# urw7rs/diffusion-models-made-easy

Hardware: AMD Instinct MI355X
Metric: denoising steps/sec + training images/sec, DDPM UNet CIFAR10 32×32 @1/2/4/8 GPU (higher is better)
Workload: dtype bf16; 1 GPU; DDPM T=1000 sampling, CIFAR10 32x32, default UNet (32,416,643 params, random init), batch 128 per GPU, t.shape=(1,); global_batch=128, parallelism=dp1 (independent chains per GPU, no data-path collective)

## Files before the change

### diffusion-models-made-easy_amd/_lib.py

```python

from __future__ import annotations

import ctypes as C
import os
import subprocess
import threading

_HERE = os.path.dirname(os.path.abspath(__file__))
LIB_PATH = os.environ.get("DMME_LIB_PATH") or os.path.join(_HERE, "libdmme_hip.so")
CSRC = os.path.join(_HERE, "csrc")

F16R32 = 4
F32, BF16, BF16X3, F16 = 0, 1, 2, 3
CHAIN_DDPM, CHAIN_DDIM, CHAIN_IDDPM, CHAIN_DDPM_GUIDED, CHAIN_DDIM_GUIDED, CHAIN_GDDIM = 0, 1, 2, 3, 4, 5
CHAIN_DDPM_CFG, CHAIN_GDDIM_CFG = 6, 7
CHAIN_DPMPP, CHAIN_DPMPP_CFG = 8, 9
CHAIN_REPAINT = 10
PRED_EPS, PRED_X0, PRED_V = 0, 1, 2
PREDICTIONS = {"eps": PRED_EPS, "x0": PRED_X0, "v": PRED_V}
ARCH_DDPM, ARCH_IDDPM, ARCH_CLASSIFIER, ARCH_DDPM_COND = 0, 1, 2, 3
DTYPES = {"fp32": F32, "float32": F32, "32": F32, "bf16": BF16, "bfloat16": BF16, "16": BF16, "bf16-mixed": BF16, "16-mixed": BF16,
          "bf16x3": BF16X3, "fp16": F16, "float16": F16, "half": F16, "fp16r32": F16R32}

_lock = threading.Lock()
# ... 7 lines not shown
        ("emb_dim", C.c_int),
        ("num_groups", C.c_int),
        ("dropout", C.c_float),
        ("num_depths", C.c_int),
        ("channels_per_depth", C.c_int * 8),
        ("num_blocks", C.c_int),
        ("num_attention_depths", C.c_int),
        ("attention_depths", C.c_int * 8),
        ("arch", C.c_int),
        ("num_heads", C.c_int),
        ("num_classes", C.c_int),
    ]


class ConvDesc(C.Structure):
    _fields_ = [(n, C.c_int) for n in (
        "dtype", "N", "Hin", "Win", "C1", "C2", "upsample", "stride", "taps", "Cout", "pro_silu", "out_silu",
        "nt", "tproj_ld", "in_nchw", "out_nchw", "force_generic")]


BUCKET_FN = C.CFUNCTYPE(None, C.c_void_p, C.c_int, C.c_int64, C.c_int64)


class DmmeError(RuntimeError):
    pass


def build(verbose: bool = False) -> str:
    cmd = ["make", "-C", CSRC, "-j", str(min(8, os.cpu_count() or 1))]
    res = subprocess.run(cmd, stdout=subprocess.PIPE, stderr=subprocess.STDOUT, text=True)
    if verbose or res.returncode != 0:
        print(res.stdout)
    if res.returncode != 0:
        raise DmmeError("building libdmme_hip.so failed")
    return LIB_PATH


_vp, _i, _i64, _f, _u64 = C.c_void_p, C.c_int, C.c_int64, C.c_float, C.c_uint64

PROTOTYPES = {
    "dmme_last_error": (C.c_char_p, []),
    "dmme_version": (_i, []),
    "dmme_device_count": (_i, []),
    "dmme_unet_plan_create": (_i, [C.POINTER(UNetCfg), _i, _i, _i, _i, _i, C.POINTER(_vp)]),
    "dmme_unet_plan_destroy": (None, [_vp]),
    "dmme_unet_plan_num_params": (_i, [_vp]),
    "dmme_unet_plan_param_info": (_i, [_vp, _i, C.c_char_p, _i, C.POINTER(_i), C.POINTER(_i64), C.POINTER(_i64), C.POINTER(_i)]),
    "dmme_unet_plan_ref_numel": (_i64, [_vp]),
    "dmme_unet_plan_packed_bytes": (_i64, [_vp]),
    "dmme_unet_plan_workspace_bytes": (_i64, [_vp]),
    "dmme_unet_plan_dropmask_numel": (_i64, [_vp]),
    "dmme_unet_plan_out_channels": (_i, [_vp]),
    "dmme_unet_plan_num_launches": (_i, [_vp]),
    "dmme_unet_pack_params": (_i, [_vp, _vp, _vp, _vp]),
    "dmme_unet_forward": (_i, [_vp, _vp, _vp, _vp, _i, _vp, _vp, _vp, _vp]),
    "dmme_unet_forward_nograd": (_i, [_vp, _vp, _vp, _vp, _i, _vp, _vp, _vp, _vp]),
    "dmme_unet_forward_cond": (_i, [_vp, _vp, _vp, _vp, _i, _vp, _vp, _vp, _vp, _i, _vp, _vp]),
    "dmme_unet_backward_cond": (_i, [_vp, _vp, _vp, _vp, _vp, _i, _vp, _vp, _vp, _vp, _vp, _vp, _vp, _vp, _vp, _vp]),
    "dmme_unet_backward_input_cond": (_i, [_vp, _vp, _vp, _vp, _vp, _i, _vp, _vp, _vp, _vp, _vp, _vp, _vp]),
    "dmme_label_dropout": (_i, [_vp, _i, _i, _f, _u64, _u64, _vp, _vp, _vp]),
    "dmme_cfg_step": (_i, [_i, _vp, _vp, _vp, _f, _f, _f, _f, _i, _i, _i64, _vp]),
    "dmme_chain_update_cfg": (_i, [_i, _vp, _vp, _vp, _vp, _vp, _vp, _i, _i64, _vp]),
    "dmme_cfg_chain_step": (_i, [_vp, _vp, _vp, _vp, _vp, _vp, _vp, _i, _vp, _vp, _vp, _vp]),
    "dmme_dpmpp_step": (_i, [_vp, _vp, _vp, C.POINTER(_f), _i, _i, _i64, _i, _vp]),
    "dmme_chain_update_dpmpp": (_i, [_vp, _vp, _vp, _vp, _vp, _vp, _i, _i64, _i, _vp]),
    "dmme_dpmpp_chain_step": (_i, [_vp, _vp, _vp, _vp, _vp, _vp, _vp, _vp, _vp, _vp]),
    "dmme_cfg_dpmpp_step": (_i, [_vp, _vp, _vp, C.POINTER(_f), _i, _i, _i64, _vp]),
    "dmme_chain_update_cfg_dpmpp": (_i, [_vp, _vp, _vp, _vp, _vp, _vp, _i, _i64, _vp]),
    "dmme_cfg_dpmpp_chain_step": (_i, [_vp, _vp, _vp, _vp, _vp, _vp, _vp, _vp, _vp, _vp, _vp, _vp]),
    "dmme_repaint_step": (_i, [_vp, _vp, _vp, _vp, _vp, C.POINTER(_f), _i, _i64, _i, _vp]),
    "dmme_chain_update_repaint": (_i, [_vp, _vp, _vp, _vp, _vp, _vp, _vp, _vp, _i, _i64, _i, _vp]),
    "dmme_repaint_chain_step": (_i, [_vp, _vp, _vp, _vp, _vp, _vp, _vp, _vp, _vp, _vp, _vp]),
    "dmme_unet_plan_num_ops": (_i, [_vp]),
    "dmme_unet_plan_level_info": (_i, [_vp, C.c_char_p, _i]),
    "dmme_unet_plan_check": (_i, [_vp]),
    "dmme_debug_level_stamps": (_i, [_vp, _i, _i]),
    "dmme_unet_plan_op_info": (_i, [_vp, _i, C.c_char_p, _i, C.POINTER(C.c_double), C.POINTER(C.c_double)]),
    "dmme_unet_forward_profiled": (_i, [_vp, _vp, _vp, _vp, _i, _vp, _vp, _vp, _vp, _vp]),
    "dmme_unet_plan_packed_bwd_bytes": (_i64, [_vp]),
    "dmme_unet_plan_bwd_workspace_bytes": (_i64, [_vp]),
    "dmme_unet_pack_params_bwd": (_i, [_vp, _vp, _vp, _vp]),
    "dmme_unet_backward": (_i, [_vp, _vp, _vp, _vp, _vp, _i, _vp, _vp, _vp, _vp, _vp, _vp, _vp]),
    "dmme_unet_backward_buckets": (_i, [_vp, _vp, _vp, _vp, _vp, _i, _vp, _vp, _vp, _vp, _vp, _vp, _vp, BUCKET_FN, _vp]),
    "dmme_unet_backward_input": (_i, [_vp, _vp, _vp, _vp, _vp, _i, _vp, _vp, _vp, _vp, _vp, _vp]),
    "dmme_unet_plan_grad_buckets": (_i, [_vp, C.POINTER(_i64), C.POINTER(_i64), C.POINTER(_i), _i]),
    "dmme_unet_plan_bwd_summary": (_i, [_vp, C.c_char_p, _i]),
    "dmme_grad_norm": (_i, [_vp, _i64, _vp, _vp, _vp]),
    "dmme_adam_step": (_i, [_vp, _vp, _vp, _vp, _vp, _i64, _f, _f, _f, _f, _i, _vp, _f, _f, _f, _vp]),
    "dmme_amp_init": (_i, [_vp, _f, _vp]),
    "dmme_amp_scale": (_i, [_vp, _i64, _vp, _vp]),
    "dmme_adam_step_amp": (_i, [_vp, _vp, _vp, _vp, _vp, _i64, _f, _f, _f, _f, _vp, _f, _f, _f, _vp, _f, _f, _i, _vp]),
    "dmme_grad_pack_bf16": (_i, [_vp, _i64, _vp, _i64, _vp]),
    "dmme_shard_reduce_bf16": (_i, [_vp, _i, _i64, _f, _vp, _vp]),
    "dmme_grad_unpack_bf16": (_i, [_vp, _i64, _vp, _vp]),
    "dmme_unet_debug_read": (_i, [_vp, _vp, C.c_char_p, _vp, _i64, C.POINTER(_i64), _vp]),
    "dmme_unet_debug_read_grad": (_i, [_vp, _vp, C.c_char_p, _vp, _i64, C.POINTER(_i64), _vp]),
    "dmme_unet_debug_read_norm_stats": (_i, [_vp, _vp, C.c_char_p, _vp, _i64, C.POINTER(_i64), _vp]),
    "dmme_dropout_masks": (_i, [_vp, _u64, _u64, _vp, _vp]),
    "dmme_randn": (_i, [_vp, _i64, _u64, _u64, _vp]),
    "dmme_q_sample": (_i, [_vp, _vp, _vp, _vp, _vp, _i, _i64, _vp, _vp, _vp]),
    "dmme_ddpm_step": (_i, [_vp, _vp, _vp, _f, _f, _f, _i, _i64, _vp]),
    "dmme_ddim_step": (_i, [_vp, _vp, _f, _f, _i64, _vp]),
    "dmme_gddim_step": (_i, [_vp, _vp, _vp, _f, _f, _f, _i64, _vp]),
    "dmme_slerp": (_i, [_vp, _vp, _vp, _i, _i, _i64, _vp, _vp]),
    "dmme_chain_set": (_i, [_vp, _i64, _vp, _u64, _u64, _vp]),
    "dmme_chain_update": (_i, [_i, _vp, _vp, _vp, _vp, _vp, _i, _i64, _vp]),
    "dmme_chain_step": (_i, [_vp, _vp, _vp, _vp, _vp, _i, _vp, _vp, _vp, _vp]),
    "dmme_chain_update_gddim": (_i, [_vp, _vp, _vp, _vp, _vp, _vp, _i, _i64, _vp]),
    "dmme_log_softmax_grad": (_i, [_vp, _vp, _i, _i, _i, _f, _vp, _vp, _vp, _vp]),
    "dmme_chain_update_guided": (_i, [_i, _vp, _vp, _vp, _vp, _vp, _vp, _vp, _i, _i64, _vp]),
    "dmme_guided_chain_step": (_i, [_vp, _vp, _vp, _vp, _vp, _vp, _vp, _vp, _vp, _vp, _vp, _vp, _vp, _vp, _vp, _i, _vp, _vp, _vp, _vp]),
    "dmme_mse_loss": (_i, [_vp, _vp, _i64, _vp, _vp, _f, _vp, _vp]),
    "dmme_pred_to_eps": (_i, [_i, _vp, _vp, _vp, _i, _vp, _i, _i, _i64, _vp]),
    "dmme_unet_plan_set_prediction": (_i, [_vp, _i, _vp, _i]),
    "dmme_q_sample_pred": (_i, [_i, _vp, _vp, _vp, _vp, _vp, _i, _i64, _vp, _vp, _vp]),
    "dmme_mse_loss_rows": (_i, [_vp, _vp, _vp, _vp, _i, _i64, _vp, _vp, _f, _vp, _vp]),
    "dmme_image_batch": (_i, [_vp, _i64, _vp, _vp, _i, _i, _i, _i, _vp, _vp]),
    "dmme_grid_tile": (_i, [_vp, _i, _i, _i, _i, _i, _i, _i, _i, _i, _i, _i, _vp, _vp]),
    "dmme_iddpm_step": (_i, [_vp, _vp, _vp, _f, _f, _f, _f, _i, _i, _i64, _vp]),
    "dmme_iddpm_loss": (_i, [_vp, _vp, _vp, _vp, _vp, _vp, _i, _i64, _f, _f, _vp, _vp, _f, _vp, _vp]),
    "dmme_iddpm_loss_rows": (_i, [_vp, _vp, _vp, _vp, _vp, _vp, _i, _vp, _i, _i64, _f, _f, _vp, _vp, _vp, _f, _vp, _vp, _vp]),
    "dmme_iddpm_prior_rows": (_i, [_vp, _i, _i64, _f, _vp, _vp]),
    "dmme_tsampler_draw": (_i, [_vp, _vp, _i, _i, _f, _u64, _u64, _i, _vp, _vp, _vp, _vp]),
    "dmme_tsampler_update": (_i, [_vp, _vp, _i, _i, _vp, _vp, _i, _vp, _vp]),
    "dmme_conv2d": (_i, [C.POINTER(ConvDesc), _vp, _vp, _vp, _vp, _vp, _vp, _vp, _vp, _vp, _vp, _i, _vp, _vp]),
    "dmme_conv2d_res": (_i, [C.POINTER(ConvDesc), _vp, _vp, _vp, _vp, _vp, _vp, _vp, _vp, _vp, _i, _i, _vp, _vp, _vp, _vp]),
    "dmme_groupnorm_scale_shift": (_i, [_i, _vp, _vp, _i, _i, _i, _i, _i, _vp, _vp, _f, _vp, _vp, _vp, _i, _vp]),
    "dmme_attention": (_i, [_i, _vp, _i, _i, _i, _vp, _i, _vp]),
    "dmme_attention_proj": (_i, [_i, _vp, _i, _i, _i, _vp, _vp, _vp, _vp, _vp, _vp, _i, _vp]),
    "dmme_attention_heads": (_i, [_i, _vp, _i, _i, _i, _i, _vp, _i, _vp]),
    "dmme_nchw_to_nhwc": (_i, [_i, _vp, _i, _i, _i, _vp, _vp]),
    "dmme_nhwc_to_nchw": (_i, [_i, _vp, _i, _i, _i, _vp, _vp]),
    "dmme_pack_weight": (_i, [_i, _vp, _i, _i, _i, _vp, _vp]),
    "dmme_event_create": (_i, [C.POINTER(_vp)]),
    "dmme_event_record": (_i, [_vp, _vp]),
    "dmme_event_elapsed_ms": (_i, [_vp, _vp, C.POINTER(_f)]),
    "dmme_event_destroy": (_i, [_vp]),
    "dmme_debug_set_stamps": (_i, [_vp]),
    "dmme_debug_mfma_valu": (_i, [_i, _i, _i, _vp, _vp]),
    "dmme_debug_issue_probe": (_i, [_i, _i, _i, _i, _i, _vp, _vp, _vp]),
    "dmme_debug_l2_stream": (_i, [_vp, _i64, _i, _i, _i, _i, _vp, _vp]),
}


def lib():
    global _lib
    if _lib is not None:
        return _lib
    with _lock:
        if _lib is not None:
            return _lib
        if not os.path.exists(LIB_PATH):
            raise DmmeError(
                f"{LIB_PATH} is missing: the HIP extension is not built. Run `python -c 'import __graft_entry__ as g; g.build()'` "
                "(or `make -C diffusion-models-made-easy_amd/csrc`). There is no CPU fallback for the product path."
            )
        h = C.CDLL(LIB_PATH)
        for name, (res, args) in PROTOTYPES.items():
            fn = getattr(h, name)
            fn.restype = res
            fn.argtypes = args
        _lib = h
    return _lib


def check(rc: int, what: str = ""):
    if rc != 0:
        msg = lib().dmme_last_error().decode("utf-8", "replace")
        if rc == -2:
            raise NotImplementedError(f"{what}: {msg}")
        if rc == -1:
            raise ValueError(f"{what}: {msg}")
        raise DmmeError(f"{what} failed (status {rc}): {msg}")


def require_gpu():
    if lib().dmme_device_count() <= 0:
        raise DmmeError("libdmme_hip.so loaded but no HIP device is visible; the denoiser path only runs on an MI355X")


def dtype_code(precision) -> int:
    key = str(precision).lower()
# ... 28 lines not shown
```

### diffusion-models-made-easy_amd/csrc/attn_mfma.hip

```cpp
#include <stdlib.h>

#include "conv_common.h"

namespace dmme {

typedef float f32x16 __attribute__((ext_vector_type(16)));
typedef __bf16 bf16x8 __attribute__((ext_vector_type(8)));
typedef short s16x4 __attribute__((ext_vector_type(4)));
typedef short s16x8 __attribute__((ext_vector_type(8)));

constexpr int AT_KT = 32;
#ifndef AT_PAIR_STEPS
#define AT_PAIR_STEPS 1
#endif

struct AttnGeom {
    int S, ld, Cfull, heads, N;
    float scale;
};
template <int D>
__device__ __forceinline__ int64_t at_qkv_off(const AttnGeom& g, int bh) {
    return (int64_t)(bh / g.heads) * g.S * g.ld + (int64_t)(bh % g.heads) * 3 * D;
}
template <int D>
__device__ __forceinline__ int64_t at_o_off(const AttnGeom& g, int bh) {
    return (int64_t)(bh % g.N) * g.S * g.Cfull + (int64_t)(bh / g.N) * D;
}

template <typename T, typename V>
__device__ __forceinline__ void at_mma(const V& a, const V& b, f32x16& acc);
template <>
__device__ __forceinline__ void at_mma<bf16, bf16x8>(const bf16x8& a, const bf16x8& b, f32x16& acc) {
    acc = __builtin_amdgcn_mfma_f32_32x32x16_bf16(a, b, acc, 0, 0, 0);
}
typedef f16 f16x8_at __attribute__((ext_vector_type(8)));
template <>
__device__ __forceinline__ void at_mma<f16, f16x8_at>(const f16x8_at& a, const f16x8_at& b, f32x16& acc) {
    acc = __builtin_amdgcn_mfma_f32_32x32x16_f16(a, b, acc, 0, 0, 0);
}

template <int C, int NW, typename T = bf16>
__global__ void __launch_bounds__(64 * NW) attn_mfma_kernel(const T* __restrict__ qkv, AttnGeom g, T* __restrict__ out, float* __restrict__ lse,
                                                            int xcd_order) {
    typedef T tx8 __attribute__((ext_vector_type(8)));
    constexpr int AT_QB = 32 * NW, NT = 64 * NW;
    const int S = g.S;
    constexpr int KSTEPS = C / 16;
    constexpr int CT = C / 32;
    constexpr int KP = C * 2 + 16;
    constexpr int VP = C * 2 + 64;
    constexpr bool QLDS = C > 128;
    constexpr int QP = C * 2 + 16;
    extern __shared__ __attribute__((aligned(16))) char lds[];
// ... 132 lines not shown
        }
        tx8 pf[2];
#pragma unroll
        for (int s2 = 0; s2 < 2; ++s2)
#pragma unroll
            for (int j = 0; j < 8; ++j) pf[s2][j] = (T)p[8 * s2 + j];
#pragma unroll
        for (int ct = 0; ct < CT; ct += VG) {
            const int cur = (ct / VG) & 1, nxt = cur ^ 1;
            if (ct + VG < CT) {
                AT_VREAD(ct + VG, vlo[nxt], vhi[nxt])
            }
            __builtin_amdgcn_sched_barrier(0);
#pragma unroll
            for (int cu = 0; cu < VG; ++cu)
#pragma unroll
                for (int s2 = 0; s2 < 2; ++s2) {
                    s16x8 vf;
                    vf[0] = vlo[cur][cu][s2][0]; vf[1] = vlo[cur][cu][s2][1]; vf[2] = vlo[cur][cu][s2][2]; vf[3] = vlo[cur][cu][s2][3];
                    vf[4] = vhi[cur][cu][s2][0]; vf[5] = vhi[cur][cu][s2][1]; vf[6] = vhi[cur][cu][s2][2]; vf[7] = vhi[cur][cu][s2][3];
                    at_mma<T>(__builtin_bit_cast(tx8, vf), pf[s2], o[ct + cu]);
                }
            __builtin_amdgcn_sched_barrier(0);
        }
#undef AT_VREAD
    }
    const float ltot = l + __shfl_xor(l, 32, 64);
    const float inv = 1.0f / ltot;
    if (lse && h == 0) lse[(int64_t)n * S + q_row] = m + log2f(ltot);
    T* orow = out + at_o_off<C>(g, n) + (int64_t)q_row * g.Cfull;
#pragma unroll
    for (int ct = 0; ct < CT; ++ct) {
#pragma unroll
        for (int jg = 0; jg < 4; ++jg) {
            typedef T bf16x4 __attribute__((ext_vector_type(4)));
            bf16x4 v;
#pragma unroll
            for (int e = 0; e < 4; ++e) v[e] = (T)(o[ct][jg * 4 + e] * inv);
            *reinterpret_cast<bf16x4*>(orow + ct * 32 + 8 * jg + 4 * h) = v;
        }
    }
}

struct AttnProj {
    const void* w;
    const float* bias;
    const void* res;
    void* dst;
    float* gn_part;
    int gn_tiles, gn_cg;
    long long* stamps;
    int dbg;
};
__device__ __forceinline__ float at_keep_f32(float x) {
    asm volatile("" : "+v"(x));
    return x;
}
__device__ __forceinline__ float at_sum64(float v) {
    v = half_sum(v);
    float a = v, b = v;
    permlane32_swap(a, b);
    return a + b;
}
template <int C, typename T = bf16, bool PROJ = false>
__global__ void __launch_bounds__(256) attn_full_kernel(const T* __restrict__ qkv, AttnGeom g, T* __restrict__ out, float* __restrict__ lse, int xcd_order, AttnProj pj) {
    typedef T tx8 __attribute__((ext_vector_type(8)));
    constexpr int S = 256, NKT = S / AT_KT, KSTEPS = C / 16, CT = C / 32;
    constexpr int NTOT = 2 * NKT + (PROJ ? CT : 0);
    constexpr int ROWB = C * 2, TILEB = AT_KT * ROWB;
    constexpr int DPT = TILEB / (256 * 16);
    constexpr bool PAIR = AT_PAIR_STEPS != 0;
    constexpr int NSLOT_BYTES = 8 * TILEB;
    constexpr int NSLOT = 8, AHEAD = PAIR ? 6 : 7;
    static_assert(!PAIR || (NTOT % 2 == 0 && NKT % 2 == 0), "pair steps: even tile counts per phase");
    static_assert(DPT >= 1 && DPT * 256 * 16 == TILEB, "attn_full: tile does not split over the DMA lanes");
    extern __shared__ __attribute__((aligned(16))) char lds[];
    const int tid = threadIdx.x, lane = tid & 63, wave = __builtin_amdgcn_readfirstlane(tid >> 6);
    const int r = lane & 31, h = lane >> 5;
    constexpr int qblocks = S / 128;
    int n = blockIdx.x / qblocks, qb = blockIdx.x % qblocks;
    if (xcd_order & 1) {
        const int x = blockIdx.x & 7, j = blockIdx.x >> 3;
        n = (j / qblocks) * 8 + x;
        qb = j % qblocks;
    }
    const T* base = qkv + at_qkv_off<C>(g, n);
    const int ld = g.ld;
    const int q_row = qb * 128 + wave * 32 + r;
    const unsigned lds0 = (unsigned)__builtin_amdgcn_readfirstlane((int)(unsigned)(size_t)(__attribute__((address_space(3))) char*)lds);
#ifdef AT_STAMPS
    long long* st_lds = reinterpret_cast<long long*>(lds + (PROJ ? (4 * 32 * (C * 4 + 16) > NSLOT_BYTES ? 4 * 32 * (C * 4 + 16) : NSLOT_BYTES) : NSLOT_BYTES));
    int st_i = 0;
    const bool stamping = PROJ && pj.stamps && blockIdx.x == 0 && tid == 0;
#define AF_STAMP() { if (PROJ && stamping && st_i < 120) st_lds[st_i++] = (long long)clock64(); }
#else
#define AF_STAMP()
#endif
    AF_STAMP()
    unsigned koff[DPT], voff[DPT];
#pragma unroll
    for (int i = 0; i < DPT; ++i) {
        const int I = wave + 4 * i, byte = I * 1024 + lane * 16, row = byte / ROWB, pc = (byte % ROWB) >> 4;
        koff[i] = (unsigned)(row * ld * 2 + (((pc & ~7) | ((pc & 7) ^ (row & 7))) << 4));
        voff[i] = (unsigned)(row * ld * 2 + (((pc & ~7) | ((pc & 7) ^ ((row & 3) << 1))) << 4));
    }
    unsigned woff[PROJ ? DPT : 1];
    if constexpr (PROJ) {
#pragma unroll
        for (int i = 0; i < DPT; ++i) {
            const int I = wave + 4 * i, byte = I * 1024 + lane * 16, row = byte / ROWB, pc = (byte % ROWB) >> 4;
            woff[i] = (unsigned)(row * ROWB + (((pc & ~7) | ((pc & 7) ^ (row & 7))) << 4));
        }
    }
    auto dma_tile = [&](int t) __attribute__((always_inline)) {
        const unsigned dst = lds0 + (unsigned)((t % NSLOT) * TILEB);
        if (PROJ && t >= 2 * NKT) {
            const char* src = (const char*)pj.w + (size_t)(t - 2 * NKT) * TILEB;
#pragma unroll
            for (int i = 0; i < DPT; ++i) glds16_hidden_s(src, woff[i], dst + (unsigned)((wave + 4 * i) * 1024));
            return;
        }
        const bool isv = t >= NKT;
        const T* kvb = (PROJ && (pj.dbg & 8)) ? qkv : base;
        const char* src = (const char*)(kvb + (int64_t)((isv ? t - NKT : t) * AT_KT) * ld + (isv ? 2 * C : C));
#pragma unroll
        for (int i = 0; i < DPT; ++i) glds16_hidden_s(src, isv ? voff[i] : koff[i], dst + (unsigned)((wave + 4 * i) * 1024));
    };
#pragma unroll
    for (int t = 0; t < AHEAD; ++t) dma_tile(t);
    uint4 qf[KSTEPS];
#pragma unroll
    for (int ks = 0; ks < KSTEPS; ++ks) qf[ks] = *reinterpret_cast<const uint4*>(base + (int64_t)q_row * ld + ks * 16 + h * 8);
    unsigned kb[4];
    {
        const int x = h ^ (r & 7);
#pragma unroll
        for (int i = 0; i < 4; ++i) kb[i] = lds0 + (unsigned)(r * ROWB + (((2 * i) ^ x) << 4));
    }
    const int tr_q = (lane & 15) >> 2, tr_p = lane & 3, tr_g1 = (lane >> 4) & 1;
    unsigned vb[2];
#pragma unroll
    for (int par = 0; par < 2; ++par)
        vb[par] = lds0 + (unsigned)((4 * h + tr_q) * ROWB + ((((par ^ (tr_q >> 1)) << 2) | ((tr_g1 ^ (tr_q & 1)) << 1) | (tr_p >> 1)) << 4) + ((tr_p & 1) << 3));
    typedef __attribute__((address_space(3))) char lc;
    typedef unsigned u32x4_af __attribute__((ext_vector_type(4)));
    typedef __attribute__((address_space(3))) u32x4_af lu4;

    f32x16 st[NKT];
#pragma unroll
    for (int t = 0; t < NKT; ++t)
#pragma unroll
        for (int j = 0; j < 16; ++j) st[t][j] = 0.f;
        \
#define AF_STEP_SYNC(TT)                                                                                                           \
    do {                                                                                                                           \
        if constexpr (PAIR) {                                                                                                      \
            if constexpr (((TT) & 1) != 0) break;   \
               \
            constexpr int last_ = (TT) + 5 < NTOT - 1 ? (TT) + 5 : NTOT - 1;                                                       \
            wait_vm_keep<(last_ - ((TT) + 1)) * DPT>();                                                                            \
            asm volatile("s_barrier" ::: "memory");                                                                                \
                                       \
            if ((TT) + 6 < NTOT) dma_tile((TT) + 6);                                                                               \
            if ((TT) + 7 < NTOT) dma_tile((TT) + 7);                                                                               \
        } else {                                                                                                                   \
        constexpr int younger_ = (TT) + AHEAD - 1 < NTOT ? AHEAD - 1 : NTOT - 1 - (TT);                                            \
        wait_vm_keep<younger_ * DPT>();                                                                                            \
        asm volatile("s_barrier" ::: "memory");                                                                                    \
        if ((TT) + AHEAD < NTOT) dma_tile((TT) + AHEAD);                                                                           \
        }                                                                                                                          \
        AF_STAMP()                                                                                                                 \
                                                                                               \
        if ((xcd_order >> 1) == 1) __builtin_amdgcn_s_sleep(2);                                                                    \
        else if ((xcd_order >> 1) == 2) __builtin_amdgcn_s_sleep(4);                                                               \
        else if ((xcd_order >> 1) == 3) __builtin_amdgcn_s_sleep(8);                                                               \
        else if ((xcd_order >> 1) == 4) __builtin_amdgcn_s_sleep(16);                                                              \
    } while (0)
#define AF_A_TILE(t, BF, ACC)                                                                                                      \
    {                                                                                                                              \
        AF_STEP_SYNC(t);                                                                                                           \
        constexpr unsigned so = (unsigned)(((t) % NSLOT) * TILEB);                                                                 \
        constexpr int FG = 4;                                                                                                      \
        uint4 kf[2][FG];                                                                                                           \
        _Pragma("unroll") for (int u = 0; u < FG; ++u) kf[0][u] = __builtin_bit_cast(uint4, *(const lu4*)((const lc*)(size_t)kb[u & 3] + (so + (unsigned)((2 * u) >> 3) * 128u))); \
        _Pragma("unroll") for (int g0 = 0; g0 < KSTEPS; g0 += FG) {                                                                \
            const int cur = (g0 / FG) & 1, nxt = cur ^ 1;                                                                          \
            if (g0 + FG < KSTEPS) {                                                                                                \
                _Pragma("unroll") for (int u = 0; u < FG; ++u) {                                                                   \
                    const int ks = g0 + FG + u;                                                                                    \
                    kf[nxt][u] = __builtin_bit_cast(uint4, *(const lu4*)((const lc*)(size_t)kb[ks & 3] + (so + (unsigned)((2 * ks) >> 3) * 128u)));           \
                }                                                                                                                  \
            }                                                                                                                      \
            __builtin_amdgcn_sched_barrier(0);                                                                                     \
            if (!(PROJ && (t) >= 2 * NKT && (pj.dbg & 4)))                                                                         \
            _Pragma("unroll") for (int u = 0; u < FG; ++u) at_mma<T>(__builtin_bit_cast(tx8, kf[cur][u]), __builtin_bit_cast(tx8, BF[g0 + u]), ACC); \
            __builtin_amdgcn_sched_barrier(0);                                                                                     \
        }                                                                                                                          \
        AF_STAMP()                                                                                                                 \
    }
#define AF_K_TILE(t) AF_A_TILE(t, qf, st[t])
    AF_K_TILE(0) AF_K_TILE(1) AF_K_TILE(2) AF_K_TILE(3) AF_K_TILE(4) AF_K_TILE(5) AF_K_TILE(6) AF_K_TILE(7)
#undef AF_K_TILE
    const float c1 = 1.4426950408889634f * g.scale;
    float mx = st[0][0];
#pragma unroll
    for (int t = 0; t < NKT; ++t)
#pragma unroll
        for (int j = 0; j < 16; ++j) mx = fmaxf(mx, st[t][j]);
    mx = fmaxf(mx, __shfl_xor(mx, 32, 64));
    const float m = mx * c1;
    float l = 0.f;
    tx8 pf[NKT][2];
#pragma unroll
    for (int t = 0; t < NKT; ++t)
#pragma unroll
        for (int j = 0; j < 16; ++j) {
            const float p = __builtin_amdgcn_exp2f(fmaf(st[t][j], c1, -m));
            l += p;
            pf[t][j >> 3][j & 7] = (T)p;
        }
    const float ltot = l + __shfl_xor(l, 32, 64);
    AF_STAMP()
    f32x16 o[CT];
#pragma unroll
    for (int ct = 0; ct < CT; ++ct)
#pragma unroll
        for (int j = 0; j < 16; ++j) o[ct][j] = 0.f;
#define AF_VREAD(CT0, DST_LO, DST_HI)                                                                                              \
    _Pragma("unroll") for (int cu = 0; cu < VG; ++cu) _Pragma("unroll") for (int s2 = 0; s2 < 2; ++s2) {                            \
        const int ct_ = (CT0) + cu;                                                                                                \
        const lc* a0 = (const lc*)(size_t)vb[ct_ & 1] + (so + (unsigned)((16 * s2) * ROWB + (ct_ >> 1) * 128));                     \
        DST_LO[cu][s2] = __builtin_amdgcn_ds_read_tr16_b64_v4i16((__attribute__((address_space(3))) s16x4*)a0);                    \
        DST_HI[cu][s2] = __builtin_amdgcn_ds_read_tr16_b64_v4i16((__attribute__((address_space(3))) s16x4*)(a0 + 8 * ROWB));       \
    }
#define AF_V_TILE(t)                                                                                                               \
    {                                                                                                                              \
        AF_STEP_SYNC(NKT + (t));                                                                                                   \
        constexpr unsigned so = (unsigned)(((NKT + (t)) % NSLOT) * TILEB);                                                         \
        constexpr int VG = 2;                                                                                                      \
        s16x4 vlo[2][VG][2], vhi[2][VG][2];                                                                                        \
        AF_VREAD(0, vlo[0], vhi[0])                                                                                                \
        _Pragma("unroll") for (int ct = 0; ct < CT; ct += VG) {                                                                    \
            const int cur = (ct / VG) & 1, nxt = cur ^ 1;                                                                          \
            if (ct + VG < CT) {                                                                                                    \
                AF_VREAD(ct + VG, vlo[nxt], vhi[nxt])                                                                              \
            }                                                                                                                      \
            __builtin_amdgcn_sched_barrier(0);                                                                                     \
            _Pragma("unroll") for (int cu = 0; cu < VG; ++cu) _Pragma("unroll") for (int s2 = 0; s2 < 2; ++s2) {                    \
                s16x8 vf;                                                                                                          \
                vf[0] = vlo[cur][cu][s2][0]; vf[1] = vlo[cur][cu][s2][1]; vf[2] = vlo[cur][cu][s2][2]; vf[3] = vlo[cur][cu][s2][3]; \
                vf[4] = vhi[cur][cu][s2][0]; vf[5] = vhi[cur][cu][s2][1]; vf[6] = vhi[cur][cu][s2][2]; vf[7] = vhi[cur][cu][s2][3]; \
                at_mma<T>(__builtin_bit_cast(tx8, vf), pf[t][s2], o[ct + cu]);                                                     \
            }                                                                                                                      \
            __builtin_amdgcn_sched_barrier(0);                                                                                     \
        }                                                                                                                          \
        AF_STAMP()                                                                                                                 \
    }
    AF_V_TILE(0) AF_V_TILE(1) AF_V_TILE(2) AF_V_TILE(3) AF_V_TILE(4) AF_V_TILE(5) AF_V_TILE(6) AF_V_TILE(7)
#undef AF_V_TILE
#undef AF_VREAD
    const float inv = 1.0f / ltot;
    if constexpr (!PROJ) {
        if (lse && h == 0) lse[(int64_t)n * S + q_row] = m + log2f(ltot);
        T* orow = out + at_o_off<C>(g, n) + (int64_t)q_row * g.Cfull;
#pragma unroll
        for (int ct = 0; ct < CT; ++ct) {
#pragma unroll
            for (int jg = 0; jg < 4; ++jg) {
                typedef T tx4 __attribute__((ext_vector_type(4)));
                tx4 v;
#pragma unroll
                for (int e = 0; e < 4; ++e) v[e] = (T)at_keep_f32(o[ct][jg * 4 + e] * inv);
                *reinterpret_cast<tx4*>(orow + ct * 32 + 8 * jg + 4 * h) = v;
            }
        }
    } else {
        uint4 of[KSTEPS];
#pragma unroll
        for (int ct = 0; ct < CT; ++ct)
#pragma unroll
            for (int s2 = 0; s2 < 2; ++s2) {
                typedef T tx2 __attribute__((ext_vector_type(2)));
                float w4[4];
#pragma unroll
                for (int p2 = 0; p2 < 4; ++p2) {
                    const int j = (2 * s2 + (p2 >> 1)) * 4 + (p2 & 1) * 2;
                    tx2 v;
                    v[0] = (T)at_keep_f32(o[ct][j] * inv);
                    v[1] = (T)at_keep_f32(o[ct][j + 1] * inv);
                    w4[p2] = __builtin_bit_cast(float, v);
                }
                permlane32_swap(w4[0], w4[2]);
                permlane32_swap(w4[1], w4[3]);
                of[2 * ct + s2] = make_uint4(__builtin_bit_cast(unsigned, w4[0]), __builtin_bit_cast(unsigned, w4[1]), __builtin_bit_cast(unsigned, w4[2]),
                                             __builtin_bit_cast(unsigned, w4[3]));
            }
        AF_STAMP()
        f32x16 ot[CT];
#pragma unroll
        for (int t = 0; t < CT; ++t)
#pragma unroll
            for (int j = 0; j < 16; ++j) ot[t][j] = 0.f;
#define AF_W_TILE(t) AF_A_TILE(2 * NKT + (t), of, ot[t])
        AF_W_TILE(0) AF_W_TILE(1) AF_W_TILE(2) AF_W_TILE(3)
        if constexpr (CT > 4) { AF_W_TILE(4) AF_W_TILE(5) AF_W_TILE(6) AF_W_TILE(7) }
#undef AF_W_TILE
        if (lse && h == 0) lse[(int64_t)n * S + q_row] = m + log2f(ltot);
        asm volatile("s_barrier" ::: "memory");
        AF_STAMP()
        constexpr int SP = C * 4 + 16;
        constexpr int LPR = C / 8, RPI = 64 / LPR, NIT = 32 / RPI;
        char* stg = lds + wave * (32 * SP);
        const int col = lane % LPR, rsub = lane / LPR;
        const int64_t tile_off = at_o_off<C>(g, n) + (int64_t)(q_row - r) * g.Cfull + col * 8;
        if (out) {
            constexpr int CP = C * 2 + 16;
#pragma unroll
            for (int ks = 0; ks < KSTEPS; ++ks) *reinterpret_cast<uint4*>(stg + r * CP + (ks * 16 + h * 8) * 2) = of[ks];
            wait_lgkm_all();
            asm volatile("" ::: "memory");
            T* obase = out + tile_off;
#pragma unroll
            for (int i = 0; i < NIT; ++i)
                *reinterpret_cast<uint4*>(obase + (int64_t)(rsub + RPI * i) * g.Cfull) = *reinterpret_cast<const uint4*>(stg + (rsub + RPI * i) * CP + col * 16);
            wait_lgkm_all();
            asm volatile("" ::: "memory");
        }
#pragma unroll
        for (int t = 0; t < CT; ++t)
#pragma unroll
            for (int jg = 0; jg < 4; ++jg)
                *reinterpret_cast<f32x4*>(stg + r * SP + (t * 32 + 8 * jg + 4 * h) * 4) = f32x4{ot[t][jg * 4], ot[t][jg * 4 + 1], ot[t][jg * 4 + 2], ot[t][jg * 4 + 3]};
        const T* rbase = (const T*)pj.res + tile_off;
        T* dbase = (T*)pj.dst + tile_off;
        if (pj.dbg & 2) {
            if (ot[0][0] == 12345.f) dbase[0] = (T)ot[CT - 1][3];
            return;
        }
        uint4 rv[NIT];
#pragma unroll
        for (int i = 0; i < NIT; ++i) rv[i] = *reinterpret_cast<const uint4*>(rbase + (int64_t)(rsub + RPI * i) * g.Cfull);
        const f32x4 b0 = *reinterpret_cast<const f32x4*>(pj.bias + col * 8), b1 = *reinterpret_cast<const f32x4*>(pj.bias + col * 8 + 4);
        wait_lgkm_all();
        asm volatile("" ::: "memory");
        AF_STAMP()
        float xs[NIT][8];
#pragma unroll
        for (int i = 0; i < NIT; ++i) {
            const char* sp = stg + (rsub + RPI * i) * SP + col * 32;
            const f32x4 a0 = *reinterpret_cast<const f32x4*>(sp), a1 = *reinterpret_cast<const f32x4*>(sp + 16);
            const tx8 y = __builtin_bit_cast(tx8, rv[i]);
            tx8 o8;
#pragma unroll
            for (int e = 0; e < 4; ++e) {
                o8[e] = (T)(a0[e] + b0[e] + (float)y[e]);
                o8[4 + e] = (T)(a1[e] + b1[e] + (float)y[4 + e]);
// ... 3 lines not shown
            *reinterpret_cast<uint4*>(dbase + (int64_t)(rsub + RPI * i) * g.Cfull) = __builtin_bit_cast(uint4, o8);
        }
        AF_STAMP()
        if (pj.gn_part && !(pj.dbg & 1)) {
            auto col_sum = [&](float v) __attribute__((always_inline)) -> float {
                if constexpr (LPR == 16) {
                    float a = v, b = v;
                    permlane16_swap(a, b);
                    v = a + b;
                }
                float a = v, b = v;
                permlane32_swap(a, b);
                return a + b;
            };
            const bool cg8 = pj.gn_cg == 8;
            float sA = 0.f, sB = 0.f;
#pragma unroll
            for (int i = 0; i < NIT; ++i)
#pragma unroll
                for (int e = 0; e < 4; ++e) {
                    sA += xs[i][e];
                    sB += xs[i][4 + e];
                }
            if (cg8) sA = sB = sA + sB;
            const float inv_n = cg8 ? 1.f / 256.f : 1.f / 128.f;
            const float mA = col_sum(sA) * inv_n, mB = col_sum(sB) * inv_n;
            float qA = 0.f, qB = 0.f;
#pragma unroll
            for (int i = 0; i < NIT; ++i)
#pragma unroll
                for (int e = 0; e < 4; ++e) {
                    const float da = xs[i][e] - mA, db = xs[i][4 + e] - mB;
                    qA = fmaf(da, da, qA);
                    qB = fmaf(db, db, qB);
                }
            if (cg8) qA = qB = qA + qB;
            const float m2A = col_sum(qA), m2B = col_sum(qB);
            const int tile_s = (q_row - r) >> 5, G = C / pj.gn_cg;
            float* po = pj.gn_part + ((int64_t)n * pj.gn_tiles + tile_s) * G * 2;
            if (lane < LPR) {
                if (cg8) *reinterpret_cast<f32x2*>(po + col * 2) = f32x2{mA, m2A};
                else *reinterpret_cast<f32x4*>(po + col * 4) = f32x4{mA, m2A, mB, m2B};
            }
        }
        AF_STAMP()
#ifdef AT_STAMPS
        if (stamping)
            for (int i = 0; i < st_i; ++i) pj.stamps[i] = st_lds[i];
#endif
    }
#undef AF_STAMP
#undef AF_A_TILE
#undef AF_STEP_SYNC
}

template <int C, typename T = bf16>
__global__ void __launch_bounds__(256) attn_split_kernel(const T* __restrict__ qkv, AttnGeom g, T* __restrict__ out, float* __restrict__ lse) {
    typedef T tx8 __attribute__((ext_vector_type(8)));
    constexpr int S = 256, KSTEPS = C / 16, CT = C / 32;
    constexpr int ROWB = C * 2, TILEB = AT_KT * ROWB;
    constexpr int DPT = TILEB / 1024;
    constexpr int QB = S / 32;
    extern __shared__ __attribute__((aligned(16))) char lds[];
    const int tid = threadIdx.x, lane = tid & 63, wave = __builtin_amdgcn_readfirstlane(tid >> 6);
    const int r = lane & 31, h = lane >> 5;
    const int n = blockIdx.x / QB, qb = blockIdx.x % QB;
    const T* base = qkv + at_qkv_off<C>(g, n);
    const int ld = g.ld;
    const int q_row = qb * 32 + r;
    char* ldsW = lds + wave * 2 * TILEB;
    float* xch = reinterpret_cast<float*>(lds + 4 * 2 * TILEB);
    const unsigned lw0 = (unsigned)__builtin_amdgcn_readfirstlane((int)(unsigned)(size_t)(__attribute__((address_space(3))) char*)ldsW);
    unsigned koff[DPT], voff[DPT];
#pragma unroll
    for (int i = 0; i < DPT; ++i) {
        const int byte = i * 1024 + lane * 16, row = byte / ROWB, pc = (byte % ROWB) >> 4;
        koff[i] = (unsigned)(row * ld * 2 + (((pc & ~7) | ((pc & 7) ^ (row & 7))) << 4));
        voff[i] = (unsigned)(row * ld * 2 + (((pc & ~7) | ((pc & 7) ^ ((row & 3) << 1))) << 4));
    }
    auto dma_k = [&](int kt, int slot) __attribute__((always_inline)) {
        const char* src = (const char*)(base + (int64_t)(kt * AT_KT) * ld + C);
#pragma unroll
        for (int i = 0; i < DPT; ++i) glds16_hidden_s(src, koff[i], lw0 + (unsigned)(slot * TILEB + i * 1024));
    };
    auto dma_v = [&](int kt, int slot) __attribute__((always_inline)) {
        const char* src = (const char*)(base + (int64_t)(kt * AT_KT) * ld + 2 * C);
#pragma unroll
        for (int i = 0; i < DPT; ++i) glds16_hidden_s(src, voff[i], lw0 + (unsigned)(slot * TILEB + i * 1024));
    };
    dma_k(2 * wave, 0);
    dma_k(2 * wave + 1, 1);
    uint4 qf[KSTEPS];
#pragma unroll
    for (int ks = 0; ks < KSTEPS; ++ks) qf[ks] = *reinterpret_cast<const uint4*>(base + (int64_t)q_row * ld + ks * 16 + h * 8);
    unsigned kb[4];
    {
        const int x = h ^ (r & 7);
#pragma unroll
        for (int i = 0; i < 4; ++i) kb[i] = lw0 + (unsigned)(r * ROWB + (((2 * i) ^ x) << 4));
    }
    const int tr_q = (lane & 15) >> 2, tr_p = lane & 3, tr_g1 = (lane >> 4) & 1;
    unsigned vb[2];
#pragma unroll
    for (int par = 0; par < 2; ++par)
        vb[par] = lw0 + (unsigned)((4 * h + tr_q) * ROWB + ((((par ^ (tr_q >> 1)) << 2) | ((tr_g1 ^ (tr_q & 1)) << 1) | (tr_p >> 1)) << 4) + ((tr_p & 1) << 3));
    typedef __attribute__((address_space(3))) char lc;
// ... 56 lines not shown
                const s16x4 lo = __builtin_amdgcn_ds_read_tr16_b64_v4i16((__attribute__((address_space(3))) s16x4*)a0);
                const s16x4 hi = __builtin_amdgcn_ds_read_tr16_b64_v4i16((__attribute__((address_space(3))) s16x4*)(a0 + 8 * ROWB));
                s16x8 vf;
                vf[0] = lo[0]; vf[1] = lo[1]; vf[2] = lo[2]; vf[3] = lo[3];
                vf[4] = hi[0]; vf[5] = hi[1]; vf[6] = hi[2]; vf[7] = hi[3];
                at_mma<T>(__builtin_bit_cast(tx8, vf), pf[t][s2], o[ct]);
            }
    }
    __syncthreads();
    float* red = reinterpret_cast<float*>(lds);
#pragma unroll
    for (int ct = 0; ct < CT; ++ct)
#pragma unroll
        for (int j = 0; j < 16; ++j) red[((wave * CT + ct) * 16 + j) * 64 + lane] = o[ct][j];
    __syncthreads();
    const float inv = 1.0f / ltot;
    if (lse && wave == 0 && h == 0) lse[(int64_t)n * S + q_row] = m + log2f(ltot);
    T* orow = out + at_o_off<C>(g, n) + (int64_t)q_row * g.Cfull;
    constexpr int CPW = CT / 4;
#pragma unroll
    for (int c = 0; c < CPW; ++c) {
        const int ct = wave * CPW + c;
#pragma unroll
        for (int jg = 0; jg < 4; ++jg) {
            typedef T tx4 __attribute__((ext_vector_type(4)));
            tx4 v;
#pragma unroll
            for (int e = 0; e < 4; ++e) {
                const int j = jg * 4 + e;
                float sum = 0.f;
#pragma unroll
                for (int w = 0; w < 4; ++w) sum += red[((w * CT + ct) * 16 + j) * 64 + lane];
                v[e] = (T)(sum * inv);
            }
            *reinterpret_cast<tx4*>(orow + ct * 32 + 8 * jg + 4 * h) = v;
        }
    }
}

template <int D, typename T>
static int launch_attn_split_t(const T* qkv, const AttnGeom& g, T* out, float* lse, hipStream_t s) {
    const int rows = g.N * g.heads;
    const size_t lds = (size_t)8 * AT_KT * D * 2 + 1024;
    static bool attr_done = false;
    if (!attr_done) {
        DMME_CHECK_HIP(hipFuncSetAttribute(reinterpret_cast<const void*>(attn_split_kernel<D, T>), hipFuncAttributeMaxDynamicSharedMemorySize, 160 * 1024));
        attr_done = true;
    }
    hipLaunchKernelGGL((attn_split_kernel<D, T>), dim3((unsigned)(rows * 8)), dim3(256), lds, s, qkv, g, out, lse);
    DMME_CHECK_LAUNCH();
    return DMME_OK;
}

template <int D, typename T, bool PROJ = false>
static int launch_attn_full_t(const T* qkv, const AttnGeom& g, T* out, float* lse, hipStream_t s, const AttnProj& pj = AttnProj{}) {
    const int rows = g.N * g.heads;
    const size_t ring = (size_t)8 * AT_KT * D * 2, stage = (size_t)4 * 32 * (D * 4 + 16);
#ifdef AT_STAMPS
    const size_t lds = (PROJ && stage > ring ? stage : ring) + 1024;
#else
    const size_t lds = PROJ && stage > ring ? stage : ring;
#endif
    static bool attr_done = false;
    if (!attr_done) {
        DMME_CHECK_HIP(hipFuncSetAttribute(reinterpret_cast<const void*>(attn_full_kernel<D, T, PROJ>), hipFuncAttributeMaxDynamicSharedMemorySize, 160 * 1024));
        attr_done = true;
    }
    const int xcd_order = ((!debug_route("no_xcd_order") && rows % 8 == 0) ? 1 : 0) | ((debug_route("attn_sleep", -1) >= 0 ? debug_route("attn_sleep", -1) : rows * 2 >= 256 ? 2 : 0) << 1);
    hipLaunchKernelGGL((attn_full_kernel<D, T, PROJ>), dim3((unsigned)(rows * 2)), dim3(256), lds, s, qkv, g, out, lse, xcd_order, pj);
    DMME_CHECK_LAUNCH();
    return DMME_OK;
}
bool attn_full_takes(int S, int D) {
    return S == 256 && (D == 128 || D == 256) && !getenv("DMME_NO_ATTN_FULL");
}

bool attn_mfma_supported(int dtype, int N, int S, int C) { return attn_heads_mfma_supported(dtype, N, S, C, 1); }
bool attn_heads_mfma_supported(int dtype, int N, int S, int C, int heads) {
    (void)N;
    if (!is16(dtype) || heads < 1 || C % heads) return false;
    const int D = C / heads;
    return (D == 64 || D == 128 || D == 256) && S >= 64 && S % 64 == 0 && (S % 128 == 0 || S == 64);
}
static AttnGeom attn_geom(int N, int S, int C, int heads) { return AttnGeom{S, 3 * C, C, heads, N, 1.0f / sqrtf((float)C)}; }

template <int D, int NW, typename T>
static int launch_attn_fwd_nw(const T* qkv, const AttnGeom& g, T* out, float* lse, hipStream_t s) {
    const int rows = g.N * g.heads, qblocks = g.S / (32 * NW);
    const size_t lds = (size_t)AT_KT * (D * 2 + 16) + (size_t)AT_KT * (D * 2 + 64) + (D > 128 ? (size_t)32 * NW * (D * 2 + 16) : 0);
    static bool attr_done = false;
    if (!attr_done) {
        DMME_CHECK_HIP(hipFuncSetAttribute(reinterpret_cast<const void*>(attn_mfma_kernel<D, NW, T>), hipFuncAttributeMaxDynamicSharedMemorySize, 128 * 1024));
        attr_done = true;
    }
    const bool xcd_off = (debug_route("no_xcd_order") != 0);
    const int xcd_order = (!xcd_off && qblocks > 1 && rows % 8 == 0) ? 1 : 0;
    hipLaunchKernelGGL((attn_mfma_kernel<D, NW, T>), dim3((unsigned)(rows * qblocks)), dim3(64 * NW), lds, s, qkv, g, out, lse, xcd_order);
    DMME_CHECK_LAUNCH();
    return DMME_OK;
}
template <int D, typename T>
static int launch_attn_fwd_t(const T* qkv, const AttnGeom& g, T* out, float* lse, hipStream_t s) {
    if (g.S % 128 == 0) return launch_attn_fwd_nw<D, 4, T>(qkv, g, out, lse, s);
    return launch_attn_fwd_nw<D, 2, T>(qkv, g, out, lse, s);
}
int launch_attn_heads_mfma(int dtype, const void* qkv, int N, int S, int C, int heads, void* out, float* lse, hipStream_t s) {
    DMME_REQUIRE(attn_heads_mfma_supported(dtype, N, S, C, heads), DMME_ERR_UNSUPPORTED, "attn_mfma: unsupported shape S=%d C=%d heads=%d", S, C, heads);
    const AttnGeom g = attn_geom(N, S, C, heads);
    if (attn_full_takes(S, C / heads) && N * heads * 2 < 256 && !debug_route("no_attn_split")) {
        if (dtype == DMME_F16)
            return C / heads == 256 ? launch_attn_split_t<256, f16>((const f16*)qkv, g, (f16*)out, lse, s) : launch_attn_split_t<128, f16>((const f16*)qkv, g, (f16*)out, lse, s);
        return C / heads == 256 ? launch_attn_split_t<256, bf16>((const bf16*)qkv, g, (bf16*)out, lse, s) : launch_attn_split_t<128, bf16>((const bf16*)qkv, g, (bf16*)out, lse, s);
    }
    if (attn_full_takes(S, C / heads)) {
        if (dtype == DMME_F16)
            return C / heads == 256 ? launch_attn_full_t<256, f16>((const f16*)qkv, g, (f16*)out, lse, s) : launch_attn_full_t<128, f16>((const f16*)qkv, g, (f16*)out, lse, s);
        return C / heads == 256 ? launch_attn_full_t<256, bf16>((const bf16*)qkv, g, (bf16*)out, lse, s) : launch_attn_full_t<128, bf16>((const bf16*)qkv, g, (bf16*)out, lse, s);
    }
    if (dtype == DMME_F16) {
        switch (C / heads) {
            case 256: return launch_attn_fwd_t<256, f16>((const f16*)qkv, g, (f16*)out, lse, s);
            case 128: return launch_attn_fwd_t<128, f16>((const f16*)qkv, g, (f16*)out, lse, s);
            default: return launch_attn_fwd_t<64, f16>((const f16*)qkv, g, (f16*)out, lse, s);
        }
    }
    switch (C / heads) {
        case 256: return launch_attn_fwd_t<256, bf16>((const bf16*)qkv, g, (bf16*)out, lse, s);
        case 128: return launch_attn_fwd_t<128, bf16>((const bf16*)qkv, g, (bf16*)out, lse, s);
        default: return launch_attn_fwd_t<64, bf16>((const bf16*)qkv, g, (bf16*)out, lse, s);
    }
}
int launch_attn_mfma(int dtype, const void* qkv, int N, int S, int C, void* out, float* lse, hipStream_t s) {
    return launch_attn_heads_mfma(dtype, qkv, N, S, C, 1, out, lse, s);
}
static bool attn_proj_shape_ok(int dtype, int N, int S, int C, int gn_cg, int gn_tiles) {
    if (!is16(dtype) || S != 256 || (C != 128 && C != 256) || N * 2 < 256) return false;
    return gn_tiles == 0 || ((gn_cg == 4 || gn_cg == 8) && C % gn_cg == 0 && gn_tiles == S / 32);
}
bool attn_proj_fusable(int dtype, int N, int S, int C, int gn_cg, int gn_tiles) {
    if (!attn_full_takes(S, C) || debug_route("no_attn_proj")) return false;
    return attn_proj_shape_ok(dtype, N, S, C, gn_cg, gn_tiles);
}
int launch_attn_proj(int dtype, const void* qkv, int N, int S, int C, void* ctx, float* lse, const void* w, const float* bias, const void* res, void* dst,
                     float* gn_part, int gn_tiles, int gn_cg, hipStream_t s, long long* stamps) {
    DMME_REQUIRE(attn_proj_shape_ok(dtype, N, S, C, gn_part ? gn_cg : 0, gn_part ? gn_tiles : 0) && w && bias && res && dst, DMME_ERR_UNSUPPORTED,
                 "attn_proj: unsupported shape N=%d S=%d C=%d (statistics tiles %d, %d channels per group)", N, S, C, gn_tiles, gn_cg);
    const AttnGeom g = attn_geom(N, S, C, 1);
    const AttnProj pj{w, bias, res, dst, gn_part, gn_tiles, gn_cg, stamps, debug_route("attn_proj_dbg")};
    if (dtype == DMME_F16)
        return C == 256 ? launch_attn_full_t<256, f16, true>((const f16*)qkv, g, (f16*)ctx, lse, s, pj) : launch_attn_full_t<128, f16, true>((const f16*)qkv, g, (f16*)ctx, lse, s, pj);
    return C == 256 ? launch_attn_full_t<256, bf16, true>((const bf16*)qkv, g, (bf16*)ctx, lse, s, pj) : launch_attn_full_t<128, bf16, true>((const bf16*)qkv, g, (bf16*)ctx, lse, s, pj);
}

template <int C, int NW, typename T>
__global__ void __launch_bounds__(64 * NW, 1) attn_bwd_scores_kernel(const T* __restrict__ qkv, const T* __restrict__ O,
                                                              const T* __restrict__ dO, const float* __restrict__ lse, AttnGeom g,
                                                              T* __restrict__ P, T* __restrict__ dS) {
    constexpr int AT_QB = 32 * NW, NT = 64 * NW;
    const int S = g.S, ld = g.ld;
    constexpr int KSTEPS = C / 16;
    constexpr int KP = C * 2 + 16;
    __shared__ __attribute__((aligned(16))) char lds[2 * AT_KT * KP];
    char* ldsK = lds;
    char* ldsV = lds + AT_KT * KP;
    const int tid = threadIdx.x, lane = tid & 63, wave = tid >> 6;
    const int r = lane & 31, h = lane >> 5;
    const int qblocks = S / AT_QB;
    const int n = blockIdx.x / qblocks, qb = blockIdx.x % qblocks;
    const T* base = qkv + at_qkv_off<C>(g, n);
    const int64_t orow = at_o_off<C>(g, n);
    const int q_row = qb * AT_QB + wave * 32 + r;
    uint4 qf[KSTEPS], dof[KSTEPS];
    float dpart = 0.f;
#pragma unroll
    for (int ks = 0; ks < KSTEPS; ++ks) {
        qf[ks] = *reinterpret_cast<const uint4*>(base + (int64_t)q_row * ld + ks * 16 + h * 8);
        dof[ks] = *reinterpret_cast<const uint4*>(dO + orow + (int64_t)q_row * g.Cfull + ks * 16 + h * 8);
        const uint4 ov = *reinterpret_cast<const uint4*>(O + orow + (int64_t)q_row * g.Cfull + ks * 16 + h * 8);
        const typename Vec8<T>::type a = __builtin_bit_cast(typename Vec8<T>::type, dof[ks]), b = __builtin_bit_cast(typename Vec8<T>::type, ov);
#pragma unroll
        for (int j = 0; j < 8; ++j) dpart = fmaf((float)a[j], (float)b[j], dpart);
    }
    const float delta = dpart + __shfl_xor(dpart, 32, 64);
    const float L = lse[(int64_t)n * S + q_row];
    const float c1 = 1.4426950408889634f * g.scale;
    T* Prow = P + ((int64_t)n * S + q_row) * S;
    T* dSrow = dS + ((int64_t)n * S + q_row) * S;

    constexpr int NV = AT_KT * (C / 8) / NT;
    static_assert(NV * NT == AT_KT * (C / 8), "whole vectors per thread");
    typedef unsigned atb_u32x4 __attribute__((ext_vector_type(4)));
    atb_u32x4 kreg[NV], vreg[NV];
#define ATB_FETCH(K0)                                                                     \
    _Pragma("unroll") for (int i = 0; i < NV; ++i) {                                       \
        const int u = tid + i * NT, row = u / (C / 8), cu = u % (C / 8);                   \
        const T* src = base + (int64_t)((K0) + row) * ld + cu * 8;                      \
        kreg[i] = *reinterpret_cast<const atb_u32x4*>(src + C);                            \
        vreg[i] = *reinterpret_cast<const atb_u32x4*>(src + 2 * C);                        \
    }
    ATB_FETCH(0)
    for (int k0 = 0; k0 < S; k0 += AT_KT) {
        __syncthreads();
#pragma unroll
        for (int i = 0; i < NV; ++i) {
// ... 192 lines not shown
```

### diffusion-models-made-easy_amd/csrc/common.h

```cpp
#pragma once

#include <hip/hip_runtime.h>
#include <stdint.h>

#include "dmme_hip.h"

namespace dmme {

void set_error(const char* fmt, ...) __attribute__((format(printf, 1, 2)));

int debug_route(const char* key, int dflt = 0);

#define DMME_CHECK_HIP(expr)                                                                          \
    do {                                                                                              \
        hipError_t e_ = (expr);                                                                       \
        if (e_ != hipSuccess) {                                                                       \
            ::dmme::set_error("%s failed: %s (%s:%d)", #expr, hipGetErrorString(e_), __FILE__, __LINE__); \
            return DMME_ERR_HIP;                                                                      \
        }                                                                                             \
    } while (0)

#define DMME_REQUIRE(cond, code, ...)        \
    do {                                     \
        if (!(cond)) {                       \
// ... 231 lines not shown
bool conv1x1_split_route(int dtype, const ConvArgs& a, ConvRoute& r);
bool conv1x1_domain(int dtype, const ConvArgs& a);
bool conv1x1_as_route(int dtype, const ConvArgs& a, ConvRoute& r);
bool conv1x1_tiled_route(int dtype, const ConvArgs& a, ConvRoute& r);
bool conv3x3_split_route(int dtype, const ConvArgs& a, ConvRoute& r);
bool conv3x3_pipe_route(int dtype, const ConvArgs& a, ConvRoute& r);
bool conv3x3_ws_route(int dtype, const ConvArgs& a, ConvRoute& r);
bool conv3x3_kw_route(int dtype, const ConvArgs& a, ConvRoute& r);
bool conv_mfma_route(int dtype, const ConvArgs& a, ConvRoute& r);
void conv_generic_route(const ConvArgs& a, ConvRoute& r);
bool conv_mfma_supported(int dtype, const ConvArgs& a);
int launch_conv_generic(int dtype, const ConvArgs& a, hipStream_t s);
const char* conv_generic_kernel_name(const ConvArgs& a);
int launch_conv_mfma(const ConvRoute& r, int dtype, const ConvArgs& a, hipStream_t s);
int launch_conv_out_thin(const ConvArgs& a, hipStream_t s);
int launch_conv1x1(const ConvRoute& r, int dtype, const ConvArgs& a, hipStream_t s);
int launch_conv1x1_as(const ConvArgs& a, hipStream_t s);
int launch_conv3x3(const ConvRoute& r, int dtype, const ConvArgs& a, hipStream_t s);
int launch_conv_kw(int dtype, const ConvArgs& a, const ConvTile& g, int NI, int ring, int BM, int ksplit, hipStream_t s);
int launch_conv(int dtype, const ConvArgs& a, hipStream_t s, int force = 0);
int launch_conv(const ConvRoute& r, int dtype, const ConvArgs& a, hipStream_t s);
void conv_label(const ConvRoute& r, int dtype, const ConvArgs& a, char* buf, int cap);
bool conv_stats_query(int dtype, const ConvArgs& a, int cg, int* tiles, int* px);
bool conv_gn_in_query(int dtype, const ConvArgs& a);
bool conv1x1_tiled_gn_in_ok(const ConvArgs& a, const ConvRoute& r);
bool conv3x3_pipe_gn_in_ok(int dtype, const ConvArgs& a, const ConvRoute& r);
int conv_gn_direct_query(int dtype, const ConvArgs& a, const int* cg, int n);
int launch_gn_finalize_parts(const float* part1, int tiles1, int cnt1, int C1, const float* part2, int tiles2, int cnt2, int C2, int N, int groups,
                             const float* gamma, const float* beta, float eps, float* scale, float* shift, float* mean_rstd, const float* t_shift,
                             const float* t_scale, int t_ld, int nt, hipStream_t s);

int launch_gn_generic(int dtype, const void* src1, const void* src2, int N, int HW, int C1, int C2, int groups,
                      const float* gamma, const float* beta, float eps, float* scale, float* shift, float* mean_rstd,
                      hipStream_t s);
bool gn_fast_supported(int dtype, int N, int HW, int C1, int C2, int groups);
size_t gn_fast_scratch_floats(int N, int HW, int C, int groups);
int launch_gn_fast(int dtype, const void* src1, const void* src2, int N, int HW, int C1, int C2, int groups,
                   const float* gamma, const float* beta, float eps, float* scale, float* shift, float* mean_rstd,
                   float* partial, hipStream_t s, void* act = nullptr, int act_silu = 0, const float* dmask = nullptr);
bool gn_small_act_supported(int dtype, int HW, int C1, int C2, int groups);

int launch_attn_generic(int dtype, const void* qkv, int N, int S, int C, void* out, hipStream_t s);
int launch_attn_heads(int dtype, const void* qkv, int N, int S, int C, int heads, void* out, hipStream_t s);
int launch_attn_heads_bwd(int dtype, const void* qkv, const void* dO, int N, int S, int C, int heads, float* P, float* dS, void* dqkv, hipStream_t s);
int launch_gn_modulate(float* scale, float* shift, const float* t_shift, const float* t_scale, int ld, int nt, int N, int C, hipStream_t s);
bool attn_x3_supported(int N, int S, int C, int heads);
int launch_attn_x3(const void* qkv, int N, int S, int C, int heads, void* out, hipStream_t s);
bool attn_mfma_supported(int dtype, int N, int S, int C);
bool attn_full_takes(int S, int D);
int launch_attn_mfma(int dtype, const void* qkv, int N, int S, int C, void* out, float* lse, hipStream_t s);
bool attn_proj_fusable(int dtype, int N, int S, int C, int gn_cg, int gn_tiles);
int launch_attn_proj(int dtype, const void* qkv, int N, int S, int C, void* ctx, float* lse, const void* w, const float* bias, const void* res, void* dst,
                     float* gn_part, int gn_tiles, int gn_cg, hipStream_t s, long long* stamps = nullptr);
bool attn_heads_mfma_supported(int dtype, int N, int S, int C, int heads);
int launch_attn_heads_mfma(int dtype, const void* qkv, int N, int S, int C, int heads, void* out, float* lse, hipStream_t s);
int launch_attn_heads_bwd_mfma(int dtype, const void* qkv, const void* O, const void* dO, const float* lse, int N, int S, int C, int heads, void* P,
                               void* dS, void* dqkv, hipStream_t s);
bool attn_bwd_mfma_supported(int dtype, int N, int S, int C);
int launch_attn_bwd_mfma(int dtype, const void* qkv, const void* O, const void* dO, const float* lse, int N, int S, int C, void* P, void* dS,
                         void* dqkv, hipStream_t s);

constexpr unsigned kFwdMarkKeep = 0x4B454550u, kFwdMarkNograd = 0x4E4F4752u;
constexpr unsigned kErrNogradBackward = 0x80000000u;
int launch_time_sinusoid(const int64_t* t, int nt, const float* freqs, int half, float* out, hipStream_t s, unsigned* mark = nullptr,
                         unsigned mark_val = 0);
int launch_linear_wave(int dtype, const float* in, int nt, int K, const void* W, const float* bias, int Nout,
                       int out_silu, float* out, hipStream_t s);
int launch_label_cond(const float* z2, int nt, const float* E, const int64_t* labels, int B, int K, int emb, float* temb, float* zsave, int* status,
                      hipStream_t s);
int launch_label_grad(const float* dz2, const int64_t* labels, int B, int K, int emb, float* dE, hipStream_t s);

int launch_nchw_to_nhwc(int dtype, const float* src, int N, int C, int HW, void* dst, hipStream_t s, const unsigned* mark = nullptr,
                        unsigned* err = nullptr);
int launch_nhwc_to_nchw(int dtype, const void* src, int N, int C, int HW, float* dst, hipStream_t s);
int launch_pack_weight(int dtype, const float* src, int Cout, int Cin, int taps, void* dst, hipStream_t s);
int launch_cast_f32_to_16(int dtype, const float* src, int64_t numel, void* dst, hipStream_t s);

struct PackItem {
    int64_t src_off;
    int64_t dst_off;
    int32_t cout, cin, taps;
    int32_t row0, rows;
    int32_t ci0, nci;
    int32_t as_f32;
};
int launch_pack_table(int dtype, const PackItem* items_dev, int n_items, const float* ref_flat, void* packed,
                      hipStream_t s);

int launch_randn(float* out, int64_t numel, uint64_t seed, uint64_t offset, hipStream_t s);
int launch_dropmask(float* out, int64_t numel, float p, uint64_t seed, uint64_t offset, hipStream_t s);
int launch_q_sample(const float* x0, const float* z, const float* sqrt_abar, const float* sqrt_1m_abar,
                    const int64_t* t, int B, int64_t chw, float* x_t, float* target, hipStream_t s);
int launch_pred_to_eps(int pred, float* model_out, const float* x, const float* ab, int T, const int64_t* t, int t_len, int B, int64_t chw,
                       hipStream_t s);
int slerp_parts(int64_t chw);
int launch_slerp(const float* xa, const float* xb, const float* w, int n, int B, int64_t chw, float* out, float* scratch, hipStream_t s);
int launch_chain_set(void* state, int64_t i, const int64_t* t_table, uint64_t seed, uint64_t offset, hipStream_t s);

constexpr bool kind_known(int k) { return k >= DMME_CHAIN_DDPM && k <= DMME_CHAIN_REPAINT; }
constexpr bool kind_cfg(int k) { return k == DMME_CHAIN_DDPM_CFG || k == DMME_CHAIN_GDDIM_CFG || k == DMME_CHAIN_DPMPP_CFG; }
constexpr int kind_base(int k) {
    return k == DMME_CHAIN_DDPM_CFG ? DMME_CHAIN_DDPM : k == DMME_CHAIN_GDDIM_CFG ? DMME_CHAIN_GDDIM : k == DMME_CHAIN_DPMPP_CFG ? DMME_CHAIN_DPMPP : k;
}
constexpr bool kind_hist(int k) { return kind_base(k) == DMME_CHAIN_DPMPP; }
constexpr bool kind_paint(int k) { return k == DMME_CHAIN_REPAINT; }
constexpr int kind_row(int k) { return kind_hist(k) || kind_paint(k) ? 8 : 4; }
// ... 166 lines not shown
```

### diffusion-models-made-easy_amd/csrc/kernels_generic.hip

```cpp
#include <stdlib.h>

#include <algorithm>

#include "common.h"

namespace dmme {

template <typename T>
__global__ void __launch_bounds__(256) conv_generic_kernel(ConvArgs a) {
    const int64_t total = (int64_t)a.N * a.Hout * a.Wout * a.Cout;
    const int Cin = a.C1 + a.C2;
    const int Hv = a.up ? 2 * a.Hin : a.Hin, Wv = a.up ? 2 * a.Win : a.Win;
    const int k = a.taps == 9 ? 3 : 1, pad = a.taps == 9 ? 1 : 0;
    for (int64_t idx = blockIdx.x * (int64_t)blockDim.x + threadIdx.x; idx < total;
         idx += (int64_t)gridDim.x * blockDim.x) {
        const int co = (int)(idx % a.Cout);
        int64_t p = idx / a.Cout;
        const int ow = (int)(p % a.Wout);
        p /= a.Wout;
        const int oh = (int)(p % a.Hout);
        const int n = (int)(p / a.Hout);
        const T* w = (const T*)a.w + (int64_t)co * a.taps * Cin;
        const float* sc = a.scale ? a.scale + (int64_t)n * Cin : nullptr;
        const float* sh = a.scale ? a.shift + (int64_t)n * Cin : nullptr;
// ... 765 lines not shown
                T o[V];
#pragma unroll
                for (int j = 0; j < V; ++j) o[j] = from_f<T>(tile[co * pitch + (cv * V + j) * taps + tap]);
                *reinterpret_cast<uint4*>(dst + ((int64_t)(it.row0 + co) * taps + tap) * it.cin + it.ci0 + cv * V) = *reinterpret_cast<const uint4*>(o);
            }
        } else {
            for (int e = threadIdx.x; e < total; e += blockDim.x) {
                const int cil = e % nci, q = e / nci, tap = q % taps, co = q / taps;
                dst[((int64_t)(it.row0 + co) * taps + tap) * it.cin + it.ci0 + cil] = from_f<T>(tile[co * pitch + cil * taps + tap]);
            }
        }
    }
}
template <typename T>
__global__ void __launch_bounds__(256) cast_f32_to_16_kernel(const float* __restrict__ src, int64_t nvec, T* __restrict__ dst) {
    for (int64_t v = (int64_t)blockIdx.x * blockDim.x + threadIdx.x; v < nvec; v += (int64_t)gridDim.x * blockDim.x) {
        typedef float f4 __attribute__((ext_vector_type(4)));
        typedef T t8 __attribute__((ext_vector_type(8)));
        const f4 a = *reinterpret_cast<const f4*>(src + 8 * v), b = *reinterpret_cast<const f4*>(src + 8 * v + 4);
        t8 o;
#pragma unroll
        for (int e = 0; e < 4; ++e) {
            o[e] = (T)a[e];
            o[4 + e] = (T)b[e];
        }
        *reinterpret_cast<t8*>(dst + 8 * v) = o;
    }
}
int launch_cast_f32_to_16(int dtype, const float* src, int64_t numel, void* dst, hipStream_t s) {
    DMME_REQUIRE(is16(dtype) && numel % 8 == 0, DMME_ERR_INVALID, "cast: 16-bit destination types, whole 16-byte vectors");
    const int64_t nvec = numel / 8;
    const unsigned blocks = (unsigned)std::min<int64_t>((nvec + 255) / 256, 256 * 16);
    if (dtype == DMME_F16)
        hipLaunchKernelGGL(cast_f32_to_16_kernel<f16>, dim3(blocks), dim3(256), 0, s, src, nvec, (f16*)dst);
    else
        hipLaunchKernelGGL(cast_f32_to_16_kernel<bf16>, dim3(blocks), dim3(256), 0, s, src, nvec, (bf16*)dst);
    DMME_CHECK_LAUNCH();
    return DMME_OK;
}

int launch_pack_table(int dtype, const PackItem* items_dev, int n_items, const float* ref_flat, void* packed,
                      hipStream_t s) {
    if (n_items == 0) return DMME_OK;
    if (dtype == DMME_BF16)
        hipLaunchKernelGGL(pack_table_kernel<bf16>, dim3(n_items), dim3(256), 0, s, items_dev, ref_flat, (char*)packed);
    else if (dtype == DMME_F16)
        hipLaunchKernelGGL(pack_table_kernel<f16>, dim3(n_items), dim3(256), 0, s, items_dev, ref_flat, (char*)packed);
    else
        hipLaunchKernelGGL(pack_table_kernel<float>, dim3(n_items), dim3(256), 0, s, items_dev, ref_flat, (char*)packed);
    DMME_CHECK_LAUNCH();
    return DMME_OK;
}

template <int DEPTH>
__global__ void __launch_bounds__(256) l2_stream_kernel(const uint4* __restrict__ buf, int nvec, int iters, unsigned* __restrict__ sink) {
    unsigned acc = 0;
    const int tid = threadIdx.x;
    for (int it = 0; it < iters; ++it) {
        for (int base = 0; base + DEPTH * 256 <= nvec; base += DEPTH * 256) {
            uint4 v[DEPTH];
#pragma unroll
            for (int d = 0; d < DEPTH; ++d) v[d] = buf[base + d * 256 + tid];
#pragma unroll
            for (int d = 0; d < DEPTH; ++d) acc ^= v[d].x ^ v[d].y ^ v[d].z ^ v[d].w;
        }
    }
    if (acc == 0x12345u) sink[blockIdx.x] = acc;
}
typedef __attribute__((address_space(3))) char l2s_lds_c;
template <int DEPTH>
__global__ void __launch_bounds__(256) l2_stream_dma_kernel(const uint4* __restrict__ buf, int nvec, int iters, unsigned* __restrict__ sink, int row_stride) {
    extern __shared__ __attribute__((aligned(16))) char lds[];
    const int tid = threadIdx.x, wave = tid >> 6;
    (void)wave;
    unsigned acc = 0;
    for (int it = 0; it < iters; ++it) {
        int gbase = 0;
        for (int base = 0; base + DEPTH * 256 <= nvec; base += DEPTH * 256) {
            if (row_stride) {
                gbase += DEPTH * 32 * row_stride;
                if (gbase + (DEPTH * 32 + 32) * row_stride >= nvec) gbase = 0;
            }
#pragma unroll
            for (int d = 0; d < DEPTH; ++d) {
#if defined(__HIP_DEVICE_COMPILE__)
                const unsigned l = (unsigned)__builtin_amdgcn_readfirstlane((int)((unsigned)(size_t)(l2s_lds_c*)lds + (unsigned)((d * 4 + wave) * 1024)));
                const int idx = row_stride ? gbase + (d * 32 + (tid >> 3)) * row_stride + (tid & 7) : base + d * 256 + tid;
                __builtin_amdgcn_global_load_lds(buf + idx, (l2s_lds_c*)(size_t)l, 16, 0, 0);
#endif
            }
#if defined(__HIP_DEVICE_COMPILE__)
            asm volatile("s_waitcnt vmcnt(0)" ::: "memory");
#endif
        }
        acc ^= reinterpret_cast<unsigned*>(lds)[tid];
    }
    if (acc == 0x12345u) sink[blockIdx.x] = acc;
}
typedef float f32x16_d __attribute__((ext_vector_type(16)));
typedef __bf16 bf16x8_d __attribute__((ext_vector_type(8)));
__global__ void __launch_bounds__(512, 1) mfma_valu_kernel(int mode, int iters, float* __restrict__ sink) {
    const int wave = threadIdx.x >> 6;
    float out = 0.f;
    if (wave < 4) {
        if (!(mode & 1)) return;
        bf16x8_d a, b;
// ... 215 lines not shown
```

### diffusion-models-made-easy_amd/csrc/plan.h

```cpp
#pragma once
#include <stdarg.h>
#include <stdlib.h>
#include <stdio.h>
#include <string.h>

#include <algorithm>
#include <memory>
#include <string>
#include <unordered_map>
#include <vector>

#include "common.h"
#include "lvl.h"

namespace dmme {

static inline int64_t align_up(int64_t v, int64_t a) { return (v + a - 1) / a * a; }

template <typename T>
class DevTable {
    T* p_ = nullptr;

public:
    DevTable() = default;
// ... 44 lines not shown
    bool is_buffer = false;
    bool as_f32 = true;
    int pack_code = -1;
    int cout = 1, cin = 1, taps = 1;
    int64_t numel() const { return shape[0] * shape[1] * shape[2] * shape[3]; }
};

struct Tensor {
    int64_t off = 0;
    int C = 0, H = 0, W = 0;
    int f32 = 0;
    int64_t stats_off = -1;
    int stats_tiles = 0, stats_cnt = 0;
};

enum OpKind { OP_SINUS, OP_LINEAR, OP_GN, OP_CONV, OP_ATTN, OP_CAST, OP_LABEL };

struct Op {
    OpKind kind;
    int64_t lin_in = 0, lin_out = 0;
    int lin_K = 0, lin_N = 0, lin_w = -1, lin_b = -1, lin_silu = 0;
    int64_t lin_pre = -1;
    int gn_src1 = -1, gn_src2 = -1, gn_gamma = -1, gn_beta = -1;
    int64_t b_rowsum = 0, b_ab = 0;
    int64_t b_gnrows = -1;
    int gn_rows_deferred = 0;
    int64_t gn_scale = 0, gn_shift = 0, gn_mr = 0;
    int gn_mod_col = -1, gn_mod_C = 0;
    int64_t gn_act = -1;
    int gn_force_small = 0;
    int gn_consumer = -1;
    int gn_direct = 0;
    int gn_in_consumer = 0;
    int src1 = -1, src2 = -1;
    int w = -1, b = -1;
    int gn = -1;
    int pro_silu = 0, out_silu = 0;
    int64_t dmask_off = -1;
    int tproj_col = -1;
    int res1 = -1, res2 = -1;
    int dst = -1;
    int up = 0, stride = 1, taps = 9;
    int use_act = 0;
    int gd_n = 0, gd_gn[2] = {-1, -1}, gd_coff[2] = {0, 0};
    int gd_act = -1;
    int res_alias = 0;
    int rseg = -1, fused_away = 0;
    int wg_layer = -1;
    int64_t wg_act = -1;
    int bias_deferred = 0;
    int at_qkv = -1, at_out = -1, at_heads = 1;
    int64_t at_lse = 0;
    int at_proj = -1;
    int mix = 0, route_f32 = 0;
    int mix2 = 0;
    int cast_src = -1, cast_dst = -1;
    int lvl = -1, lvl_first = 0;
};

struct LvlRun {
    int op_first = 0, op_last = 0;
    int sh = 0, NG = 0, NGS = 0, GB = 1, NJ = 1;
    std::vector<LvlOp> ops;
    std::vector<std::pair<int, int>> made;
    DevTable<LvlOp> ops_dev;
    std::vector<LvlOp> ops_nograd;
    DevTable<LvlOp> ops_nograd_dev;
    int raw_skipped = 0;
    DevTable<unsigned> sync_dev;
    double flops = 0, bytes = 0;
};

}

using namespace dmme;

struct dmme_plan {
    dmme_unet_cfg cfg;
    int B, H, W, dtype, device;
    int x3 = 0;
    int mix = 0;
    int out_channels = 0;
    int head_src = -1, p_hgw = -1, p_hgb = -1, p_hw = -1, p_hb = -1;
    int64_t bws_hpool = 0, bws_hrows = 0;
    int cond = 0, p_lemb = -1, label_op = -1;
    std::vector<Param> params;
    std::vector<Tensor> tensors;
    std::vector<Op> ops;
    std::unordered_map<std::string, int> named;
    int64_t ref_numel = 0, packed_bytes = 0, ws_bytes = 0, dropmask_numel = 0;
    int64_t ws_tsin = 0, ws_th1 = 0, ws_temb = 0, ws_tproj = 0, ws_gnpart = 0;
    int64_t ws_mark = 0;
    int64_t ws_tz1 = -1, ws_tz2 = -1;
    int64_t ws_splitk = 0, splitk_floats = 0;
    int tproj_cols = 0;
    int64_t tproj_w_off = 0, tproj_b_off = 0;
    int freqs_param = -1;
    DevTable<PackItem> items_dev;
    int n_items = 0;
    int n_launches = 0;
    struct TBlock { int tw, tb, col, cout; };
    std::vector<TBlock> tblocks;
    int p_l1w = -1, p_l1b = -1, p_l2w = -1, p_l2b = -1;
    int64_t packed_bwd_bytes = 0, bws_bytes = 0;
    std::vector<int64_t> gt_off;
    int64_t bws_zero = 0, bws_zero_bytes = 0, bws_wimage = 0, bws_gnS = 0, bws_zpage = 0;
    DevTable<PackItem> items_unpack_dev;
    int n_items_unpack = 0;
    int64_t bws_sink = 0, sink_half = 0;
    int64_t bws_tmp = 0, bws_dy = 0, bws_rowsum = 0, bws_dtproj = 0, bws_dtemb = 0, bws_dh1 = 0, bws_z = 0, bws_wT = 0, bws_attP = 0,
            bws_attdS = 0;
    DevTable<PackItem> items_bwd_dev;
    int n_items_bwd = 0;
    struct WgGroup {
        int taps = 0;
        std::vector<WgLayer> layers;
        std::vector<WgJob> jobs;
        DevTable<WgLayer> layers_dev;
        DevTable<WgJob> jobs_dev;
        int dma = 0;
        int stride = 1;
    } wg[3];
    struct GradBucket {
        int op_lo = 0, op_hi = 0;
        WgGroup wg[3];
        int col0 = 0, col1 = 0, bias0 = 0, bias1 = 0;
        std::vector<std::pair<int, int>> unpack, tcols;
        std::vector<std::pair<int64_t, int64_t>> ranges;
    };
    std::vector<GradBucket> gb;
    std::vector<int64_t> tp_tiles;
    DevTable<int64_t> tp_tiles_dev;
    int tp_n64 = 0;
    std::vector<BiasJob> bias_jobs;
    DevTable<BiasJob> bias_jobs_dev;
    std::vector<ColJob> col_jobs;
    DevTable<ColJob> col_jobs_dev;
    std::vector<LvlRun> lvl_runs;
    int lvl_max_wg = LVL_MAX_WG;
    PinnedWord err_host;
    mutable const void* nograd_ws = nullptr;
    int pred = DMME_PRED_EPS, pred_T = 0;
    const float* pred_ab = nullptr;
};

namespace dmme {

constexpr int kR32TwoPassDefault = 0;
static inline int conv_dt(const dmme_plan* P, const Op& o) { return o.route_f32 ? DMME_F32 : P->dtype; }
static inline int wg_index(const Op& o) { return o.taps == 1 ? 1 : o.stride == 2 ? 2 : 0; }

void fill_conv(const dmme_plan* P, const Op& o, const char* packed, const float* x, float* y, char* ws, const float* drop_masks, int nt, ConvArgs& a,
               bool fwd = false);
bool gn_from_parts(const dmme_plan* P, const Op& o);
void assign_levels(dmme_plan* P);
void assign_rseg(dmme_plan* P);
int run_level(const dmme_plan* P, const LvlRun& R, const char* pk, char* ws, int nt, const float* drop_masks, hipStream_t s, bool keep_ctx = true);
void assign_lvl_nograd(dmme_plan* P);
int lvl_check(const dmme_plan* P, const char* where, hipStream_t stream = nullptr, bool have_stream = false);
void build_unpack_items(const dmme_plan* P, std::vector<PackItem>& items);
void plan_backward(dmme_plan* P);

}
```

### diffusion-models-made-easy_amd/csrc/plan.hip

```cpp
#include "plan.h"

#include <functional>
#include <map>
#include <mutex>

namespace dmme {

static thread_local char g_err[512] = "";
void set_error(const char* fmt, ...) {
    va_list ap;
    va_start(ap, fmt);
    vsnprintf(g_err, sizeof(g_err), fmt, ap);
    va_end(ap);
}

int debug_route(const char* key, int dflt) {
    const char* e = getenv("DMME_DEBUG_ROUTE");
    if (!e || !*e) return dflt;
    const size_t kl = strlen(key);
    for (const char* p = e; *p;) {
        const char* end = strchr(p, ',');
        const size_t len = end ? (size_t)(end - p) : strlen(p);
        if (len >= kl && !strncmp(p, key, kl) && (len == kl || p[kl] == '=')) return len == kl ? 1 : atoi(p + kl + 1);
        if (!end) break;
// ... 864 lines not shown
    if (debug_route("no_rseg") || !is16(P->dtype) || P->mix || P->x3) return;
    std::vector<int> uses(P->tensors.size(), 0), producer(P->tensors.size(), -1);
    for (int oi = 0; oi < (int)P->ops.size(); ++oi) {
        const Op& o = P->ops[oi];
        for (int id : {o.src1, o.src2, o.res1, o.res2, o.gn_src1, o.gn_src2, o.at_qkv, o.cast_src})
            if (id >= 0) ++uses[id];
        if (o.kind == OP_CONV && o.dst >= 0) producer[o.dst] = oi;
    }
    for (int ci = 0; ci < (int)P->ops.size(); ++ci) {
        Op& c2 = P->ops[ci];
        if (c2.kind != OP_CONV || c2.taps != 9 || c2.lvl >= 0 || c2.res1 < 0 || c2.res2 >= 0 || c2.dst < 0 || c2.mix || c2.route_f32) continue;
        const int ri = producer[c2.res1];
        if (ri < 0 || uses[c2.res1] != 1) continue;
        Op& rc = P->ops[ri];
        if (rc.kind != OP_CONV || rc.taps != 1 || rc.lvl >= 0 || rc.gn >= 0 || rc.pro_silu || rc.out_silu || rc.dmask_off >= 0 || rc.tproj_col >= 0 || rc.res1 >= 0 ||
            rc.up || rc.stride != 1 || rc.src1 < 0 || rc.gd_n > 0 || rc.mix || rc.route_f32)
            continue;
        for (const auto& kv : P->named)
            if (kv.second == c2.res1) goto next;
        {
            c2.rseg = ri;
            ConvArgs a{};
            fill_conv(P, c2, (const char*)4096, (const float*)4096, (float*)4096, (char*)4096, nullptr, 1, a, true);
            if (!conv_route(P->dtype, a).rseg) {
                c2.rseg = -1;
                continue;
            }
            rc.fused_away = 1;
        }
    next:;
    }
}

void assign_attn_proj(dmme_plan* P) {
    if (P->x3) return;
    for (int ai = 0; ai + 1 < (int)P->ops.size(); ++ai) {
        Op& at = P->ops[ai];
        if (at.kind != OP_ATTN || at.lvl >= 0 || at.at_heads != 1) continue;
        Op& pr = P->ops[ai + 1];
        if (pr.kind != OP_CONV || pr.src1 != at.at_out || pr.src2 >= 0 || pr.taps != 1 || pr.lvl >= 0 || pr.gn >= 0 || pr.pro_silu || pr.out_silu || pr.dmask_off >= 0 ||
            pr.tproj_col >= 0 || pr.res1 < 0 || pr.res2 >= 0 || pr.up || pr.stride != 1 || pr.gd_n > 0 || pr.mix || pr.route_f32 || pr.dst < 0 || pr.fused_away || pr.rseg >= 0)
            continue;
        const Tensor &q = P->tensors[at.at_qkv], &td = P->tensors[pr.dst];
        if (q.f32 || td.f32 || P->tensors[pr.res1].f32 || P->tensors[at.at_out].f32) continue;
        const int S = q.H * q.W, C = q.C / 3;
        if (td.C != C || P->tensors[pr.res1].C != C) continue;
        const bool stats = td.stats_off >= 0;
        if (!attn_proj_fusable(P->dtype, P->B, S, C, stats ? td.C / P->cfg.num_groups : 0, stats ? td.stats_tiles : 0)) continue;
        at.at_proj = ai + 1;
        pr.fused_away = 2;
    }
}

int run_gn(const dmme_plan* P, const Op& o, const char* pk, char* ws, int nt, const float* drop_masks, hipStream_t s) {
    if (o.gn_direct || o.gn_in_consumer) return DMME_OK;
    const float* tsh = o.gn_mod_col >= 0 ? (const float*)(ws + P->ws_tproj) + o.gn_mod_col : nullptr;
    const float* tsc = tsh ? tsh + o.gn_mod_C : nullptr;
    int rc;
    const Tensor& t1 = P->tensors[o.gn_src1];
    const void* s1 = ws + t1.off;
    const void* s2 = o.gn_src2 >= 0 ? ws + P->tensors[o.gn_src2].off : nullptr;
    const int C2 = o.gn_src2 >= 0 ? P->tensors[o.gn_src2].C : 0;
    const float* gam = (const float*)(pk + P->params[o.gn_gamma].packed_off);
    const float* bet = (const float*)(pk + P->params[o.gn_beta].packed_off);
    float* sc = (float*)(ws + o.gn_scale);
    float* sh = (float*)(ws + o.gn_shift);
    if (gn_from_parts(P, o)) {
        const Tensor* t2 = o.gn_src2 >= 0 ? &P->tensors[o.gn_src2] : nullptr;
        return launch_gn_finalize_parts((const float*)(ws + t1.stats_off), t1.stats_tiles, t1.stats_cnt, t1.C,
                                        t2 ? (const float*)(ws + t2->stats_off) : nullptr, t2 ? t2->stats_tiles : 0,
                                        t2 ? t2->stats_cnt : 0, C2, P->B, P->cfg.num_groups, gam, bet, 1e-5f, sc, sh,
                                        (float*)(ws + o.gn_mr), tsh, tsc, P->tproj_cols, nt, s);
    }
    const int gdt = t1.f32 ? DMME_F32 : P->dtype;
    if (gn_fast_supported(gdt, P->B, t1.H * t1.W, t1.C, C2, P->cfg.num_groups)) {
        void* act = nullptr;
        int act_silu = 0;
        const float* dm = nullptr;
        if (o.gn_act >= 0) {
            const Op& cv = P->ops[o.gn_consumer];
            act = ws + o.gn_act;
            act_silu = cv.pro_silu;
            if (cv.dmask_off >= 0 && drop_masks) dm = drop_masks + cv.dmask_off;
        }
        rc = launch_gn_fast(gdt, s1, s2, P->B, t1.H * t1.W, t1.C, C2, P->cfg.num_groups, gam, bet, 1e-5f, sc, sh,
                            (float*)(ws + o.gn_mr), (float*)(ws + P->ws_gnpart), s, act, act_silu, dm);
    }
    else
        rc = launch_gn_generic(gdt, s1, s2, P->B, t1.H * t1.W, t1.C, C2, P->cfg.num_groups, gam, bet, 1e-5f, sc, sh,
                               (float*)(ws + o.gn_mr), s);
    if (rc != DMME_OK || !tsh) return rc;
    return launch_gn_modulate(sc, sh, tsh, tsc, P->tproj_cols, nt, P->B, o.gn_mod_C, s);
}

int run_op(const dmme_plan* P, const Op& o, const char* pk, const float* x, const int64_t* t, int nt, float* y,
           char* ws, const float* drop_masks, hipStream_t s, bool keep_ctx, const int64_t* labels = nullptr, int* status = nullptr) {
    if (o.lvl >= 0) return o.lvl_first ? run_level(P, P->lvl_runs[o.lvl], pk, ws, nt, drop_masks, s, keep_ctx) : DMME_OK;
    if (o.fused_away) return DMME_OK;
    switch (o.kind) {
        case OP_SINUS:
            return launch_time_sinusoid(t, nt, (const float*)(pk + P->params[P->freqs_param].packed_off),
                                        P->cfg.pos_dim / 2, (float*)(ws + P->ws_tsin), s, (unsigned*)(ws + P->ws_mark),
                                        keep_ctx ? kFwdMarkKeep : kFwdMarkNograd);
        case OP_LINEAR: {
            const char* w = o.lin_w >= 0 ? pk + P->params[o.lin_w].packed_off : pk + P->tproj_w_off;
            const float* b = (const float*)(o.lin_b >= 0 ? pk + P->params[o.lin_b].packed_off : pk + P->tproj_b_off);
            if (nt > 4)
                return launch_small_gemm(P->dtype, 0, (const float*)(ws + o.lin_in), o.lin_K, w, o.lin_K, nt, o.lin_N, o.lin_K, b, o.lin_silu,
                                         (float*)(ws + o.lin_out), o.lin_N, s, o.lin_pre >= 0 ? (float*)(ws + o.lin_pre) : nullptr);
            return launch_linear_wave(P->dtype, (const float*)(ws + o.lin_in), nt, o.lin_K, w, b, o.lin_N, o.lin_silu,
                                      (float*)(ws + o.lin_out), s);
        }
        case OP_LABEL: {
            float* z2 = (float*)(ws + P->ws_tz2);
            return launch_label_cond(z2, nt, (const float*)(pk + P->params[P->p_lemb].packed_off), labels, P->B, P->cfg.num_classes, P->cfg.emb_dim,
                                     (float*)(ws + P->ws_temb), nt == P->B ? z2 : nullptr, status, s);
        }
        case OP_GN:
            return run_gn(P, o, pk, ws, nt, drop_masks, s);
        case OP_CONV: {
            ConvArgs a{};
            fill_conv(P, o, pk, x, y, ws, drop_masks, nt, a, true);
            return launch_conv(conv_dt(P, o), a, s);
        }
        case OP_CAST: {
            const Tensor& ts = P->tensors[o.cast_src];
            return launch_cast_f32_to_16(P->dtype, (const float*)(ws + ts.off), (int64_t)P->B * ts.H * ts.W * ts.C, ws + P->tensors[o.cast_dst].off, s);
        }
        case OP_ATTN: {
            const Tensor& q = P->tensors[o.at_qkv];
            const int S = q.H * q.W, C = q.C / 3;
            if (o.at_proj >= 0) {
                ConvArgs a{};
                fill_conv(P, P->ops[o.at_proj], pk, x, y, ws, drop_masks, nt, a, true);
                return launch_attn_proj(P->dtype, ws + q.off, P->B, S, C, keep_ctx ? ws + P->tensors[o.at_out].off : nullptr, (float*)(ws + o.at_lse), a.w, a.bias,
                                        a.res1, a.dst, a.gn_part, a.gn_tiles, a.gn_cg, s);
            }
            if (P->x3 && attn_x3_supported(P->B, S, C, o.at_heads))
                return launch_attn_x3(ws + q.off, P->B, S, C, o.at_heads, ws + P->tensors[o.at_out].off, s);
            if (o.at_heads > 1) {
                if (attn_heads_mfma_supported(P->dtype, P->B, S, C, o.at_heads))
                    return launch_attn_heads_mfma(P->dtype, ws + q.off, P->B, S, C, o.at_heads, ws + P->tensors[o.at_out].off, (float*)(ws + o.at_lse), s);
                return launch_attn_heads(P->dtype, ws + q.off, P->B, S, C, o.at_heads, ws + P->tensors[o.at_out].off, s);
            }
            if (attn_mfma_supported(P->dtype, P->B, S, C))
                return launch_attn_mfma(P->dtype, ws + q.off, P->B, S, C, ws + P->tensors[o.at_out].off, (float*)(ws + o.at_lse), s);
            return launch_attn_generic(P->dtype, ws + q.off, P->B, S, C, ws + P->tensors[o.at_out].off, s);
        }
    }
    return DMME_OK;
}
void op_account(const dmme_plan* P, const Op& o, char* label, int cap, double* flops, double* bytes) {
    const double es = (double)dtype_size(P->dtype);
    const char* tn = P->dtype == DMME_BF16 ? "bf16" : P->dtype == DMME_F16 ? "f16" : "float";
    const double B = P->B;
    *flops = 0;
    *bytes = 0;
    if (o.lvl >= 0) {
        const LvlRun& R = P->lvl_runs[o.lvl];
        if (o.lvl_first) {
            snprintf(label, cap, "lvl_engine_kernel<%dx%d>", 1 << R.sh, 1 << R.sh);
            *flops = R.flops;
            *bytes = R.bytes;
        } else {
            snprintf(label, cap, "(level engine)");
        }
        return;
    }
    if (o.fused_away) {
        snprintf(label, cap, o.fused_away == 2 ? "(proj 1x1 conv inside its block's attention launch)" : "(residual 1x1 conv inside its block's conv2)");
        return;
    }
    switch (o.kind) {
        case OP_SINUS:
            snprintf(label, cap, "time_sinusoid_kernel");
            break;
        case OP_LABEL:
            snprintf(label, cap, "label_cond_kernel");
            *flops = B * P->cfg.emb_dim;
            *bytes = 4.0 * B * P->cfg.emb_dim * 3;
            break;
        case OP_LINEAR:
            snprintf(label, cap, "linear_wave_kernel<%s>", tn);
            *flops = 2.0 * o.lin_K * o.lin_N;
// ... 52 lines not shown
                *flops += 2.0 * B * S * C * C;
                *bytes = B * S * 5.0 * C * es + C * C * es;
            }
            break;
        }
    }
}


static int check_cfg(const dmme_unet_cfg* cfg, int B, int H, int W, int dtype) {
    DMME_REQUIRE(B > 0 && H > 0 && W > 0, DMME_ERR_INVALID, "plan_create: bad shape B=%d H=%d W=%d", B, H, W);
    DMME_REQUIRE(dtype == DMME_F32 || dtype == DMME_BF16 || dtype == DMME_BF16X3 || dtype == DMME_F16 || dtype == DMME_F16R32, DMME_ERR_INVALID,
                 "plan_create: bad dtype %d", dtype);
    DMME_REQUIRE(cfg->num_depths >= 1 && cfg->num_depths <= 8 && cfg->num_blocks >= 1, DMME_ERR_INVALID,
                 "plan_create: bad depth/blocks");
    DMME_REQUIRE(cfg->num_attention_depths >= 0 && cfg->num_attention_depths <= 8, DMME_ERR_INVALID, "bad attention_depths");
    DMME_REQUIRE(cfg->pos_dim >= 4 && cfg->pos_dim % 2 == 0, DMME_ERR_INVALID, "pos_dim must be even and >= 4");
    DMME_REQUIRE(cfg->arch == DMME_ARCH_DDPM || cfg->arch == DMME_ARCH_IDDPM || cfg->arch == DMME_ARCH_CLASSIFIER || cfg->arch == DMME_ARCH_DDPM_COND,
                 DMME_ERR_INVALID, "plan_create: unknown arch %d", cfg->arch);
    if (cfg->arch == DMME_ARCH_DDPM_COND) {
        const bool x3 = dtype == DMME_BF16X3, mix = dtype == DMME_F16R32;
        DMME_REQUIRE(!x3 && !mix, DMME_ERR_UNSUPPORTED, "plan_create: the class-conditional UNet runs in fp32, bf16 or fp16 (not %s)", x3 ? "bf16x3" : "fp16r32");
        DMME_REQUIRE(cfg->num_classes >= 1, DMME_ERR_INVALID, "plan_create: class-conditional UNet with num_classes=%d", cfg->num_classes);
    }
    if (cfg->arch == DMME_ARCH_CLASSIFIER) {
        const bool x3 = dtype == DMME_BF16X3, mix = dtype == DMME_F16R32;
        DMME_REQUIRE(!x3 && !mix, DMME_ERR_UNSUPPORTED, "plan_create: the classifier runs in fp32, bf16 or fp16 (not %s)", x3 ? "bf16x3" : "fp16r32");
        DMME_REQUIRE(cfg->num_classes >= 1, DMME_ERR_INVALID, "plan_create: classifier num_classes=%d", cfg->num_classes);
        DMME_REQUIRE(cfg->channels_per_depth[cfg->num_depths - 1] <= 1024, DMME_ERR_UNSUPPORTED, "plan_create: classifier head wider than 1024 channels");
    }
    if (cfg->arch == DMME_ARCH_IDDPM) {
        DMME_REQUIRE(cfg->num_heads >= 1, DMME_ERR_INVALID, "plan_create: num_heads must be >= 1");
    }
    for (int d = 0; d < cfg->num_depths; ++d)
        DMME_REQUIRE(cfg->channels_per_depth[d] > 0 && cfg->channels_per_depth[d] % cfg->num_groups == 0,
                     DMME_ERR_INVALID, "channels_per_depth[%d]=%d not divisible by num_groups=%d", d,
                     cfg->channels_per_depth[d], cfg->num_groups);
    return DMME_OK;
}

static int check_mix_kernels(const dmme_plan* P) {
    if (!P->mix) return DMME_OK;
    for (const Op& o : P->ops) {
        if (o.kind != OP_CONV || !(o.mix || o.route_f32)) continue;
        ConvArgs a{};
        fill_conv(P, o, (const char*)4096, (const float*)4096, (float*)4096, (char*)4096, nullptr, 1, a);
        const bool ok = !o.mix || conv_route(P->dtype, a).family == (o.mix == 3 ? CONV_THIN : o.mix == 4 ? CONV1X1_SPLIT : CONV3X3_SPLIT);
        DMME_REQUIRE(ok, DMME_ERR_UNSUPPORTED, "plan_create: precision fp16r32 has no kernel for the %dx%d conv %d+%d -> %d channels on the %dx%d level (B = %d)",
                     o.taps == 9 ? 3 : 1, o.taps == 9 ? 3 : 1, a.C1, a.C2, a.Cout, a.Hout, a.Wout, P->B);
    }
    return DMME_OK;
}

static int count_launches(const dmme_plan* P) {
    int n = 0;
    for (const Op& o : P->ops) {
        if (o.fused_away) continue;
        if (o.lvl >= 0)
            n += o.lvl_first;
        else if (o.kind == OP_GN)
            n += !(o.gn_direct || o.gn_in_consumer);
        else
            ++n;
    }
    return n;
}

#define DMME_TRY(expr)                 \
    do {                               \
        if (int rc_ = (expr)) return rc_; \
    } while (0)

static int upload_tables(dmme_plan* P) {
    DMME_CHECK_HIP(hipSetDevice(P->device));
    std::vector<PackItem> items, bitems, uitems;
    build_pack_items(P, items);
    build_pack_items_bwd(P, bitems);
    build_unpack_items(P, uitems);
    P->n_items = (int)items.size();
    P->n_items_bwd = (int)bitems.size();
    P->n_items_unpack = (int)uitems.size();
    DMME_TRY(P->items_dev.upload(items));
    DMME_TRY(P->items_bwd_dev.upload(bitems));
    DMME_TRY(P->items_unpack_dev.upload(uitems));
    DMME_TRY(P->tp_tiles_dev.upload(P->tp_tiles));
    DMME_TRY(P->col_jobs_dev.upload(P->col_jobs));
    DMME_TRY(P->bias_jobs_dev.upload(P->bias_jobs));
    std::vector<dmme_plan::WgGroup*> all_groups{&P->wg[0], &P->wg[1], &P->wg[2]};
    for (auto& B_ : P->gb)
        for (int k = 0; k < 3; ++k) all_groups.push_back(&B_.wg[k]);
    for (dmme_plan::WgGroup* G : all_groups) {
        if (G->jobs.empty()) continue;
        DMME_TRY(G->layers_dev.upload(G->layers));
        DMME_TRY(G->jobs_dev.upload(G->jobs));
    }
    DMME_TRY(P->err_host.alloc());
    for (LvlRun& R : P->lvl_runs) {
        DMME_TRY(R.ops_dev.upload(R.ops));
        if (R.raw_skipped > 0) DMME_TRY(R.ops_nograd_dev.upload(R.ops_nograd));
        DMME_TRY(R.sync_dev.zeroed(16 + R.ops.size() * 2 * (size_t)R.NG * LVL_NS));
    }
    return DMME_OK;
}

}

extern "C" {

DMME_API const char* dmme_last_error(void) { return g_err; }
DMME_API int dmme_version(void) { return 114; }
DMME_API int dmme_device_count(void) {
    int n = 0;
    if (hipGetDeviceCount(&n) != hipSuccess) return 0;
    return n;
}

DMME_API int dmme_unet_plan_create(const dmme_unet_cfg* cfg, int B, int H, int W, int dtype, int device, dmme_plan** out) {
    DMME_REQUIRE(cfg && out, DMME_ERR_INVALID, "plan_create: null argument");
    DMME_TRY(check_cfg(cfg, B, H, W, dtype));
    std::unique_ptr<dmme_plan> owned(new dmme_plan());
    dmme_plan* P = owned.get();
    P->cfg = *cfg;
    if (cfg->arch == DMME_ARCH_DDPM_COND) {
        P->cond = 1;
        P->cfg.arch = DMME_ARCH_DDPM;
    }
    P->B = B;
    P->H = H;
    P->W = W;
    P->x3 = dtype == DMME_BF16X3;
    P->mix = dtype == DMME_F16R32;
    P->dtype = P->x3 ? DMME_F32 : P->mix ? DMME_F16 : dtype;
    P->device = device;
    DMME_TRY(build_plan(P));
    DMME_TRY(check_mix_kernels(P));
    assign_levels(P);
    const bool fused_gn = !getenv("DMME_NO_FUSED_GN");
    if (fused_gn) assign_stats(P);
    if (fused_gn && !getenv("DMME_NO_GN_DIRECT")) assign_direct(P);
    if (!getenv("DMME_NO_PREACT")) assign_preact(P);
    if (fused_gn) assign_gn_in(P);
    assign_rseg(P);
    assign_attn_proj(P);
    assign_lvl_nograd(P);
    P->n_launches = count_launches(P);
    plan_backward(P);
    if (device >= 0) DMME_TRY(upload_tables(P));
    *out = owned.release();
    return DMME_OK;
}

DMME_API void dmme_unet_plan_destroy(dmme_plan* plan) { delete plan; }

DMME_API int dmme_unet_plan_num_params(const dmme_plan* plan) { return plan ? (int)plan->params.size() : 0; }

DMME_API int dmme_unet_plan_param_info(const dmme_plan* plan, int index, char* name, int name_cap, int* ndim,
                              int64_t shape[4], int64_t* ref_offset, int* is_buffer) {
    DMME_REQUIRE(plan && index >= 0 && index < (int)plan->params.size(), DMME_ERR_INVALID, "param_info: bad index %d", index);
    const Param& p = plan->params[index];
    if (name && name_cap > 0) {
        strncpy(name, p.name.c_str(), (size_t)name_cap - 1);
        name[name_cap - 1] = 0;
    }
    if (ndim) *ndim = p.ndim;
    if (shape)
        for (int i = 0; i < 4; ++i) shape[i] = p.shape[i];
    if (ref_offset) *ref_offset = p.ref_off;
    if (is_buffer) *is_buffer = p.is_buffer ? 1 : 0;
    return DMME_OK;
}

DMME_API int64_t dmme_unet_plan_ref_numel(const dmme_plan* plan) { return plan ? plan->ref_numel : 0; }
DMME_API int64_t dmme_unet_plan_packed_bytes(const dmme_plan* plan) { return plan ? plan->packed_bytes : 0; }
DMME_API int64_t dmme_unet_plan_workspace_bytes(const dmme_plan* plan) { return plan ? plan->ws_bytes : 0; }
DMME_API int64_t dmme_unet_plan_dropmask_numel(const dmme_plan* plan) { return plan ? plan->dropmask_numel : 0; }
DMME_API int dmme_unet_plan_out_channels(const dmme_plan* plan) { return plan ? plan->out_channels : 0; }
DMME_API int dmme_unet_plan_num_launches(const dmme_plan* plan) { return plan ? plan->n_launches : 0; }

DMME_API int dmme_unet_pack_params(const dmme_plan* plan, const float* ref_flat, void* packed, void* stream) {
    DMME_REQUIRE(plan && ref_flat && packed, DMME_ERR_INVALID, "pack_params: null argument");
    DMME_REQUIRE(plan->items_dev, DMME_ERR_INVALID, "pack_params: plan was created without a device");
    return launch_pack_table(plan->dtype, plan->items_dev.get(), plan->n_items, ref_flat, packed, (hipStream_t)stream);
}

static int unet_forward_impl(const dmme_plan* plan, const void* packed, const float* x, const int64_t* t, int t_len,
                      float* y, void* workspace, const float* drop_masks, void* stream, bool keep_ctx, const int64_t* labels = nullptr,
                      int* status = nullptr) {
    DMME_REQUIRE(plan && packed && x && t && y && workspace, DMME_ERR_INVALID, "unet_forward: null argument");
    DMME_REQUIRE((plan->cond != 0) == (labels != nullptr), DMME_ERR_INVALID,
                 plan->cond ? "unet_forward: a class-conditional plan (DMME_ARCH_DDPM_COND) takes labels: call dmme_unet_forward_cond / dmme_cfg_chain_step"
                            : "unet_forward_cond: the plan is not class-conditional (DMME_ARCH_DDPM_COND)");
    DMME_REQUIRE(t_len == 1 || t_len == plan->B, DMME_ERR_INVALID,
                 "unet_forward: timestep tensor of length %d does not broadcast against batch %d", t_len, plan->B);
    {
        const int rc = lvl_check(plan, "unet_forward", (hipStream_t)stream, true);
        if (rc != DMME_OK) return rc;
    }
    hipStream_t s = (hipStream_t)stream;
    const dmme_plan* P = plan;
    const char* pk = (const char*)packed;
    char* ws = (char*)workspace;
    const int nt = t_len;
    if (keep_ctx) {
        if (plan->nograd_ws == workspace) plan->nograd_ws = nullptr;
    } else {
        plan->nograd_ws = workspace;
    }
    for (int oi = 0; oi < (int)P->ops.size(); ++oi) {
        const int rc = run_op(P, P->ops[oi], pk, x, t, P->cond && oi > P->label_op ? P->B : nt, y, ws, drop_masks, s, keep_ctx, labels, status);
        if (rc != DMME_OK) return rc;
    }
    if (P->head_src >= 0) {
        const Tensor& tt = P->tensors[P->head_src];
        return launch_cls_head_fwd(P->dtype, ws + tt.off, P->B, tt.H * tt.W, tt.C, P->cfg.num_groups, (const float*)(pk + P->params[P->p_hgw].packed_off),
                                   (const float*)(pk + P->params[P->p_hgb].packed_off), (const float*)(pk + P->params[P->p_hw].packed_off),
                                   (const float*)(pk + P->params[P->p_hb].packed_off), P->out_channels, y, s);
    }
    return DMME_OK;
}
DMME_API int dmme_unet_forward(const dmme_plan* plan, const void* packed, const float* x, const int64_t* t, int t_len,
                      float* y, void* workspace, const float* drop_masks, void* stream) {
    return unet_forward_impl(plan, packed, x, t, t_len, y, workspace, drop_masks, stream, true);
}
DMME_API int dmme_unet_forward_nograd(const dmme_plan* plan, const void* packed, const float* x, const int64_t* t, int t_len,
                      float* y, void* workspace, const float* drop_masks, void* stream) {
    return unet_forward_impl(plan, packed, x, t, t_len, y, workspace, drop_masks, stream, false);
}

DMME_API int dmme_unet_forward_cond(const dmme_plan* plan, const void* packed, const float* x, const int64_t* t, int t_len, const int64_t* labels,
                                    float* y, void* workspace, const float* drop_masks, int keep_ctx, int* status, void* stream) {
    DMME_REQUIRE(labels, DMME_ERR_INVALID, "unet_forward_cond: null argument (labels)");
    return unet_forward_impl(plan, packed, x, t, t_len, y, workspace, drop_masks, stream, keep_ctx != 0, labels, status);
}

DMME_API int dmme_unet_plan_num_ops(const dmme_plan* plan) { return plan ? (int)plan->ops.size() : 0; }
// ... 477 lines not shown
}

DMME_API int dmme_conv2d_res(const dmme_conv_desc* d, const void* src1, const void* src2, const void* weight, const float* bias, const float* scale,
                             const float* shift, const float* dmask, const void* r_src1, const void* r_src2, int r_C1, int r_C2, const void* r_weight,
                             const float* r_bias, void* dst, void* stream) {
    DMME_REQUIRE(d && src1 && weight && bias && dst && r_src1 && r_weight && r_bias, DMME_ERR_INVALID, "conv2d_res: null argument");
    DMME_REQUIRE(d->dtype == DMME_BF16 || d->dtype == DMME_F16, DMME_ERR_UNSUPPORTED, "conv2d_res: 16-bit tensors only (dtype %d)", d->dtype);
    ConvArgs a{};
    a.src1 = src1; a.src2 = src2; a.w = weight; a.bias = bias; a.scale = scale; a.shift = shift; a.dmask = dmask; a.dst = dst;
    a.N = d->N; a.Hin = d->Hin; a.Win = d->Win; a.C1 = d->C1; a.C2 = src2 ? d->C2 : 0;
    a.up = d->upsample; a.stride = d->stride; a.taps = d->taps;
    a.Hout = a.Hin; a.Wout = a.Win; a.Cout = d->Cout;
    a.pro_silu = d->pro_silu; a.out_silu = d->out_silu;
    a.f16 = d->dtype == DMME_F16;
    a.stamps = g_stamps;
    a.r_src1 = r_src1; a.r_src2 = r_C2 > 0 ? r_src2 : nullptr; a.r_C1 = r_C1; a.r_C2 = r_C2 > 0 ? r_C2 : 0; a.r_w = r_weight; a.r_bias = r_bias;
    const ConvRoute r = conv_route(d->dtype, a);
    DMME_REQUIRE(a.taps == 9 && a.stride == 1 && !a.up && r.rseg, DMME_ERR_UNSUPPORTED,
                 "conv2d_res: the wave-specialised 3x3 kernel does not take this shape with a residual segment (%d+%d -> %d channels, %d+%d raw, %dx%dx%d)", a.C1, a.C2,
                 a.Cout, a.r_C1, a.r_C2, a.N, a.Hin, a.Win);
    return launch_conv(r, d->dtype, a, (hipStream_t)stream);
}

DMME_API int dmme_groupnorm_scale_shift(int dtype, const void* src1, const void* src2, int N, int HW, int C1, int C2, int groups,
                               const float* gamma, const float* beta, float eps, float* scale, float* shift,
                               float* partial_scratch, int force_generic, void* stream) {
    DMME_REQUIRE(src1 && gamma && beta && scale && shift, DMME_ERR_INVALID, "groupnorm: null argument");
    if (!src2) C2 = 0;
    DMME_REQUIRE(groups > 0 && (C1 + C2) % groups == 0, DMME_ERR_INVALID, "groupnorm: %d channels not divisible by %d groups",
                 C1 + C2, groups);
    if (!force_generic && partial_scratch && gn_fast_supported(dtype, N, HW, C1, C2, groups))
        return launch_gn_fast(dtype, src1, src2, N, HW, C1, C2, groups, gamma, beta, eps, scale, shift, nullptr,
                              partial_scratch, (hipStream_t)stream);
    return launch_gn_generic(dtype, src1, src2, N, HW, C1, C2, groups, gamma, beta, eps, scale, shift, nullptr,
                             (hipStream_t)stream);
}

DMME_API int dmme_attention(int dtype, const void* qkv, int N, int S, int C, void* out, int force_generic, void* stream) {
    DMME_REQUIRE(qkv && out && N > 0 && S > 0 && C > 0, DMME_ERR_INVALID, "attention: bad argument");
    if (dtype == DMME_BF16X3) {
        if (!force_generic && attn_x3_supported(N, S, C, 1)) return launch_attn_x3(qkv, N, S, C, 1, out, (hipStream_t)stream);
        dtype = DMME_F32;
    }
    if (!force_generic && attn_mfma_supported(dtype, N, S, C)) return launch_attn_mfma(dtype, qkv, N, S, C, out, nullptr, (hipStream_t)stream);
    return launch_attn_generic(dtype, qkv, N, S, C, out, (hipStream_t)stream);
}

DMME_API int dmme_attention_proj(int dtype, const void* qkv, int N, int S, int C, const void* w, const float* bias, const void* res, void* dst, void* ctx,
                                 float* gn_part, int gn_cg, void* stream) {
    DMME_REQUIRE(qkv && w && bias && res && dst && N > 0 && S > 0 && C > 0, DMME_ERR_INVALID, "attention_proj: bad argument");
    return launch_attn_proj(dtype, qkv, N, S, C, ctx, nullptr, w, bias, res, dst, gn_part, S / 32, gn_cg, (hipStream_t)stream, g_stamps);
}

DMME_API int dmme_attention_heads(int dtype, const void* qkv, int N, int S, int C, int heads, void* out, int force_generic, void* stream) {
    DMME_REQUIRE(qkv && out && N > 0 && S > 0 && C > 0 && heads > 0 && C % heads == 0, DMME_ERR_INVALID, "attention_heads: bad argument");
    if (dtype == DMME_BF16X3) {
        if (!force_generic && attn_x3_supported(N, S, C, heads)) return launch_attn_x3(qkv, N, S, C, heads, out, (hipStream_t)stream);
        dtype = DMME_F32;
    }
    if (!force_generic && attn_heads_mfma_supported(dtype, N, S, C, heads))
        return launch_attn_heads_mfma(dtype, qkv, N, S, C, heads, out, nullptr, (hipStream_t)stream);
    return launch_attn_heads(dtype, qkv, N, S, C, heads, out, (hipStream_t)stream);
}

DMME_API int dmme_nchw_to_nhwc(int dtype, const float* src, int N, int C, int HW, void* dst, void* stream) {
    DMME_REQUIRE(src && dst, DMME_ERR_INVALID, "nchw_to_nhwc: null argument");
    return launch_nchw_to_nhwc(dtype, src, N, C, HW, dst, (hipStream_t)stream);
}
DMME_API int dmme_nhwc_to_nchw(int dtype, const void* src, int N, int C, int HW, float* dst, void* stream) {
    DMME_REQUIRE(src && dst, DMME_ERR_INVALID, "nhwc_to_nchw: null argument");
    return launch_nhwc_to_nchw(dtype, src, N, C, HW, dst, (hipStream_t)stream);
}
DMME_API int dmme_pack_weight(int dtype, const float* src, int Cout, int Cin, int taps, void* dst, void* stream) {
    DMME_REQUIRE(src && dst, DMME_ERR_INVALID, "pack_weight: null argument");
    return launch_pack_weight(dtype, src, Cout, Cin, taps, dst, (hipStream_t)stream);
}

DMME_API int dmme_event_create(void** ev) {
    DMME_REQUIRE(ev, DMME_ERR_INVALID, "event_create: null");
    hipEvent_t e;
    DMME_CHECK_HIP(hipEventCreate(&e));
    *ev = (void*)e;
    return DMME_OK;
}
DMME_API int dmme_event_record(void* ev, void* stream) {
    DMME_CHECK_HIP(hipEventRecord((hipEvent_t)ev, (hipStream_t)stream));
    return DMME_OK;
}
DMME_API int dmme_event_elapsed_ms(void* start, void* stop, float* ms) {
    DMME_CHECK_HIP(hipEventSynchronize((hipEvent_t)stop));
    DMME_CHECK_HIP(hipEventElapsedTime(ms, (hipEvent_t)start, (hipEvent_t)stop));
    return DMME_OK;
}
DMME_API int dmme_event_destroy(void* ev) {
    DMME_CHECK_HIP(hipEventDestroy((hipEvent_t)ev));
    return DMME_OK;
}

}
```

### diffusion-models-made-easy_amd/diffusion_models/chain.py

```python

from __future__ import annotations

from typing import Optional

import torch
from torch import Tensor

from .. import _lib
from ..common import vis
from ..common.noise import philox_reserve


class ChainTables:

    def __init__(self, rows, ttab, device):
        self.coef = torch.tensor(rows, dtype=torch.float32).reshape(-1).to(device)
        self.ttab = torch.tensor(ttab, dtype=torch.int64).to(device)
        self.state = torch.zeros(8, dtype=torch.int64, device=device)

    def set(self, i: int, seed: int = 0, offset: int = 0):
        _lib.check(_lib.lib().dmme_chain_set(_lib.ptr(self.state), int(i), _lib.ptr(self.ttab), seed & 0xFFFFFFFFFFFFFFFF, int(offset), _lib.stream_ptr()), "dmme_chain_set")


def chain_draws(kind: int, rows) -> bool:
    if kind in (_lib.CHAIN_DDIM, _lib.CHAIN_DDIM_GUIDED, _lib.CHAIN_DPMPP, _lib.CHAIN_DPMPP_CFG):
        return False
    if kind in (_lib.CHAIN_GDDIM, _lib.CHAIN_GDDIM_CFG):
        return any(r[2] != 0.0 for r in rows)
    return True


def history_ordinals(count: int, vis_length: int):
    count, L = int(count), int(vis_length)
    if count < 0 or L < 1:
        raise ValueError(f"history_ordinals: count = {count} steps, vis_length = {L}")
    return sorted({count - int(count / (L - 1) * i) for i in range(L - 1, 0, -1)} | {count})


class HistoryRecorder:

    def __init__(self, n_images: int, C: int, H: int, W: int, ordinals, out_kind: int = 0, device="cuda"):
        self.ordinals = sorted({int(s) for s in ordinals})
        if n_images < 1 or not self.ordinals or self.ordinals[0] < 0:
            raise ValueError(f"HistoryRecorder: {n_images} images, ordinals {self.ordinals}")
        self.n_images, self.image = int(n_images), (int(C), int(H), int(W))
        L = self.stride = len(self.ordinals)
        if L == 1:
            self.xmaps = min(vis.history_nrow(self.n_images), self.n_images)
            self.ymaps = -(-self.n_images // self.xmaps)
        else:
            self.xmaps, self.ymaps = L, self.n_images
        self.pad = 0 if L * self.n_images == 1 else vis.PAD
        self.canvas = vis.new_canvas(*self.image, self.xmaps, self.ymaps, self.pad, out_kind, device)
        self._slot = {s: k for k, s in enumerate(self.ordinals)}
        self.recorded = 0

    def begin(self, x: Tensor, count: int) -> None:
        if tuple(x.shape[1:]) != self.image or x.shape[0] < self.n_images or x.device != self.canvas.device:
            raise ValueError(f"HistoryRecorder: built for {self.n_images} images of {self.image} on {self.canvas.device}, the chain runs on {tuple(x.shape)} on {x.device}")
        if self.ordinals[-1] > count:
            raise ValueError(f"HistoryRecorder: ordinal {self.ordinals[-1]} in a chain of {count} steps")
        self.recorded = 0

    def at(self, s: int, x: Tensor) -> None:
        k = self._slot.get(s)
        if k is not None:
            vis.grid_tile(x[: self.n_images], self.canvas, k, self.stride, self.xmaps, self.ymaps, self.pad)
            self.recorded += 1


def walk(x: Tensor, first: int, count: int, step, recorder=None, reserve=None) -> Tensor:
    if recorder is not None:
        recorder.begin(x, count)
    if reserve is not None:
        reserve()
    for s in range(count):
        if recorder is not None:
            recorder.at(s, x)
        step(s, first - s)
    if recorder is not None:
        recorder.at(count, x)
    return x


def capture(launch, check, carried=()):
    saved = [b.clone() for b in carried]

    def restore():
        for b, v in zip(carried, saved):
            b.copy_(v)

    launch()
    torch.cuda.synchronize()
    check()
    restore()
    graph, out, error = None, None, None
    try:
        graph = torch.cuda.CUDAGraph()
        with torch.cuda.graph(graph):
            out = launch()
    except RuntimeError as exc:
        graph, out, error = None, None, exc
    restore()
    return graph, out, error


class ChainRunner(ChainTables):

    def __init__(self, process, x: Tensor, use_graph: bool = True, spec=None):
        model = process.model
        if not (isinstance(x, Tensor) and x.is_cuda and x.dtype == torch.float32 and x.is_contiguous() and x.dim() == 4):
            raise ValueError("ChainRunner needs a contiguous fp32 GPU image batch")
        B, _, H, W = x.shape
        self.process, self.model, self.x = process, model, x
        self.plan = model._plan_for(B, H, W, x.device)
        self.kind, (n, rows, ttab) = spec if spec is not None else (process._chain_kind, process._chain_tables())
        self.draws = chain_draws(self.kind, rows)
        self.n_steps = n
        self.pred = getattr(process, "_pred", _lib.PRED_EPS)
        self.pred_ab = process._pred_table(x.device).clone() if self.pred != _lib.PRED_EPS else None
        super().__init__(rows, ttab, x.device)
        self.out = torch.empty((B, model.out_channels, H, W), dtype=torch.float32, device=x.device)
        self.quads = x.numel() // 4
        self.noise_numel = x.numel()
        self.use_graph = use_graph
        self.graph = None
        self.capture_error = None
        self._wkey = None

    def _set_prediction(self, plan=None):
        plan = self.plan if plan is None else plan
        _lib.check(_lib.lib().dmme_unet_plan_set_prediction(plan.h, self.pred, _lib.ptr(self.pred_ab), self.process.timesteps), "dmme_unet_plan_set_prediction")

    def _launch(self, packed):
        self._set_prediction()
        self._call(packed)
        self.plan.overwritten()

    def _call(self, packed):
        _lib.check(
            _lib.lib().dmme_chain_step(self.plan.h, _lib.ptr(packed), _lib.ptr(self.x), _lib.ptr(self.out), _lib.ptr(self.plan.workspace), self.kind,
                                       _lib.ptr(self.coef), _lib.ptr(self.ttab), _lib.ptr(self.state), _lib.stream_ptr()),
            "dmme_chain_step",
        )

    def _carried(self):
        return [self.x, self.state]

    def _weights_key(self):
        return (self.plan.packed_version, self.plan.packed.data_ptr())

    def step(self):
        model = self.model
        if model.training:
            raise RuntimeError("ChainRunner: sampling chains run in eval mode (no dropout masks inside the replayed step)")
        packed = model._packed_for(self.plan)
        wkey = self._weights_key()
        if not self.use_graph or self.capture_error is not None:
            self._launch(packed)
            return self.x
        if self.graph is None or self._wkey != wkey:
            self.graph, _, self.capture_error = capture(lambda: self._launch(packed), self.plan.check, self._carried())
            if self.graph is None:
                self._launch(packed)
                return self.x
            self._wkey = wkey
        self.plan.check()
        self.graph.replay()
        self.plan.overwritten()
        return self.x

    def run(self, first: int, count: int, recorder: Optional[HistoryRecorder] = None):

        def reserve():
            seed, off = philox_reserve(self.x.device, self.noise_numel * count) if self.draws else (0, 0)
            self.set(first, seed, off)

        walk(self.x, first, count, lambda s, i: self.step(), recorder, reserve)
        torch.cuda.current_stream(self.x.device).synchronize()
        self.plan.check()
        return self.x
```

### diffusion-models-made-easy_amd/models/ddpm.py

```python

from __future__ import annotations

import ctypes as C
import weakref
from typing import Dict, Optional, Sequence, Tuple

import torch
from torch import Tensor, nn

from .. import _lib


class _Scope(nn.Module):
    """Parameter container used to reproduce the reference's dotted state_dict keys."""


def _cfg_struct(in_channels, pos_dim, emb_dim, num_groups, dropout, channels_per_depth, num_blocks, attention_depths, arch=0, num_heads=1,
                num_classes=0):
    cfg = _lib.UNetCfg()
    cfg.arch, cfg.num_heads, cfg.num_classes = int(arch), int(num_heads), int(num_classes)
    cfg.in_channels, cfg.pos_dim, cfg.emb_dim, cfg.num_groups = in_channels, pos_dim, emb_dim, num_groups
    cfg.dropout = float(dropout)
    if not 1 <= len(channels_per_depth) <= 8 or len(attention_depths) > 8:
        raise ValueError("channels_per_depth must have 1..8 entries and attention_depths at most 8")
    cfg.num_depths = len(channels_per_depth)
    for i, c in enumerate(channels_per_depth):
        cfg.channels_per_depth[i] = int(c)
    cfg.num_blocks = num_blocks
    cfg.num_attention_depths = len(attention_depths)
    for i, d in enumerate(attention_depths):
        cfg.attention_depths[i] = int(d)
    return cfg


class _Plan:

    def __init__(self, cfg, B, H, W, dtype, device_index):
        self.lib = _lib.lib()
        h = C.c_void_p()
        _lib.check(self.lib.dmme_unet_plan_create(C.byref(cfg), B, H, W, dtype, device_index, C.byref(h)), "dmme_unet_plan_create")
        self.h = h
        self.B, self.H, self.W, self.dtype = B, H, W, dtype
        self.workspace = None
        self.packed = None
        self.packed_version = None
        self.fwd_gen = 0

    def overwritten(self):
        self.fwd_gen += 1

    def param_table(self):
        n = self.lib.dmme_unet_plan_num_params(self.h)
        out = []
        name = C.create_string_buffer(256)
        ndim, off, isb = C.c_int(), C.c_int64(), C.c_int()
        shape = (C.c_int64 * 4)()
        for i in range(n):
            _lib.check(self.lib.dmme_unet_plan_param_info(self.h, i, name, 256, C.byref(ndim), shape, C.byref(off), C.byref(isb)), "param_info")
            out.append((name.value.decode(), tuple(int(shape[k]) for k in range(ndim.value)), int(off.value), bool(isb.value)))
        return out

    def check(self):
        _lib.check(self.lib.dmme_unet_plan_check(self.h), "dmme_unet_plan_check")

    def __del__(self):
        try:
            if getattr(self, "h", None):
                self.lib.dmme_unet_plan_destroy(self.h)
                self.h = None
        except Exception:
            pass


class UNet(nn.Module):

    def __init__(
        self,
        in_channels: int = 3,
        pos_dim: int = 128,
        emb_dim: int = 512,
        num_groups: int = 32,
        dropout: float = 0.1,
        channels_per_depth: Sequence[int] = (128, 256, 256, 256),
        num_blocks: int = 2,
        attention_depths: Sequence[int] = (2,),
        precision: str = "fp32",
        _arch: int = 0,
        _num_heads: int = 1,
        _num_classes: int = 0,
    ):
        super().__init__()
        self.in_channels = in_channels
        self.out_channels = 2 * in_channels if _arch == 1 else in_channels
        self.dropout = float(dropout)
        self.precision = precision
        self._dtype = _lib.dtype_code(precision)
        self._cfg = _cfg_struct(in_channels, pos_dim, emb_dim, num_groups, dropout, tuple(channels_per_depth), num_blocks, tuple(attention_depths), _arch, _num_heads,
                                _num_classes)
# ... 109 lines not shown
        with torch.no_grad():
            new = fn(flat)
        if not (isinstance(new, Tensor) and new.dtype == torch.float32 and new.numel() == flat.numel()):
            out = super()._apply(fn, *a, **kw)
            self._ensure_flat()
            return out
        if new is not flat and new.data_ptr() != flat.data_ptr():
            new = new.detach().contiguous()
            grad = self._flat_grad
            with torch.no_grad():
                new_grad = fn(grad).detach().contiguous() if grad is not None else None
            for mod, leaf, off, n, shape, is_buf in self._views:
                v = new[off : off + n].view(shape)
                if is_buf:
                    mod._buffers[leaf] = v
                else:
                    p = mod._parameters[leaf]
                    old_grad = p.grad
                    p.data = v
                    if old_grad is not None:
                        if new_grad is not None and grad is not None and old_grad.data_ptr() == grad.data_ptr() + 4 * off:
                            p.grad = new_grad[off : off + n].view(shape)
                        else:
                            with torch.no_grad():
                                p.grad = fn(old_grad)
            self._flat = new
            self._flat_grad = new_grad
            for pl in self._plans.values():
                pl.packed_version = None
            self._ensure_flat()
        return self

    def flat_parameters(self) -> Tensor:
        return self._ensure_flat()

    def set_precision(self, precision: str):
        self.precision = precision
        self._dtype = _lib.dtype_code(precision)
        return self

    def _plan_for(self, B: int, H: int, W: int, device: torch.device) -> _Plan:
        key = (B, H, W, self._dtype, device.index)
        plan = self._plans.get(key)
        if plan is None:
            plan = _Plan(self._cfg, B, H, W, self._dtype, device.index if device.index is not None else torch.cuda.current_device())
            lib = plan.lib
            plan.workspace = torch.empty(int(lib.dmme_unet_plan_workspace_bytes(plan.h)), dtype=torch.uint8, device=device)
            plan.packed = torch.empty(int(lib.dmme_unet_plan_packed_bytes(plan.h)), dtype=torch.uint8, device=device)
            plan.dropmask_numel = int(lib.dmme_unet_plan_dropmask_numel(plan.h))
            plan.masks = None
            self._plans[key] = plan
        return plan

    def _packed_for(self, plan: _Plan) -> Tensor:
        flat = self._ensure_flat()
        ver = self._weights_key(flat)
        if plan.packed_version != ver:
            _lib.check(plan.lib.dmme_unet_pack_params(plan.h, _lib.ptr(flat), _lib.ptr(plan.packed), _lib.stream_ptr()), "dmme_unet_pack_params")
            plan.packed_version = ver
        return plan.packed

    def inject_dropout_masks(self, masks: Optional[Tensor]):
        self._injected_masks = masks

    def forward(self, x: Tensor, c: Tensor) -> Tensor:
        _lib.require_gpu()
        if not x.is_cuda:
            raise _lib.DmmeError("UNet.forward needs a GPU tensor: the HIP denoiser has no CPU fallback")
        if x.dim() != 4 or x.shape[1] != self.in_channels:
            raise ValueError(f"expected input of shape (N, {self.in_channels}, H, W), got {tuple(x.shape)}")
        B, _, H, W = x.shape
        if c.numel() not in (1, B):
            raise RuntimeError(f"timestep tensor of {c.numel()} elements does not broadcast against batch {B}")
        if torch.is_grad_enabled() and (x.requires_grad or any(p.requires_grad for p in self.parameters())):
            from ..autograd import unet_apply

            return unet_apply(self, x, c)
        return self._forward_impl(x, c)

    def amp_state(self, device=None) -> Optional[Tensor]:
        if self._amp is None or self._dtype != _lib.F16:
            return None
        dev = torch.device(device) if device is not None else self.flat_parameters().device
        if dev.type == "cuda" and dev.index is None:
            dev = torch.device("cuda", torch.cuda.current_device())
        st = self._amp_state
        if st is None:
            st = torch.zeros(8, dtype=torch.float32, device=dev)
            if dev.type == "cuda":
                _lib.check(_lib.lib().dmme_amp_init(_lib.ptr(st), float(self._amp["init_scale"]), _lib.stream_ptr()), "dmme_amp_init")
            else:
                st[0] = float(self._amp["init_scale"])
            self._amp_state = st
        elif st.device != dev:
            st = st.to(dev)
            self._amp_state = st
        return st

    def mark_params_updated(self):
        self._param_epoch += 1

    def flat_grad(self) -> Tensor:
        flat = self._ensure_flat()
        g = self._flat_grad
        fresh = g is None or g.device != flat.device or g.numel() != flat.numel()
        if fresh:
            g = torch.zeros_like(flat)
            self._flat_grad = g
        rebind = fresh
        if not rebind:
            for mod, leaf, off, n, shape, is_buf in self._views:
                if not is_buf and mod._parameters[leaf].grad is None:
# ... 67 lines not shown
        if cb is not None:
            _lib.check(
                lib.dmme_unet_backward_buckets(plan.h, _lib.ptr(packed), _lib.ptr(plan.packed_bwd), _lib.ptr(xin), _lib.ptr(t), int(t.numel()), _lib.ptr(d),
                                               _lib.ptr(plan.workspace), _lib.ptr(plan.bws), _lib.ptr(masks), _lib.ptr(g), _lib.ptr(dx), _lib.stream_ptr(), cb, None),
                "dmme_unet_backward_buckets",
            )
            return
        _lib.check(
            lib.dmme_unet_backward(plan.h, _lib.ptr(packed), _lib.ptr(plan.packed_bwd), _lib.ptr(xin), _lib.ptr(t), int(t.numel()), _lib.ptr(d),
                                   _lib.ptr(plan.workspace), _lib.ptr(plan.bws), _lib.ptr(masks), _lib.ptr(g), _lib.ptr(dx), _lib.stream_ptr()),
            "dmme_unet_backward",
        )

    def _launch_backward_input(self, plan: _Plan, packed: Tensor, xin: Tensor, t: Tensor, d: Tensor, masks: Optional[Tensor], dx: Tensor):
        _lib.check(
            plan.lib.dmme_unet_backward_input(plan.h, _lib.ptr(packed), _lib.ptr(plan.packed_bwd), _lib.ptr(xin), _lib.ptr(t), int(t.numel()), _lib.ptr(d),
                                              _lib.ptr(plan.workspace), _lib.ptr(plan.bws), _lib.ptr(masks), _lib.ptr(dx), _lib.stream_ptr()),
            "dmme_unet_backward_input",
        )

    def _bwd_buffers(self, plan: _Plan) -> Tensor:
        lib = plan.lib
        dev = plan.workspace.device
        if getattr(plan, "bws", None) is None:
            plan.bws = torch.empty(int(lib.dmme_unet_plan_bwd_workspace_bytes(plan.h)), dtype=torch.uint8, device=dev)
            plan.packed_bwd = torch.empty(int(lib.dmme_unet_plan_packed_bwd_bytes(plan.h)), dtype=torch.uint8, device=dev)
            plan.packed_bwd_version = None
        flat = self._ensure_flat()
        packed = self._packed_for(plan)
        ver = self._weights_key(flat)
        if plan.packed_bwd_version != ver:
            _lib.check(lib.dmme_unet_pack_params_bwd(plan.h, _lib.ptr(flat), _lib.ptr(plan.packed_bwd), _lib.stream_ptr()), "dmme_unet_pack_params_bwd")
            plan.packed_bwd_version = ver
        return packed

    def _backward_input_impl(self, saved, dy: Tensor) -> Tensor:
        plan, xin, t, masks, gen = saved
        if gen != plan.fwd_gen:
            raise RuntimeError("input gradient: another forward of the same shape overwrote the saved activations")
        packed = self._bwd_buffers(plan)
        d = dy.detach().to(torch.float32).contiguous()
        dx = torch.empty_like(xin)
        self._launch_backward_input(plan, packed, xin, t, d, masks, dx)
        return dx

    def _out_shape(self, B: int, H: int, W: int) -> Tuple[int, ...]:
        return (B, self.out_channels, H, W)

    def _forward_impl(self, x: Tensor, c: Tensor, want_ctx: bool = False):
        if getattr(self, "_exchange_in_flight", False):
            raise _lib.DmmeError("UNet.forward while a gradient exchange of this model is in flight: call reducer.finish() first")
        B, _, H, W = x.shape
        plan = self._plan_for(B, H, W, x.device)
        packed = self._packed_for(plan)
        xin = x.detach().to(torch.float32).contiguous()
        if c.is_floating_point() and bool((c != c.round()).any()):
            raise NotImplementedError("fractional timesteps are not supported by the HIP path (integer t only)")
        t = c.detach().reshape(-1).to(device=x.device, dtype=torch.int64).contiguous()
        y = torch.empty(self._out_shape(B, H, W), dtype=torch.float32, device=x.device)
        masks = None
        if self.training and self.dropout > 0:
            if self._injected_masks is not None:
                masks = self._injected_masks.to(device=x.device, dtype=torch.float32).contiguous()
                if masks.numel() != plan.dropmask_numel:
                    raise ValueError(f"injected dropout masks have {masks.numel()} elements, plan needs {plan.dropmask_numel}")
            else:
                if plan.masks is None:
                    plan.masks = torch.empty(plan.dropmask_numel, dtype=torch.float32, device=x.device)
                masks = plan.masks
                from ..common.noise import philox_reserve

                self._mask_calls += 1
                seed, off = philox_reserve(x.device, plan.dropmask_numel)
                _lib.check(plan.lib.dmme_dropout_masks(plan.h, seed ^ 0x5DEECE66D, off, _lib.ptr(masks), _lib.stream_ptr()), "dmme_dropout_masks")
        self._launch_forward(plan, packed, xin, t, y, masks, want_ctx)
        self._last_plan = plan
        plan.overwritten()
        if want_ctx:
            return y, (plan, xin, t, masks, plan.fwd_gen)
        return y

    def graphed_forward(self, x_static: Tensor, t_static: Tensor) -> Tensor:
        if self.training or getattr(self, "_graph_disabled", False):
            return self._forward_impl(x_static, t_static)
        flat = self._ensure_flat()
        key = (x_static.data_ptr(), t_static.data_ptr(), tuple(x_static.shape), self._dtype) + self._weights_key(flat)
        g = getattr(self, "_graph", None)
        if g is None or g[0] != key:
            from ..diffusion_models.chain import capture

            with torch.no_grad():
                graph, y, error = capture(lambda: self._forward_impl(x_static, t_static), lambda: self._last_plan.check())
                if error is not None:
                    if isinstance(error, _lib.DmmeError):
                        raise error
                    self._graph_disabled, self._graph_error, self._graph = True, error, None
                    return self._forward_impl(x_static, t_static)
            g = (key, graph, y, self._last_plan)
            self._graph = g
        plan = g[3]
        plan.check()
        g[1].replay()
        plan.overwritten()
        return g[2]

    def check_engine(self):
        torch.cuda.synchronize()
# ... 31 lines not shown
```

### include/dmme_hip.h

```cpp
#ifndef DMME_HIP_H
#define DMME_HIP_H

#include <stddef.h>
#include <stdint.h>

#if defined(DMME_BUILD)
#define DMME_API __attribute__((visibility("default")))
#else
#define DMME_API
#endif

#ifdef __cplusplus
extern "C" {
#endif

typedef enum {
    DMME_OK = 0,
    DMME_ERR_INVALID = -1,
    DMME_ERR_UNSUPPORTED = -2,
    DMME_ERR_HIP = -3,
    DMME_ERR_NOMEM = -4
} dmme_status;

typedef enum { DMME_F32 = 0, DMME_BF16 = 1, DMME_BF16X3 = 2, DMME_F16 = 3, DMME_F16R32 = 4 } dmme_dtype;

typedef enum {
    DMME_ARCH_DDPM = 0,
    DMME_ARCH_IDDPM = 1,
    DMME_ARCH_CLASSIFIER = 2,
    DMME_ARCH_DDPM_COND = 3
} dmme_unet_arch;

typedef struct {
    int in_channels;
    int pos_dim;
    int emb_dim;
    int num_groups;
    float dropout;
    int num_depths;
    int channels_per_depth[8];
    int num_blocks;
    int num_attention_depths;
    int attention_depths[8];
    int arch;
    int num_heads;
    int num_classes;
} dmme_unet_cfg;

typedef struct dmme_plan dmme_plan;

DMME_API const char* dmme_last_error(void);
DMME_API int dmme_version(void);
DMME_API int dmme_device_count(void);

DMME_API int dmme_unet_plan_create(const dmme_unet_cfg* cfg, int B, int H, int W, int dtype, int device, dmme_plan** out);
DMME_API void dmme_unet_plan_destroy(dmme_plan* plan);

DMME_API int dmme_unet_plan_num_params(const dmme_plan* plan);
DMME_API int dmme_unet_plan_param_info(const dmme_plan* plan, int index, char* name, int name_cap, int* ndim,
                              int64_t shape[4], int64_t* ref_offset, int* is_buffer);
DMME_API int64_t dmme_unet_plan_ref_numel(const dmme_plan* plan);
DMME_API int64_t dmme_unet_plan_packed_bytes(const dmme_plan* plan);
DMME_API int64_t dmme_unet_plan_workspace_bytes(const dmme_plan* plan);
DMME_API int64_t dmme_unet_plan_dropmask_numel(const dmme_plan* plan);
DMME_API int dmme_unet_plan_out_channels(const dmme_plan* plan);
DMME_API int dmme_unet_plan_num_launches(const dmme_plan* plan);

DMME_API int dmme_unet_pack_params(const dmme_plan* plan, const float* ref_flat, void* packed, void* stream);

DMME_API int dmme_unet_forward(const dmme_plan* plan, const void* packed, const float* x, const int64_t* t, int t_len,
                      float* y, void* workspace, const float* drop_masks, void* stream);
DMME_API int dmme_unet_forward_nograd(const dmme_plan* plan, const void* packed, const float* x, const int64_t* t, int t_len,
                      float* y, void* workspace, const float* drop_masks, void* stream);

DMME_API int dmme_unet_forward_cond(const dmme_plan* plan, const void* packed, const float* x, const int64_t* t, int t_len, const int64_t* labels,
                                    float* y, void* workspace, const float* drop_masks, int keep_ctx, int* status, void* stream);

DMME_API int dmme_unet_plan_num_ops(const dmme_plan* plan);
DMME_API int dmme_unet_plan_level_info(const dmme_plan* plan, char* buf, int cap);
DMME_API int dmme_unet_plan_check(const dmme_plan* plan);
DMME_API int dmme_unet_plan_op_info(const dmme_plan* plan, int index, char* label, int label_cap, double* flops,
                           double* bytes);
DMME_API int dmme_unet_forward_profiled(const dmme_plan* plan, const void* packed, const float* x, const int64_t* t,
                               int t_len, float* y, void* workspace, const float* drop_masks, void* stream,
                               float* op_ms);

DMME_API int64_t dmme_unet_plan_packed_bwd_bytes(const dmme_plan* plan);
DMME_API int64_t dmme_unet_plan_bwd_workspace_bytes(const dmme_plan* plan);
DMME_API int dmme_unet_pack_params_bwd(const dmme_plan* plan, const float* ref_flat, void* packed_bwd, void* stream);
DMME_API int dmme_unet_backward(const dmme_plan* plan, const void* packed, const void* packed_bwd, const float* x,
                       const int64_t* t, int t_len, const float* d_y, void* workspace, void* bwd_workspace,
                       const float* drop_masks, float* grad_flat, float* d_x, void* stream);
typedef void (*dmme_bucket_fn)(void* user, int bucket, int64_t offset, int64_t numel);
DMME_API int dmme_unet_backward_buckets(const dmme_plan* plan, const void* packed, const void* packed_bwd, const float* x,
                               const int64_t* t, int t_len, const float* d_y, void* workspace, void* bwd_workspace,
                               const float* drop_masks, float* grad_flat, float* d_x, void* stream, dmme_bucket_fn ready, void* user);
DMME_API int dmme_unet_backward_input(const dmme_plan* plan, const void* packed, const void* packed_bwd, const float* x, const int64_t* t,
                                      int t_len, const float* d_y, void* workspace, void* bwd_workspace, const float* drop_masks, float* d_x,
                                      void* stream);
DMME_API int dmme_unet_plan_grad_buckets(const dmme_plan* plan, int64_t* offsets, int64_t* numels, int* bucket_of, int cap);
DMME_API int dmme_unet_backward_cond(const dmme_plan* plan, const void* packed, const void* packed_bwd, const float* x, const int64_t* t, int t_len,
                                     const int64_t* labels, const float* d_y, void* workspace, void* bwd_workspace, const float* drop_masks,
                                     float* grad_flat, float* d_x, void* stream, dmme_bucket_fn ready, void* user);
DMME_API int dmme_unet_backward_input_cond(const dmme_plan* plan, const void* packed, const void* packed_bwd, const float* x, const int64_t* t,
                                           int t_len, const int64_t* labels, const float* d_y, void* workspace, void* bwd_workspace,
                                           const float* drop_masks, float* d_x, void* stream);
DMME_API int dmme_unet_plan_bwd_summary(const dmme_plan* plan, char* buf, int cap);
DMME_API int dmme_debug_level_stamps(void* buf, int run, int workgroup);
DMME_API int dmme_debug_mfma_valu(int mode, int iters, int blocks, void* sink, void* stream);
DMME_API int dmme_debug_issue_probe(int kind, int n_inner, int iters, int flags, int blocks, void* sink, const void* src, void* stream);
DMME_API int dmme_debug_l2_stream(const void* buf, int64_t bytes, int iters, int mode, int depth, int blocks, void* sink, void* stream);
DMME_API int dmme_grad_norm(const float* grad, int64_t numel, float* norm_out, float* scratch, void* stream);
DMME_API int dmme_adam_step(float* param, const float* grad, float* exp_avg, float* exp_avg_sq, float* ema, int64_t numel,
                            float lr, float beta1, float beta2, float eps, int step, const float* grad_norm, float max_norm,
                            float ema_decay, float grad_scale, void* stream);
DMME_API int dmme_amp_init(float* amp_state, float init_scale, void* stream);
DMME_API int dmme_amp_scale(float* grad, int64_t numel, const float* amp_state, void* stream);
DMME_API int dmme_adam_step_amp(float* param, const float* grad, float* exp_avg, float* exp_avg_sq, float* ema, int64_t numel, float lr, float beta1,
                                float beta2, float eps, const float* grad_norm, float max_grad_norm, float ema_decay, float grad_scale,
                                float* amp_state, float growth_factor, float backoff_factor, int growth_interval, void* stream);
DMME_API int dmme_grad_pack_bf16(const float* grad, int64_t numel, void* dst_bf16, int64_t numel_padded, void* stream);
// ... 98 lines not shown


DMME_API int dmme_iddpm_step(float* x, const float* model_out, const float* z, float inv_sqrt_alpha, float eps_coef, float log_beta,
                    float log_beta_tilde, int add_noise, int B, int64_t chw, void* stream);

DMME_API int dmme_iddpm_loss(const float* model_out, const float* x_t, const float* x_0, const float* target, const int64_t* t,
                    const float* coef, int B, int64_t chw, float w_simple, float w_vlb, float* loss, float* d_out,
                    float grad_scale, float* scratch, void* stream);


DMME_API int dmme_iddpm_loss_rows(const float* model_out, const float* x_t, const float* x_0, const float* target, const int64_t* t,
                                  const float* coef, int T, const float* weight, int B, int64_t chw, float w_simple, float w_vlb, float* loss,
                                  float* rows, float* d_out, float grad_scale, int* status, float* scratch, void* stream);

DMME_API int dmme_iddpm_prior_rows(const float* x_0, int B, int64_t chw, float alpha_bar_T, float* prior, void* stream);

DMME_API int dmme_tsampler_draw(const float* hist, const int* count, int T, int H, float uniform_prob, uint64_t philox_seed,
                                uint64_t philox_offset, int B, int64_t* t, float* weight, float* p, void* stream);

DMME_API int dmme_tsampler_update(float* hist, int* count, int T, int H, const int64_t* t, const float* L, int B, int* status, void* stream);

typedef struct {
    int dtype;
    int N, Hin, Win;
    int C1, C2;
    int upsample;
    int stride;
    int taps;
    int Cout;
    int pro_silu;
    int out_silu;
    int nt;
    int tproj_ld;
    int in_nchw;
    int out_nchw;
    int force_generic;
} dmme_conv_desc;

DMME_API int dmme_conv2d(const dmme_conv_desc* d, const void* src1, const void* src2, const void* weight,
                const float* bias, const float* scale, const float* shift, const float* dmask,
                const float* tproj, const void* res1, const void* res2, int R1, void* dst, void* stream);

DMME_API int dmme_conv2d_res(const dmme_conv_desc* d, const void* src1, const void* src2, const void* weight, const float* bias,
                const float* scale, const float* shift, const float* dmask, const void* r_src1, const void* r_src2, int r_C1,
                int r_C2, const void* r_weight, const float* r_bias, void* dst, void* stream);

DMME_API int dmme_groupnorm_scale_shift(int dtype, const void* src1, const void* src2, int N, int HW, int C1, int C2,
                               int groups, const float* gamma, const float* beta, float eps, float* scale,
                               float* shift, float* partial_scratch, int force_generic, void* stream);

DMME_API int dmme_attention(int dtype, const void* qkv, int N, int S, int C, void* out, int force_generic, void* stream);
DMME_API int dmme_attention_proj(int dtype, const void* qkv, int N, int S, int C, const void* w, const float* bias, const void* res,
                                 void* dst, void* ctx, float* gn_part, int gn_cg, void* stream);

DMME_API int dmme_attention_heads(int dtype, const void* qkv, int N, int S, int C, int heads, void* out, int force_generic, void* stream);

DMME_API int dmme_nchw_to_nhwc(int dtype, const float* src, int N, int C, int HW, void* dst, void* stream);
DMME_API int dmme_nhwc_to_nchw(int dtype, const void* src, int N, int C, int HW, float* dst, void* stream);
DMME_API int dmme_pack_weight(int dtype, const float* src, int Cout, int Cin, int taps, void* dst, void* stream);

DMME_API int dmme_debug_set_stamps(void* buf);

DMME_API int dmme_event_create(void** ev);
DMME_API int dmme_event_record(void* ev, void* stream);
DMME_API int dmme_event_elapsed_ms(void* start, void* stop, float* ms);
DMME_API int dmme_event_destroy(void* ev);

#ifdef __cplusplus
}
#endif
#endif
```

Before: 453.1 denoising steps/s (one step = UNet forward + DDPM update on a batch of 128), summed over GPUs.

## Fold attention QKV/proj weights algebraically into a single fused attention-block kernel

For inference, the attention block's QK^T product is refactored algebraically. A precomputed matrix M (derived from Wq, Wk and biases) is applied to the normalized input, so keys and values can be read straight from the normalized activations instead of a materialized qkv tensor. The value and output projections are folded together (wpv, bias2), and the groupnorm scale/shift is applied inside the kernel. This drops the separate qkv projection conv and its memory traffic for sampling, and the folded weights are packed once per weight version. It adds weight-preprocessing complexity and numerical differences from folding in bf16. Separately, Python GC is disabled during graph capture.

```diff
diff --git a/diffusion-models-made-easy_amd/_lib.py b/diffusion-models-made-easy_amd/_lib.py
--- a/diffusion-models-made-easy_amd/_lib.py
+++ b/diffusion-models-made-easy_amd/_lib.py
@@ -83,7 +83,10 @@
     "dmme_unet_plan_dropmask_numel": (_i64, [_vp]),
     "dmme_unet_plan_out_channels": (_i, [_vp]),
     "dmme_unet_plan_num_launches": (_i, [_vp]),
+    "dmme_unet_plan_num_launches_nograd": (_i, [_vp]),
+    "dmme_unet_plan_num_folded": (_i, [_vp]),
     "dmme_unet_pack_params": (_i, [_vp, _vp, _vp, _vp]),
+    "dmme_unet_pack_folded": (_i, [_vp, _vp, _vp]),
     "dmme_unet_forward": (_i, [_vp, _vp, _vp, _vp, _i, _vp, _vp, _vp, _vp]),
     "dmme_unet_forward_nograd": (_i, [_vp, _vp, _vp, _vp, _i, _vp, _vp, _vp, _vp]),
     "dmme_unet_forward_cond": (_i, [_vp, _vp, _vp, _vp, _i, _vp, _vp, _vp, _vp, _i, _vp, _vp]),
@@ -159,6 +162,8 @@
     "dmme_groupnorm_scale_shift": (_i, [_i, _vp, _vp, _i, _i, _i, _i, _i, _vp, _vp, _f, _vp, _vp, _vp, _i, _vp]),
     "dmme_attention": (_i, [_i, _vp, _i, _i, _i, _vp, _i, _vp]),
     "dmme_attention_proj": (_i, [_i, _vp, _i, _i, _i, _vp, _vp, _vp, _vp, _vp, _vp, _i, _vp]),
+    "dmme_attention_fold": (_i, [_i, _i, _vp, _vp, _vp, _vp, _vp, _vp, _vp, _vp, _vp]),
+    "dmme_attention_block": (_i, [_i, _vp, _i, _i, _i, _vp, _i, _i, _i, _vp, _vp, _f, _vp, _vp, _vp, _vp, _vp, _vp, _vp, _vp, _vp, _i, _vp]),
     "dmme_attention_heads": (_i, [_i, _vp, _i, _i, _i, _i, _vp, _i, _vp]),
     "dmme_nchw_to_nhwc": (_i, [_i, _vp, _i, _i, _i, _vp, _vp]),
     "dmme_nhwc_to_nchw": (_i, [_i, _vp, _i, _i, _i, _vp, _vp]),
diff --git a/diffusion-models-made-easy_amd/csrc/attn_mfma.hip b/diffusion-models-made-easy_amd/csrc/attn_mfma.hip
--- a/diffusion-models-made-easy_amd/csrc/attn_mfma.hip
+++ b/diffusion-models-made-easy_amd/csrc/attn_mfma.hip
@@ -1,4 +1,6 @@
 #include <stdlib.h>
+
+#include <type_traits>
 
 #include "conv_common.h"
 
@@ -237,6 +239,15 @@
     long long* stamps;
     int dbg;
 };
+struct AttnFold {
+    const void* M;
+    const float* c;
+    const float* scale;
+    const float* shift;
+    GnIn gni;
+    int has_gni;
+};
+struct AttnNoFold {};
 __device__ __forceinline__ float at_keep_f32(float x) {
     asm volatile("" : "+v"(x));
     return x;
@@ -247,15 +258,20 @@
     permlane32_swap(a, b);
     return a + b;
 }
-template <int C, typename T = bf16, bool PROJ = false>
-__global__ void __launch_bounds__(256) attn_full_kernel(const T* __restrict__ qkv, AttnGeom g, T* __restrict__ out, float* __restrict__ lse, int xcd_order, AttnProj pj) {
+template <int C, typename T = bf16, bool PROJ = false, bool FOLD = false>
+__global__ void __launch_bounds__(256) attn_full_kernel(const T* __restrict__ qkv, AttnGeom g, T* __restrict__ out, float* __restrict__ lse, int xcd_order, AttnProj pj,
+                                                        typename std::conditional<FOLD, AttnFold, AttnNoFold>::type fd) {
     typedef T tx8 __attribute__((ext_vector_type(8)));
+    static_assert(!FOLD || PROJ, "attn_full: the folded form carries the proj phase");
     constexpr int S = 256, NKT = S / AT_KT, KSTEPS = C / 16, CT = C / 32;
-    constexpr int NTOT = 2 * NKT + (PROJ ? CT : 0);
+    constexpr int T0 = FOLD ? CT : 0;
+    constexpr int NTOT = T0 + 2 * NKT + (PROJ ? CT : 0);
+    constexpr int KOFF = FOLD ? 0 : C, VOFF = FOLD ? 0 : 2 * C;
     constexpr int ROWB = C * 2, TILEB = AT_KT * ROWB;
     constexpr int DPT = TILEB / (256 * 16);
     constexpr bool PAIR = AT_PAIR_STEPS != 0;
     constexpr int NSLOT_BYTES = 8 * TILEB;
+    constexpr int MAINB = PROJ && 4 * 32 * (C * 4 + 16) > NSLOT_BYTES ? 4 * 32 * (C * 4 + 16) : NSLOT_BYTES;
     constexpr int NSLOT = 8, AHEAD = PAIR ? 6 : 7;
     static_assert(!PAIR || (NTOT % 2 == 0 && NKT % 2 == 0), "pair steps: even tile counts per phase");
     static_assert(DPT >= 1 && DPT * 256 * 16 == TILEB, "attn_full: tile does not split over the DMA lanes");
@@ -274,7 +290,7 @@
     const int q_row = qb * 128 + wave * 32 + r;
     const unsigned lds0 = (unsigned)__builtin_amdgcn_readfirstlane((int)(unsigned)(size_t)(__attribute__((address_space(3))) char*)lds);
 #ifdef AT_STAMPS
-    long long* st_lds = reinterpret_cast<long long*>(lds + (PROJ ? (4 * 32 * (C * 4 + 16) > NSLOT_BYTES ? 4 * 32 * (C * 4 + 16) : NSLOT_BYTES) : NSLOT_BYTES));
+    long long* st_lds = reinterpret_cast<long long*>(lds + MAINB);
     int st_i = 0;
     const bool stamping = PROJ && pj.stamps && blockIdx.x == 0 && tid == 0;
 #define AF_STAMP() { if (PROJ && stamping && st_i < 120) st_lds[st_i++] = (long long)clock64(); }
@@ -299,6 +315,15 @@
     }
     auto dma_tile = [&](int t) __attribute__((always_inline)) {
         const unsigned dst = lds0 + (unsigned)((t % NSLOT) * TILEB);
+        if constexpr (FOLD) {
+            if (t < T0) {
+                const char* src = (const char*)fd.M + (size_t)t * TILEB;
+#pragma unroll
+                for (int i = 0; i < DPT; ++i) glds16_hidden_s(src, woff[i], dst + (unsigned)((wave + 4 * i) * 1024));
+                return;
+            }
+        }
+        t -= T0;
         if (PROJ && t >= 2 * NKT) {
             const char* src = (const char*)pj.w + (size_t)(t - 2 * NKT) * TILEB;
 #pragma unroll
@@ -307,7 +332,7 @@
         }
         const bool isv = t >= NKT;
         const T* kvb = (PROJ && (pj.dbg & 8)) ? qkv : base;
-        const char* src = (const char*)(kvb + (int64_t)((isv ? t - NKT : t) * AT_KT) * ld + (isv ? 2 * C : C));
+        const char* src = (const char*)(kvb + (int64_t)((isv ? t - NKT : t) * AT_KT) * ld + (isv ? VOFF : KOFF));
 #pragma unroll
         for (int i = 0; i < DPT; ++i) glds16_hidden_s(src, isv ? voff[i] : koff[i], dst + (unsigned)((wave + 4 * i) * 1024));
     };
@@ -316,6 +341,43 @@
     uint4 qf[KSTEPS];
 #pragma unroll
     for (int ks = 0; ks < KSTEPS; ++ks) qf[ks] = *reinterpret_cast<const uint4*>(base + (int64_t)q_row * ld + ks * 16 + h * 8);
+    typedef __attribute__((address_space(3))) char lc;
+    typedef __attribute__((address_space(3))) f32x4 lf4;
+#ifdef AT_STAMPS
+    const lc* rows3 = (const lc*)(lds + MAINB + 1024);
+#else
+    const lc* rows3 = (const lc*)(lds + MAINB);
+#endif
+    if constexpr (FOLD) {
+        if (tid < C) {
+            float sc, sh;
+            if (fd.has_gni) {
+                gn_in_scale_shift_g(fd.gni, const_cast<float*>(fd.scale), const_cast<float*>(fd.shift), n, tid, C, qb == 0 && fd.scale != nullptr, sc, sh);
+            } else {
+                sc = fd.scale[(int64_t)n * C + tid];
+                sh = fd.shift[(int64_t)n * C + tid];
+            }
+            typedef __attribute__((address_space(3))) float lf1;
+            lf1* w3 = (lf1*)rows3;
+            w3[tid] = sc;
+            w3[C + tid] = sh;
+            w3[2 * C + tid] = fd.c[tid];
+        }
+        wait_lgkm_all();
+        asm volatile("s_barrier" ::: "memory");
+#pragma unroll
+        for (int ks = 0; ks < KSTEPS; ++ks) {
+            const int ch = ks * 16 + h * 8;
+            tx8 x = __builtin_bit_cast(tx8, qf[ks]);
+#pragma unroll
+            for (int e = 0; e < 8; e += 4) {
+                const f32x4 a4 = *(const lf4*)(rows3 + (ch + e) * 4), b4 = *(const lf4*)(rows3 + (C + ch + e) * 4);
+#pragma unroll
+                for (int j = 0; j < 4; ++j) x[e + j] = (T)fmaf((float)x[e + j], a4[j], b4[j]);
+            }
+            qf[ks] = __builtin_bit_cast(uint4, x);
+        }
+    }
     unsigned kb[4];
     {
         const int x = h ^ (r & 7);
@@ -327,7 +389,6 @@
 #pragma unroll
     for (int par = 0; par < 2; ++par)
         vb[par] = lds0 + (unsigned)((4 * h + tr_q) * ROWB + ((((par ^ (tr_q >> 1)) << 2) | ((tr_g1 ^ (tr_q & 1)) << 1) | (tr_p >> 1)) << 4) + ((tr_p & 1) << 3));
-    typedef __attribute__((address_space(3))) char lc;
     typedef unsigned u32x4_af __attribute__((ext_vector_type(4)));
     typedef __attribute__((address_space(3))) u32x4_af lu4;
 
@@ -377,13 +438,48 @@
                 }                                                                                                                  \
             }                                                                                                                      \
             __builtin_amdgcn_sched_barrier(0);                                                                                     \
-            if (!(PROJ && (t) >= 2 * NKT && (pj.dbg & 4)))                                                                         \
+            if (!(PROJ && (t) >= T0 + 2 * NKT && (pj.dbg & 4)))                                                                         \
             _Pragma("unroll") for (int u = 0; u < FG; ++u) at_mma<T>(__builtin_bit_cast(tx8, kf[cur][u]), __builtin_bit_cast(tx8, BF[g0 + u]), ACC); \
             __builtin_amdgcn_sched_barrier(0);                                                                                     \
         }                                                                                                                          \
         AF_STAMP()                                                                                                                 \
     }
-#define AF_K_TILE(t) AF_A_TILE(t, qf, st[t])
+#define AF_ACC_TO_B(DST, VAL)                                                                                                      \
+    _Pragma("unroll") for (int ct = 0; ct < CT; ++ct) _Pragma("unroll") for (int s2 = 0; s2 < 2; ++s2) {                            \
+        typedef T tx2 __attribute__((ext_vector_type(2)));                                                                         \
+        float w4[4];                                                                                                               \
+        _Pragma("unroll") for (int p2 = 0; p2 < 4; ++p2) {                   \
+            const int j = (2 * s2 + (p2 >> 1)) * 4 + (p2 & 1) * 2;                                                                 \
+            tx2 v;                                                                                                                 \
+            v[0] = (T)VAL(ct, j);                                                                                                  \
+            v[1] = (T)VAL(ct, j + 1);                                                                                              \
+            w4[p2] = __builtin_bit_cast(float, v);                                                                                 \
+        }                                                                                                                          \
+        permlane32_swap(w4[0], w4[2]);                                                                                             \
+        permlane32_swap(w4[1], w4[3]);                                                                                             \
+        DST[2 * ct + s2] = make_uint4(__builtin_bit_cast(unsigned, w4[0]), __builtin_bit_cast(unsigned, w4[1]), __builtin_bit_cast(unsigned, w4[2]), \
+                                      __builtin_bit_cast(unsigned, w4[3]));                                                        \
+    }
+    auto row_val = [&](int row, int ct, int j) __attribute__((always_inline)) -> float {
+        const f32x4 v = *(const lf4*)(rows3 + (row * C + 32 * ct + 8 * (j >> 2) + 4 * h) * 4);
+        return v[j & 3];
+    };
+    if constexpr (FOLD) {
+        f32x16 yt[CT];
+#pragma unroll
+        for (int t = 0; t < CT; ++t)
+#pragma unroll
+            for (int j = 0; j < 16; ++j) yt[t][j] = 0.f;
+#define AF_M_TILE(t) AF_A_TILE(t, qf, yt[t])
+        AF_M_TILE(0) AF_M_TILE(1) AF_M_TILE(2) AF_M_TILE(3)
+        if constexpr (CT > 4) { AF_M_TILE(4) AF_M_TILE(5) AF_M_TILE(6) AF_M_TILE(7) }
+#undef AF_M_TILE
+#define AF_YVAL(ct, j) ((yt[ct][j] + row_val(2, ct, j)) * row_val(0, ct, j))
+        AF_ACC_TO_B(qf, AF_YVAL)
+#undef AF_YVAL
+        AF_STAMP()
+    }
+#define AF_K_TILE(t) AF_A_TILE(T0 + (t), qf, st[t])
     AF_K_TILE(0) AF_K_TILE(1) AF_K_TILE(2) AF_K_TILE(3) AF_K_TILE(4) AF_K_TILE(5) AF_K_TILE(6) AF_K_TILE(7)
 #undef AF_K_TILE
     const float c1 = 1.4426950408889634f * g.scale;
@@ -401,8 +497,9 @@
 #pragma unroll
         for (int j = 0; j < 16; ++j) {
             const float p = __builtin_amdgcn_exp2f(fmaf(st[t][j], c1, -m));
-            l += p;
             pf[t][j >> 3][j & 7] = (T)p;
+            if constexpr (FOLD) l += (float)pf[t][j >> 3][j & 7];
+            else l += p;
         }
     const float ltot = l + __shfl_xor(l, 32, 64);
     AF_STAMP()
@@ -420,8 +517,8 @@
     }
 #define AF_V_TILE(t)                                                                                                               \
     {                                                                                                                              \
-        AF_STEP_SYNC(NKT + (t));                                                                                                   \
-        constexpr unsigned so = (unsigned)(((NKT + (t)) % NSLOT) * TILEB);                                                         \
+        AF_STEP_SYNC(T0 + NKT + (t));                                                                                              \
+        constexpr unsigned so = (unsigned)(((T0 + NKT + (t)) % NSLOT) * TILEB);                                                    \
         constexpr int VG = 2;                                                                                                      \
         s16x4 vlo[2][VG][2], vhi[2][VG][2];                                                                                        \
         AF_VREAD(0, vlo[0], vhi[0])                                                                                                \
@@ -461,32 +558,16 @@
         }
     } else {
         uint4 of[KSTEPS];
-#pragma unroll
-        for (int ct = 0; ct < CT; ++ct)
-#pragma unroll
-            for (int s2 = 0; s2 < 2; ++s2) {
-                typedef T tx2 __attribute__((ext_vector_type(2)));
-                float w4[4];
-#pragma unroll
-                for (int p2 = 0; p2 < 4; ++p2) {
-                    const int j = (2 * s2 + (p2 >> 1)) * 4 + (p2 & 1) * 2;
-                    tx2 v;
-                    v[0] = (T)at_keep_f32(o[ct][j] * inv);
-                    v[1] = (T)at_keep_f32(o[ct][j + 1] * inv);
-                    w4[p2] = __builtin_bit_cast(float, v);
-                }
-                permlane32_swap(w4[0], w4[2]);
-                permlane32_swap(w4[1], w4[3]);
-                of[2 * ct + s2] = make_uint4(__builtin_bit_cast(unsigned, w4[0]), __builtin_bit_cast(unsigned, w4[1]), __builtin_bit_cast(unsigned, w4[2]),
-                                             __builtin_bit_cast(unsigned, w4[3]));
-            }
+#define AF_OVAL(ct, j) (FOLD ? fmaf(o[ct][j] * inv, row_val(0, ct, j), row_val(1, ct, j)) : at_keep_f32(o[ct][j] * inv))
+        AF_ACC_TO_B(of, AF_OVAL)
+#undef AF_OVAL
         AF_STAMP()
         f32x16 ot[CT];
 #pragma unroll
         for (int t = 0; t < CT; ++t)
 #pragma unroll
             for (int j = 0; j < 16; ++j) ot[t][j] = 0.f;
-#define AF_W_TILE(t) AF_A_TILE(2 * NKT + (t), of, ot[t])
+#define AF_W_TILE(t) AF_A_TILE(T0 + 2 * NKT + (t), of, ot[t])
         AF_W_TILE(0) AF_W_TILE(1) AF_W_TILE(2) AF_W_TILE(3)
         if constexpr (CT > 4) { AF_W_TILE(4) AF_W_TILE(5) AF_W_TILE(6) AF_W_TILE(7) }
 #undef AF_W_TILE
@@ -596,6 +677,7 @@
 #undef AF_STAMP
 #undef AF_A_TILE
 #undef AF_STEP_SYNC
+#undef AF_ACC_TO_B
 }
 
 template <int C, typename T = bf16>
@@ -758,22 +840,24 @@
     return DMME_OK;
 }
 
-template <int D, typename T, bool PROJ = false>
-static int launch_attn_full_t(const T* qkv, const AttnGeom& g, T* out, float* lse, hipStream_t s, const AttnProj& pj = AttnProj{}) {
+template <int D, typename T, bool PROJ = false, bool FOLD = false>
+static int launch_attn_full_t(const T* qkv, const AttnGeom& g, T* out, float* lse, hipStream_t s, const AttnProj& pj = AttnProj{},
+                              const typename std::conditional<FOLD, AttnFold, AttnNoFold>::type& fd = {}) {
     const int rows = g.N * g.heads;
     const size_t ring = (size_t)8 * AT_KT * D * 2, stage = (size_t)4 * 32 * (D * 4 + 16);
+    const size_t rows3 = FOLD ? (size_t)3 * D * 4 : 0;
 #ifdef AT_STAMPS
-    const size_t lds = (PROJ && stage > ring ? stage : ring) + 1024;
+    const size_t lds = (PROJ && stage > ring ? stage : ring) + 1024 + rows3;
 #else
-    const size_t lds = PROJ && stage > ring ? stage : ring;
+    const size_t lds = (PROJ && stage > ring ? stage : ring) + rows3;
 #endif
     static bool attr_done = false;
     if (!attr_done) {
-        DMME_CHECK_HIP(hipFuncSetAttribute(reinterpret_cast<const void*>(attn_full_kernel<D, T, PROJ>), hipFuncAttributeMaxDynamicSharedMemorySize, 160 * 1024));
+        DMME_CHECK_HIP(hipFuncSetAttribute(reinterpret_cast<const void*>(attn_full_kernel<D, T, PROJ, FOLD>), hipFuncAttributeMaxDynamicSharedMemorySize, 160 * 1024));
         attr_done = true;
     }
     const int xcd_order = ((!debug_route("no_xcd_order") && rows % 8 == 0) ? 1 : 0) | ((debug_route("attn_sleep", -1) >= 0 ? debug_route("attn_sleep", -1) : rows * 2 >= 256 ? 2 : 0) << 1);
-    hipLaunchKernelGGL((attn_full_kernel<D, T, PROJ>), dim3((unsigned)(rows * 2)), dim3(256), lds, s, qkv, g, out, lse, xcd_order, pj);
+    hipLaunchKernelGGL((attn_full_kernel<D, T, PROJ, FOLD>), dim3((unsigned)(rows * 2)), dim3(256), lds, s, qkv, g, out, lse, xcd_order, pj, fd);
     DMME_CHECK_LAUNCH();
     return DMME_OK;
 }
@@ -856,6 +940,34 @@
     if (dtype == DMME_F16)
         return C == 256 ? launch_attn_full_t<256, f16, true>((const f16*)qkv, g, (f16*)ctx, lse, s, pj) : launch_attn_full_t<128, f16, true>((const f16*)qkv, g, (f16*)ctx, lse, s, pj);
     return C == 256 ? launch_attn_full_t<256, bf16, true>((const bf16*)qkv, g, (bf16*)ctx, lse, s, pj) : launch_attn_full_t<128, bf16, true>((const bf16*)qkv, g, (bf16*)ctx, lse, s, pj);
+}
+bool attn_fold_shape_ok(int dtype, int N, int S, int C, int gn_cg, int gn_tiles) {
+    if (!is16(dtype) || S != 256 || (C != 128 && C != 256) || N < 1) return false;
+    return gn_tiles == 0 || ((gn_cg == 4 || gn_cg == 8) && C % gn_cg == 0 && gn_tiles == S / 32);
+}
+int launch_attn_fold(int dtype, const void* x, int N, int S, int C, const GnIn* gni, const float* scale, const float* shift, const void* M, const float* c,
+                     const void* wpv, const float* bias2, const void* res, void* dst, float* gn_part, int gn_tiles, int gn_cg, hipStream_t s, long long* stamps) {
+    DMME_REQUIRE(attn_fold_shape_ok(dtype, N, S, C, gn_part ? gn_cg : 0, gn_part ? gn_tiles : 0) && x && M && c && wpv && bias2 && res && dst && (gni || (scale && shift)),
+                 DMME_ERR_UNSUPPORTED, "attn_fold: unsupported shape N=%d S=%d C=%d (statistics tiles %d, %d channels per group) or a null operand", N, S, C, gn_tiles, gn_cg);
+    if (gni) {
+        const int fg = gni->C1 / gni->groups, nf = fg > 0 ? (C / gni->groups) / fg : 0;
+        DMME_REQUIRE(gni->p1 && !gni->p2 && gni->C1 == C && gni->groups > 0 && C % gni->groups == 0 && (nf == 1 || nf == 2 || nf == 4) && gni->t1 * nf <= 32 && !gni->t_scale,
+                     DMME_ERR_UNSUPPORTED, "attn_fold: the norm's partials (%d tiles, %d channels, %d groups) are not a single unconditioned source of at most 32", gni->t1, gni->C1, gni->groups);
+    }
+    AttnGeom g{S, C, C, 1, N, 1.0f};
+    const AttnProj pj{wpv, bias2, res, dst, gn_part, gn_tiles, gn_cg, stamps, 0};
+    AttnFold fd{};
+    fd.M = M;
+    fd.c = c;
+    fd.scale = scale;
+    fd.shift = shift;
+    if (gni) {
+        fd.gni = *gni;
+        fd.has_gni = 1;
+    }
+    if (dtype == DMME_F16)
+        return C == 256 ? launch_attn_full_t<256, f16, true, true>((const f16*)x, g, nullptr, nullptr, s, pj, fd) : launch_attn_full_t<128, f16, true, true>((const f16*)x, g, nullptr, nullptr, s, pj, fd);
+    return C == 256 ? launch_attn_full_t<256, bf16, true, true>((const bf16*)x, g, nullptr, nullptr, s, pj, fd) : launch_attn_full_t<128, bf16, true, true>((const bf16*)x, g, nullptr, nullptr, s, pj, fd);
 }
 
 template <int C, int NW, typename T>
diff --git a/diffusion-models-made-easy_amd/csrc/common.h b/diffusion-models-made-easy_amd/csrc/common.h
--- a/diffusion-models-made-easy_amd/csrc/common.h
+++ b/diffusion-models-made-easy_amd/csrc/common.h
@@ -307,6 +307,16 @@
 bool attn_proj_fusable(int dtype, int N, int S, int C, int gn_cg, int gn_tiles);
 int launch_attn_proj(int dtype, const void* qkv, int N, int S, int C, void* ctx, float* lse, const void* w, const float* bias, const void* res, void* dst,
                      float* gn_part, int gn_tiles, int gn_cg, hipStream_t s, long long* stamps = nullptr);
+struct AttnFoldJob {
+    int64_t wq, bq, wp, bp;
+    int64_t M, c, wpv, bias2;
+    int32_t C, pad;
+};
+bool attn_fold_shape_ok(int dtype, int N, int S, int C, int gn_cg, int gn_tiles);
+int launch_attn_fold(int dtype, const void* x, int N, int S, int C, const GnIn* gni, const float* scale, const float* shift, const void* M, const float* c,
+                     const void* wpv, const float* bias2, const void* res, void* dst, float* gn_part, int gn_tiles, int gn_cg, hipStream_t s,
+                     long long* stamps = nullptr);
+int launch_attn_fold_weights(int dtype, const AttnFoldJob* jobs_dev, int n_jobs, int maxC, void* packed, hipStream_t s, const AttnFoldJob* one = nullptr);
 bool attn_heads_mfma_supported(int dtype, int N, int S, int C, int heads);
 int launch_attn_heads_mfma(int dtype, const void* qkv, int N, int S, int C, int heads, void* out, float* lse, hipStream_t s);
 int launch_attn_heads_bwd_mfma(int dtype, const void* qkv, const void* O, const void* dO, const float* lse, int N, int S, int C, int heads, void* P,
diff --git a/diffusion-models-made-easy_amd/csrc/kernels_generic.hip b/diffusion-models-made-easy_amd/csrc/kernels_generic.hip
--- a/diffusion-models-made-easy_amd/csrc/kernels_generic.hip
+++ b/diffusion-models-made-easy_amd/csrc/kernels_generic.hip
@@ -841,6 +841,50 @@
     return DMME_OK;
 }
 
+template <typename T>
+__global__ void __launch_bounds__(256) attn_fold_weights_kernel(const AttnFoldJob* __restrict__ jobs, AttnFoldJob one, char* __restrict__ packed) {
+    const AttnFoldJob jb = jobs ? jobs[blockIdx.x] : one;
+    const int C = jb.C, i = blockIdx.y, j = threadIdx.x;
+    if (i >= C) return;
+    const T* wq = (const T*)(packed + jb.wq);
+    const T* wk = wq + (int64_t)C * C;
+    const T* wv = wk + (int64_t)C * C;
+    const T* wp = (const T*)(packed + jb.wp);
+    const float* bq = (const float*)(packed + jb.bq);
+    const float* bv = bq + 2 * C;
+    const float s = 1.0f / sqrtf((float)C);
+    if (j < C) {
+        float m = 0.f, pv = 0.f;
+        for (int o = 0; o < C; ++o) {
+            m = fmaf((float)wk[(int64_t)o * C + i], (float)wq[(int64_t)o * C + j], m);
+            pv = fmaf((float)wp[(int64_t)i * C + o], (float)wv[(int64_t)o * C + j], pv);
+        }
+        ((T*)(packed + jb.M))[(int64_t)i * C + j] = from_f<T>(m * s);
+        ((T*)(packed + jb.wpv))[(int64_t)i * C + j] = from_f<T>(pv);
+    }
+    if (j == 0) {
+        float c = 0.f, b2 = 0.f;
+        for (int o = 0; o < C; ++o) {
+            c = fmaf((float)wk[(int64_t)o * C + i], bq[o], c);
+            b2 = fmaf((float)wp[(int64_t)i * C + o], bv[o], b2);
+        }
+        ((float*)(packed + jb.c))[i] = c * s;
+        ((float*)(packed + jb.bias2))[i] = b2 + ((const float*)(packed + jb.bp))[i];
+    }
+}
+int launch_attn_fold_weights(int dtype, const AttnFoldJob* jobs_dev, int n_jobs, int maxC, void* packed, hipStream_t s, const AttnFoldJob* one) {
+    if (n_jobs == 0) return DMME_OK;
+    DMME_REQUIRE((jobs_dev != nullptr) != (one != nullptr) && (!one || n_jobs == 1), DMME_ERR_INVALID, "attn_fold_weights: a device table, or one job by value");
+    const AttnFoldJob j1 = one ? *one : AttnFoldJob{};
+    DMME_REQUIRE(is16(dtype) && maxC >= 1 && maxC <= 256, DMME_ERR_UNSUPPORTED, "attn_fold_weights: 16-bit plans, blocks of at most 256 channels (got %d)", maxC);
+    if (dtype == DMME_F16)
+        hipLaunchKernelGGL(attn_fold_weights_kernel<f16>, dim3((unsigned)n_jobs, (unsigned)maxC), dim3(256), 0, s, jobs_dev, j1, (char*)packed);
+    else
+        hipLaunchKernelGGL(attn_fold_weights_kernel<bf16>, dim3((unsigned)n_jobs, (unsigned)maxC), dim3(256), 0, s, jobs_dev, j1, (char*)packed);
+    DMME_CHECK_LAUNCH();
+    return DMME_OK;
+}
+
 template <int DEPTH>
 __global__ void __launch_bounds__(256) l2_stream_kernel(const uint4* __restrict__ buf, int nvec, int iters, unsigned* __restrict__ sink) {
     unsigned acc = 0;
diff --git a/diffusion-models-made-easy_amd/csrc/plan.h b/diffusion-models-made-easy_amd/csrc/plan.h
--- a/diffusion-models-made-easy_amd/csrc/plan.h
+++ b/diffusion-models-made-easy_amd/csrc/plan.h
@@ -120,6 +120,9 @@
     int at_qkv = -1, at_out = -1, at_heads = 1;
     int64_t at_lse = 0;
     int at_proj = -1;
+    int at_fold_qkv = -1;
+    int folded_into = -1;
+    int64_t fold_M = -1, fold_c = -1, fold_wpv = -1, fold_b2 = -1;
     int mix = 0, route_f32 = 0;
     int mix2 = 0;
     int cast_src = -1, cast_dst = -1;
@@ -208,6 +211,10 @@
     int lvl_max_wg = LVL_MAX_WG;
     PinnedWord err_host;
     mutable const void* nograd_ws = nullptr;
+    std::vector<AttnFoldJob> fold_jobs;
+    DevTable<AttnFoldJob> fold_jobs_dev;
+    int fold_maxC = 0, n_launches_nograd = 0;
+    mutable const void* fold_packed = nullptr;
     int pred = DMME_PRED_EPS, pred_T = 0;
     const float* pred_ab = nullptr;
 };
@@ -225,6 +232,7 @@
 void assign_rseg(dmme_plan* P);
 int run_level(const dmme_plan* P, const LvlRun& R, const char* pk, char* ws, int nt, const float* drop_masks, hipStream_t s, bool keep_ctx = true);
 void assign_lvl_nograd(dmme_plan* P);
+void assign_attn_fold(dmme_plan* P);
 int lvl_check(const dmme_plan* P, const char* where, hipStream_t stream = nullptr, bool have_stream = false);
 void build_unpack_items(const dmme_plan* P, std::vector<PackItem>& items);
 void plan_backward(dmme_plan* P);
diff --git a/diffusion-models-made-easy_amd/csrc/plan.hip b/diffusion-models-made-easy_amd/csrc/plan.hip
--- a/diffusion-models-made-easy_amd/csrc/plan.hip
+++ b/diffusion-models-made-easy_amd/csrc/plan.hip
@@ -940,6 +940,63 @@
     }
 }
 
+void assign_attn_fold(dmme_plan* P) {
+    if (getenv("DMME_NO_ATTN_FOLD") || debug_route("no_attn_fold") || !is16(P->dtype) || P->x3 || P->mix) return;
+    int64_t cur = P->packed_bytes;
+    const int64_t es = (int64_t)dtype_size(P->dtype);
+    for (int ai = 1; ai < (int)P->ops.size(); ++ai) {
+        Op& at = P->ops[ai];
+        if (at.kind != OP_ATTN || at.at_proj < 0 || at.at_heads != 1 || at.lvl >= 0) continue;
+        Op& qc = P->ops[ai - 1];
+        const Op& pr = P->ops[at.at_proj];
+        if (qc.kind != OP_CONV || qc.dst != at.at_qkv || qc.taps != 1 || qc.src1 < 0 || qc.src2 >= 0 || qc.gn < 0 || qc.pro_silu || qc.out_silu || qc.dmask_off >= 0 ||
+            qc.tproj_col >= 0 || qc.res1 >= 0 || qc.res2 >= 0 || qc.up || qc.stride != 1 || qc.gd_n > 0 || qc.mix || qc.route_f32 || qc.fused_away || qc.rseg >= 0 ||
+            qc.use_act || qc.lvl >= 0 || pr.res1 != qc.src1)
+            continue;
+        const Op& gn = P->ops[qc.gn];
+        const Tensor& tx = P->tensors[qc.src1];
+        const int C = tx.C, groups = P->cfg.num_groups;
+        if (gn.kind != OP_GN || gn.gn_src1 != qc.src1 || gn.gn_src2 >= 0 || gn.gn_mod_col >= 0 || gn.gn_act >= 0 || tx.f32 ||
+            (gn.gn_in_consumer && (tx.stats_off < 0 || tx.stats_tiles > 32)) || P->tensors[at.at_qkv].C != 3 * C || P->params[qc.w].pack_code >= 0 || P->params[pr.w].pack_code >= 0)
+            continue;
+        bool only_here = true;
+        for (int oi = 0; oi < (int)P->ops.size() && only_here; ++oi) {
+            const Op& o = P->ops[oi];
+            if (oi == ai) continue;
+            if (o.kind == OP_CONV && (o.src1 == at.at_qkv || o.src2 == at.at_qkv || o.res1 == at.at_qkv || o.res2 == at.at_qkv)) only_here = false;
+            if (o.kind == OP_GN && (o.gn_src1 == at.at_qkv || o.gn_src2 == at.at_qkv)) only_here = false;
+            if (o.kind == OP_ATTN && o.at_qkv == at.at_qkv) only_here = false;
+            if (o.kind == OP_CAST && o.cast_src == at.at_qkv) only_here = false;
+        }
+        const Tensor& td = P->tensors[pr.dst];
+        const bool stats = td.stats_off >= 0;
+        if (!only_here || !attn_fold_shape_ok(P->dtype, P->B, tx.H * tx.W, C, stats ? C / groups : 0, stats ? td.stats_tiles : 0)) continue;
+        at.at_fold_qkv = ai - 1;
+        qc.folded_into = ai;
+        at.fold_M = cur;
+        cur = align_up(cur + (int64_t)C * C * es, 256);
+        at.fold_wpv = cur;
+        cur = align_up(cur + (int64_t)C * C * es, 256);
+        at.fold_c = cur;
+        cur = align_up(cur + (int64_t)C * 4, 256);
+        at.fold_b2 = cur;
+        cur = align_up(cur + (int64_t)C * 4, 256);
+        AttnFoldJob jb{};
+        jb.wq = P->params[qc.w].packed_off;
+        jb.bq = P->params[qc.b].packed_off;
+        jb.wp = P->params[pr.w].packed_off;
+        jb.bp = P->params[pr.b].packed_off;
+        jb.M = at.fold_M;
+        jb.c = at.fold_c;
+        jb.wpv = at.fold_wpv;
+        jb.bias2 = at.fold_b2;
+        jb.C = C;
+        P->fold_jobs.push_back(jb);
+        if (C > P->fold_maxC) P->fold_maxC = C;
+    }
+    P->packed_bytes = cur;
+}
+
 int run_gn(const dmme_plan* P, const Op& o, const char* pk, char* ws, int nt, const float* drop_masks, hipStream_t s) {
     if (o.gn_direct || o.gn_in_consumer) return DMME_OK;
     const float* tsh = o.gn_mod_col >= 0 ? (const float*)(ws + P->ws_tproj) + o.gn_mod_col : nullptr;
@@ -985,6 +1042,8 @@
            char* ws, const float* drop_masks, hipStream_t s, bool keep_ctx, const int64_t* labels = nullptr, int* status = nullptr) {
     if (o.lvl >= 0) return o.lvl_first ? run_level(P, P->lvl_runs[o.lvl], pk, ws, nt, drop_masks, s, keep_ctx) : DMME_OK;
     if (o.fused_away) return DMME_OK;
+    const bool fold = !keep_ctx && P->fold_packed == (const void*)pk;
+    if (fold && o.kind == OP_CONV && o.folded_into >= 0) return DMME_OK;
     switch (o.kind) {
         case OP_SINUS:
             return launch_time_sinusoid(t, nt, (const float*)(pk + P->params[P->freqs_param].packed_off),
@@ -1018,6 +1077,13 @@
         case OP_ATTN: {
             const Tensor& q = P->tensors[o.at_qkv];
             const int S = q.H * q.W, C = q.C / 3;
+            if (fold && o.at_fold_qkv >= 0) {
+                ConvArgs a{}, qa{};
+                fill_conv(P, P->ops[o.at_proj], pk, x, y, ws, drop_masks, nt, a, true);
+                fill_conv(P, P->ops[o.at_fold_qkv], pk, x, y, ws, drop_masks, nt, qa, true);
+                return launch_attn_fold(P->dtype, qa.src1, P->B, S, C, qa.has_gni ? &qa.gni : nullptr, qa.scale, qa.shift, pk + o.fold_M, (const float*)(pk + o.fold_c), pk + o.fold_wpv,
+                                        (const float*)(pk + o.fold_b2), a.res1, a.dst, a.gn_part, a.gn_tiles, a.gn_cg, s);
+            }
             if (o.at_proj >= 0) {
                 ConvArgs a{};
                 fill_conv(P, P->ops[o.at_proj], pk, x, y, ws, drop_masks, nt, a, true);
@@ -1176,10 +1242,10 @@
     return DMME_OK;
 }
 
-static int count_launches(const dmme_plan* P) {
+static int count_launches(const dmme_plan* P, bool nograd = false) {
     int n = 0;
     for (const Op& o : P->ops) {
-        if (o.fused_away) continue;
+        if (o.fused_away || (nograd && o.folded_into >= 0)) continue;
         if (o.lvl >= 0)
             n += o.lvl_first;
         else if (o.kind == OP_GN)
@@ -1210,6 +1276,7 @@
     DMME_TRY(P->tp_tiles_dev.upload(P->tp_tiles));
     DMME_TRY(P->col_jobs_dev.upload(P->col_jobs));
     DMME_TRY(P->bias_jobs_dev.upload(P->bias_jobs));
+    if (!P->fold_jobs.empty()) DMME_TRY(P->fold_jobs_dev.upload(P->fold_jobs));
     std::vector<dmme_plan::WgGroup*> all_groups{&P->wg[0], &P->wg[1], &P->wg[2]};
     for (auto& B_ : P->gb)
         for (int k = 0; k < 3; ++k) all_groups.push_back(&B_.wg[k]);
@@ -1232,7 +1299,7 @@
 extern "C" {
 
 DMME_API const char* dmme_last_error(void) { return g_err; }
-DMME_API int dmme_version(void) { return 114; }
+DMME_API int dmme_version(void) { return 115; }
 DMME_API int dmme_device_count(void) {
     int n = 0;
     if (hipGetDeviceCount(&n) != hipSuccess) return 0;
@@ -1267,7 +1334,9 @@
     assign_rseg(P);
     assign_attn_proj(P);
     assign_lvl_nograd(P);
+    assign_attn_fold(P);
     P->n_launches = count_launches(P);
+    P->n_launches_nograd = count_launches(P, true);
     plan_backward(P);
     if (device >= 0) DMME_TRY(upload_tables(P));
     *out = owned.release();
@@ -1300,11 +1369,23 @@
 DMME_API int64_t dmme_unet_plan_dropmask_numel(const dmme_plan* plan) { return plan ? plan->dropmask_numel : 0; }
 DMME_API int dmme_unet_plan_out_channels(const dmme_plan* plan) { return plan ? plan->out_channels : 0; }
 DMME_API int dmme_unet_plan_num_launches(const dmme_plan* plan) { return plan ? plan->n_launches : 0; }
+DMME_API int dmme_unet_plan_num_launches_nograd(const dmme_plan* plan) { return plan ? plan->n_launches_nograd : 0; }
+DMME_API int dmme_unet_plan_num_folded(const dmme_plan* plan) { return plan ? (int)plan->fold_jobs.size() : 0; }
 
 DMME_API int dmme_unet_pack_params(const dmme_plan* plan, const float* ref_flat, void* packed, void* stream) {
     DMME_REQUIRE(plan && ref_flat && packed, DMME_ERR_INVALID, "pack_params: null argument");
     DMME_REQUIRE(plan->items_dev, DMME_ERR_INVALID, "pack_params: plan was created without a device");
+    if (plan->fold_packed == packed) plan->fold_packed = nullptr;
     return launch_pack_table(plan->dtype, plan->items_dev.get(), plan->n_items, ref_flat, packed, (hipStream_t)stream);
+}
+
+DMME_API int dmme_unet_pack_folded(const dmme_plan* plan, void* packed, void* stream) {
+    DMME_REQUIRE(plan && packed, DMME_ERR_INVALID, "pack_folded: null argument");
+    DMME_REQUIRE(plan->items_dev, DMME_ERR_INVALID, "pack_folded: plan was created without a device");
+    if (plan->fold_jobs.empty()) return DMME_OK;
+    const int rc = launch_attn_fold_weights(plan->dtype, plan->fold_jobs_dev.get(), (int)plan->fold_jobs.size(), plan->fold_maxC, packed, (hipStream_t)stream);
+    if (rc == DMME_OK) plan->fold_packed = packed;
+    return rc;
 }
 
 static int unet_forward_impl(const dmme_plan* plan, const void* packed, const float* x, const int64_t* t, int t_len,
@@ -1888,6 +1969,40 @@
     return launch_attn_proj(dtype, qkv, N, S, C, ctx, nullptr, w, bias, res, dst, gn_part, S / 32, gn_cg, (hipStream_t)stream, g_stamps);
 }
 
+DMME_API int dmme_attention_fold(int dtype, int C, const void* wqkv, const float* bqkv, const void* wp, const float* bp, void* M, float* c, void* wpv, float* bias2,
+                                 void* stream) {
+    DMME_REQUIRE(wqkv && bqkv && wp && bp && M && c && wpv && bias2 && C > 0, DMME_ERR_INVALID, "attention_fold: bad argument");
+    AttnFoldJob jb{};
+    jb.wq = (int64_t)(intptr_t)wqkv;
+    jb.bq = (int64_t)(intptr_t)bqkv;
+    jb.wp = (int64_t)(intptr_t)wp;
+    jb.bp = (int64_t)(intptr_t)bp;
+    jb.M = (int64_t)(intptr_t)M;
+    jb.c = (int64_t)(intptr_t)c;
+    jb.wpv = (int64_t)(intptr_t)wpv;
+    jb.bias2 = (int64_t)(intptr_t)bias2;
+    jb.C = C;
+    return launch_attn_fold_weights(dtype, nullptr, 1, C, nullptr, (hipStream_t)stream, &jb);
+}
+DMME_API int dmme_attention_block(int dtype, const void* x, int N, int S, int C, const float* parts, int part_tiles, int part_cnt, int groups, const float* gamma,
+                                  const float* beta, float eps, float* scale, float* shift, const void* M, const float* c, const void* wpv, const float* bias2,
+                                  const void* res, void* dst, float* gn_part, int gn_cg, void* stream) {
+    DMME_REQUIRE(x && M && c && wpv && bias2 && res && dst && N > 0 && S > 0 && C > 0, DMME_ERR_INVALID, "attention_block: bad argument");
+    GnIn gni{};
+    if (parts) {
+        DMME_REQUIRE(gamma && beta && groups > 0 && part_tiles > 0 && part_cnt > 0, DMME_ERR_INVALID, "attention_block: partials without gamma / beta / geometry");
+        gni.p1 = parts;
+        gni.t1 = part_tiles;
+        gni.cnt1 = part_cnt;
+        gni.C1 = C;
+        gni.groups = groups;
+        gni.gamma = gamma;
+        gni.beta = beta;
+        gni.eps = eps;
+    }
+    return launch_attn_fold(dtype, x, N, S, C, parts ? &gni : nullptr, scale, shift, M, c, wpv, bias2, res, dst, gn_part, S / 32, gn_cg, (hipStream_t)stream, g_stamps);
+}
+
 DMME_API int dmme_attention_heads(int dtype, const void* qkv, int N, int S, int C, int heads, void* out, int force_generic, void* stream) {
     DMME_REQUIRE(qkv && out && N > 0 && S > 0 && C > 0 && heads > 0 && C % heads == 0, DMME_ERR_INVALID, "attention_heads: bad argument");
     if (dtype == DMME_BF16X3) {
diff --git a/diffusion-models-made-easy_amd/diffusion_models/chain.py b/diffusion-models-made-easy_amd/diffusion_models/chain.py
--- a/diffusion-models-made-easy_amd/diffusion_models/chain.py
+++ b/diffusion-models-made-easy_amd/diffusion_models/chain.py
@@ -1,6 +1,7 @@
 
 from __future__ import annotations
 
+import gc
 from typing import Optional
 
 import torch
@@ -95,12 +96,18 @@
     check()
     restore()
     graph, out, error = None, None, None
+    gc.collect()
+    gc_was_on = gc.isenabled()
+    gc.disable()
     try:
         graph = torch.cuda.CUDAGraph()
         with torch.cuda.graph(graph):
             out = launch()
     except RuntimeError as exc:
         graph, out, error = None, None, exc
+    finally:
+        if gc_was_on:
+            gc.enable()
     restore()
     return graph, out, error
 
@@ -148,13 +155,13 @@
         return [self.x, self.state]
 
     def _weights_key(self):
-        return (self.plan.packed_version, self.plan.packed.data_ptr())
+        return (self.plan.packed_version, self.plan.fold_version, self.plan.packed.data_ptr())
 
     def step(self):
         model = self.model
         if model.training:
             raise RuntimeError("ChainRunner: sampling chains run in eval mode (no dropout masks inside the replayed step)")
-        packed = model._packed_for(self.plan)
+        packed = model._packed_for(self.plan, fold=True)
         wkey = self._weights_key()
         if not self.use_graph or self.capture_error is not None:
             self._launch(packed)
diff --git a/diffusion-models-made-easy_amd/models/ddpm.py b/diffusion-models-made-easy_amd/models/ddpm.py
--- a/diffusion-models-made-easy_amd/models/ddpm.py
+++ b/diffusion-models-made-easy_amd/models/ddpm.py
@@ -44,6 +44,7 @@
         self.workspace = None
         self.packed = None
         self.packed_version = None
+        self.fold_version = None
         self.fwd_gen = 0
 
     def overwritten(self):
@@ -259,12 +260,16 @@
             self._plans[key] = plan
         return plan
 
-    def _packed_for(self, plan: _Plan) -> Tensor:
+    def _packed_for(self, plan: _Plan, fold: bool = False) -> Tensor:
         flat = self._ensure_flat()
         ver = self._weights_key(flat)
         if plan.packed_version != ver:
             _lib.check(plan.lib.dmme_unet_pack_params(plan.h, _lib.ptr(flat), _lib.ptr(plan.packed), _lib.stream_ptr()), "dmme_unet_pack_params")
             plan.packed_version = ver
+            plan.fold_version = None
+        if fold and plan.fold_version != ver:
+            _lib.check(plan.lib.dmme_unet_pack_folded(plan.h, _lib.ptr(plan.packed), _lib.stream_ptr()), "dmme_unet_pack_folded")
+            plan.fold_version = ver
         return plan.packed
 
     def inject_dropout_masks(self, masks: Optional[Tensor]):
@@ -438,7 +443,7 @@
             raise _lib.DmmeError("UNet.forward while a gradient exchange of this model is in flight: call reducer.finish() first")
         B, _, H, W = x.shape
         plan = self._plan_for(B, H, W, x.device)
-        packed = self._packed_for(plan)
+        packed = self._packed_for(plan, fold=not want_ctx)
         xin = x.detach().to(torch.float32).contiguous()
         if c.is_floating_point() and bool((c != c.round()).any()):
             raise NotImplementedError("fractional timesteps are not supported by the HIP path (integer t only)")
diff --git a/include/dmme_hip.h b/include/dmme_hip.h
--- a/include/dmme_hip.h
+++ b/include/dmme_hip.h
@@ -65,8 +65,11 @@
 DMME_API int64_t dmme_unet_plan_dropmask_numel(const dmme_plan* plan);
 DMME_API int dmme_unet_plan_out_channels(const dmme_plan* plan);
 DMME_API int dmme_unet_plan_num_launches(const dmme_plan* plan);
+DMME_API int dmme_unet_plan_num_launches_nograd(const dmme_plan* plan);
+DMME_API int dmme_unet_plan_num_folded(const dmme_plan* plan);
 
 DMME_API int dmme_unet_pack_params(const dmme_plan* plan, const float* ref_flat, void* packed, void* stream);
+DMME_API int dmme_unet_pack_folded(const dmme_plan* plan, void* packed, void* stream);
 
 DMME_API int dmme_unet_forward(const dmme_plan* plan, const void* packed, const float* x, const int64_t* t, int t_len,
                       float* y, void* workspace, const float* drop_masks, void* stream);
@@ -271,6 +274,11 @@
 DMME_API int dmme_attention(int dtype, const void* qkv, int N, int S, int C, void* out, int force_generic, void* stream);
 DMME_API int dmme_attention_proj(int dtype, const void* qkv, int N, int S, int C, const void* w, const float* bias, const void* res,
                                  void* dst, void* ctx, float* gn_part, int gn_cg, void* stream);
+DMME_API int dmme_attention_fold(int dtype, int C, const void* wqkv, const float* bqkv, const void* wp, const float* bp, void* M, float* c, void* wpv,
+                                 float* bias2, void* stream);
+DMME_API int dmme_attention_block(int dtype, const void* x, int N, int S, int C, const float* parts, int part_tiles, int part_cnt, int groups,
+                                  const float* gamma, const float* beta, float eps, float* scale, float* shift, const void* M, const float* c,
+                                  const void* wpv, const float* bias2, const void* res, void* dst, float* gn_part, int gn_cg, void* stream);
 
 DMME_API int dmme_attention_heads(int dtype, const void* qkv, int N, int S, int C, int heads, void* out, int force_generic, void* stream);
 
```

Measured after the change: 472.6 denoising steps/s (one step = UNet forward + DDPM update on a batch of 128), summed over GPUs, median of 6. 4.3% higher.
